# eigenfoo/littlemcmc

Hardware: AMD Instinct MI355X
Metric: leapfrog-steps/sec (all chains) (higher is better)
Workload: dtype f64

## Files before the change

include/lmc_hip.h:

```cpp
#ifndef LMC_HIP_H_
#define LMC_HIP_H_

#include <stdint.h>

#ifdef __cplusplus
extern "C" {
#endif

#define LMC_ABI_VERSION 8

#define LMC_OK 0
#define LMC_ERR_INVALID 1
#define LMC_ERR_HIP 2
#define LMC_ERR_STATE 3

#define LMC_KIND_NUTS 0
#define LMC_KIND_HMC 1

#define LMC_POT_DIAG_ADAPT 0
#define LMC_POT_DIAG 1
#define LMC_POT_FULL 2
#define LMC_POT_FULL_INV 3
#define LMC_POT_FULL_ADAPT 4
#define LMC_POT_FULL_F64 5

#define LMC_TARGET_STD_NORMAL 0
#define LMC_TARGET_DIAG_GAUSSIAN 1
#define LMC_TARGET_AR1 2
#define LMC_TARGET_FUNNEL 3
#define LMC_TARGET_NORMAL1D 4
#define LMC_TARGET_USER 5
#define LMC_TARGET_EXTERNAL 6

#define LMC_SDOT_NATIVE 0
#define LMC_SDOT_OPENBLAS_SKYLAKEX 1
#define LMC_SDOT_OPENBLAS_HASWELL 2

#define LMC_RNG_NUMPY 0
#define LMC_RNG_PHILOX 1

#define LMC_LDS_PLAN_AUTO 0
#define LMC_LDS_PLAN_SHALLOW 1
#define LMC_LDS_PLAN_DEEP 2

#define LMC_STATUS_BAD_INITIAL_ENERGY 1

#define LMC_STAT_STEP_SIZE 0
#define LMC_STAT_STEP_SIZE_BAR 1
#define LMC_STAT_ACCEPT 2
#define LMC_STAT_ENERGY_ERROR 3
#define LMC_STAT_ENERGY 4
#define LMC_STAT_MAX_ENERGY_ERROR 5
#define LMC_STAT_MODEL_LOGP 6
#define LMC_NUM_STAT_F64 7
#define LMC_STAT_DEPTH 0
#define LMC_STAT_TREE_SIZE 1
#define LMC_NUM_STAT_I32 2
#define LMC_STAT_DIVERGING 0
#define LMC_STAT_TUNE 1
#define LMC_STAT_ACCEPTED 2
#define LMC_NUM_STAT_U8 3

#define LMC_CT_REACHED_MAX_TREEDEPTH 0
#define LMC_CT_DIVS_AFTER_TUNE 1
#define LMC_CT_SAMPLES_AFTER_TUNE 2
#define LMC_CT_LEAPFROGS 3
#define LMC_CT_WAVE_TICKS 4
#define LMC_NUM_COUNTERS 5

typedef struct lmc_engine lmc_engine;

typedef struct lmc_tuning {
    int32_t sub_blocks;
    int32_t force_general;
    int32_t general_team;
    int32_t run_ns, run_w;
    int32_t dense_coop_off;
    int32_t dense_cache_rows_p1;
    int32_t dense_lds_slots_p1;
    int32_t chol_hbm;
    int32_t reserved[3];
} lmc_tuning;

typedef struct lmc_config {
    int32_t abi_version;
    int32_t device;
    int32_t chains;
    int32_t dim;
    int32_t kind;
    int32_t target_family;
    int32_t potential;
    int32_t adapt_step_size;
    double target_accept;
    double emax;
    double step_scale;
    double gamma;
    double k;
    double t0;
    int32_t max_treedepth;
    int32_t early_max_treedepth;
    double path_length;
    int32_t max_steps;
    int32_t adaptation_window;
    int32_t lds_levels;
    int32_t start_energy_sdot;
    double adaptation_window_multiplier;
    int32_t rng_mode;
    int32_t mass_f64;
    int32_t lds_plan;
    int32_t reserved0;
    lmc_tuning tuning;
} lmc_config;

void lmc_config_defaults(lmc_config* cfg, int32_t chains, int32_t dim);

const char* lmc_last_error(const lmc_engine* e);
int32_t lmc_abi_version(void);
const char* lmc_build_hash(void);
int32_t lmc_device_count(void);
int32_t lmc_has_target(int32_t family);

int lmc_engine_create(const lmc_config* cfg, lmc_engine** out);
void lmc_engine_destroy(lmc_engine* e);
int lmc_engine_set_stream(lmc_engine* e, void* hip_stream);
int lmc_engine_synchronize(lmc_engine* e);

int lmc_engine_set_target_params(lmc_engine* e, const double* params, int64_t n);

int lmc_engine_set_potential(lmc_engine* e, const double* initial_mean, const double* initial_diag,
                             double initial_weight, int32_t per_chain);

int lmc_engine_set_dense_potential(lmc_engine* e, const double* matrix, const double* initial_mean,
                                   double initial_weight, int32_t adaptation_window,
                                   double adaptation_window_multiplier, int32_t update_window);

int lmc_engine_seed(lmc_engine* e, const uint32_t* seeds);
int lmc_engine_set_rng_state(lmc_engine* e, int32_t chain, const uint32_t* key, int32_t pos,
                             int32_t has_gauss, double gauss);
int lmc_engine_get_rng_state(lmc_engine* e, int32_t chain, uint32_t* key, int32_t* pos,
                             int32_t* has_gauss, double* gauss);

int lmc_engine_set_position(lmc_engine* e, const double* q, int32_t per_chain);
int lmc_engine_get_position(lmc_engine* e, double* q);

int lmc_engine_reset_tuning(lmc_engine* e);
int lmc_engine_set_dual_average(lmc_engine* e, double log_step, double log_bar, double hbar,
                                int32_t count);

int lmc_engine_set_step_jitter(lmc_engine* e, int32_t enable, double lo, double hi);
int lmc_engine_set_step_sizes(lmc_engine* e, const double* step_sizes);
int lmc_engine_diag_update(lmc_engine* e, int32_t tune);
int lmc_engine_reserve(lmc_engine* e, int64_t capacity, int64_t trace_begin);
int lmc_engine_attach_trace(lmc_engine* e, double* dst, int64_t trace_begin);
int lmc_engine_request_stop(lmc_engine* e, int32_t stop);
int64_t lmc_engine_progress(lmc_engine* e);
int lmc_engine_run(lmc_engine* e, int64_t n_tune, int64_t iter_begin, int32_t n_iters);
#define LMC_MAX_RUN_STREAMS 8
int lmc_engine_run_streams(lmc_engine* e, void** streams, int32_t capacity);
int32_t lmc_engine_last_run_plan(lmc_engine* e);

int lmc_engine_get_trace(lmc_engine* e, double* dst, int64_t iter_begin, int64_t n_iters);
int lmc_engine_get_stat_f64(lmc_engine* e, int32_t stat, double* dst, int64_t iter_begin, int64_t n_iters);
int lmc_engine_get_stat_i32(lmc_engine* e, int32_t stat, int32_t* dst, int64_t iter_begin, int64_t n_iters);
int lmc_engine_get_stat_u8(lmc_engine* e, int32_t stat, uint8_t* dst, int64_t iter_begin, int64_t n_iters);
#define LMC_PLANE_F64 0
#define LMC_PLANE_I32 1
#define LMC_PLANE_U8 2
#define LMC_AS_NATIVE 0
#define LMC_AS_F64 1
#define LMC_AS_I64 2
#define LMC_MAX_PLANES 16
typedef struct lmc_window_plane {
    void* dst;
    int32_t kind;
    int32_t idx;
    int32_t as;
    int32_t reserved;
} lmc_window_plane;
typedef struct lmc_window_dst {
    int64_t n_out;
    int64_t first;
    double* trace;
    int32_t n_planes;
    int32_t copy_workgroups;
    lmc_window_plane plane[LMC_MAX_PLANES];
} lmc_window_dst;
int lmc_engine_copy_window_async(lmc_engine* e, const lmc_window_dst* dst, int64_t iter_begin, int64_t n_iters);
int lmc_engine_copy_wait(lmc_engine* e);
void* lmc_host_alloc(uint64_t bytes);
void lmc_host_free(void* p);
int lmc_host_register(void* p, uint64_t bytes);
int lmc_host_unregister(void* p);

#define LMC_STAT_RECORD_BYTES 64
void* lmc_engine_trace_device_ptr(lmc_engine* e);
void* lmc_engine_stat_records_device_ptr(lmc_engine* e);
int64_t lmc_engine_trace_begin(lmc_engine* e);
int64_t lmc_engine_capacity(lmc_engine* e);

int lmc_engine_get_adapt_state(lmc_engine* e, float* var, double* dual_avg, int32_t* da_count,
                               int32_t* n_samples);
typedef struct lmc_chain_state {
    float* var;
    double* fore_mean;
    double* fore_raw_var;
    double* back_mean;
    double* back_raw_var;
    double* fore_w_sum;
    double* back_w_sum;
    int32_t* n_samples;
    double* log_step;
    double* log_bar;
    double* hbar;
    int32_t* da_count;
    int32_t* iter_count;
    int32_t* window;
    double* var64;
} lmc_chain_state;
int lmc_engine_get_chain_state(lmc_engine* e, const lmc_chain_state* dst);
int lmc_engine_set_chain_state(lmc_engine* e, const lmc_chain_state* src);
typedef struct lmc_dense_state {
    float* cov;
    float* chol;
    double* fore_mean;
    double* fore_raw_cov;
    double* fore_n;
    double* back_mean;
    double* back_raw_cov;
    double* back_n;
    int32_t* window;
    int32_t* previous_update;
    int32_t* chol_failures;
    double* cov64;
    double* chol64;
} lmc_dense_state;
int lmc_engine_get_dense_state(lmc_engine* e, const lmc_dense_state* dst);
int lmc_engine_set_dense_state(lmc_engine* e, const lmc_dense_state* src);
int lmc_engine_get_dense_chain(lmc_engine* e, int32_t chain, float* cov, float* chol);
int lmc_engine_get_dense_chain_f64(lmc_engine* e, int32_t chain, double* cov, double* chol);
int lmc_engine_get_dense_factor_f64(lmc_engine* e, double* chol);
int lmc_engine_dense_update(lmc_engine* e, int32_t tune);

// ... 33 lines not shown
```

littlemcmc_amd/_abi.py:

```python
import ctypes as C
import os

import numpy as np

_HERE = os.path.dirname(os.path.abspath(__file__))
LIB_PATH = os.environ.get("LMC_HIP_LIB") or os.path.join(_HERE, "liblmc_hip.so")

ABI_VERSION = 8
OK = 0

KIND_NUTS, KIND_HMC = 0, 1
POT_DIAG_ADAPT, POT_DIAG, POT_FULL, POT_FULL_INV, POT_FULL_ADAPT, POT_FULL_F64 = range(6)
TARGET_STD_NORMAL, TARGET_DIAG_GAUSSIAN, TARGET_AR1, TARGET_FUNNEL, TARGET_NORMAL1D, TARGET_USER, TARGET_EXTERNAL = range(7)
STATUS_BAD_INITIAL_ENERGY = 1
SDOT_NATIVE, SDOT_OPENBLAS_SKYLAKEX, SDOT_OPENBLAS_HASWELL = 0, 1, 2
RNG_NUMPY, RNG_PHILOX = 0, 1
LDS_PLAN_AUTO, LDS_PLAN_SHALLOW, LDS_PLAN_DEEP = 0, 1, 2
PLANE_F64, PLANE_I32, PLANE_U8 = 0, 1, 2
AS_NATIVE, AS_F64, AS_I64 = 0, 1, 2
MAX_PLANES = 16
MAX_RUN_STREAMS = 8
(STAT_STEP_SIZE, STAT_STEP_SIZE_BAR, STAT_ACCEPT, STAT_ENERGY_ERROR, STAT_ENERGY, STAT_MAX_ENERGY_ERROR,
 STAT_MODEL_LOGP) = range(7)
STAT_DEPTH, STAT_TREE_SIZE = 0, 1
STAT_DIVERGING, STAT_TUNE, STAT_ACCEPTED = 0, 1, 2
CT_REACHED_MAX_TREEDEPTH, CT_DIVS_AFTER_TUNE, CT_SAMPLES_AFTER_TUNE, CT_LEAPFROGS, CT_WAVE_TICKS = range(5)
NUM_COUNTERS = 5
STAT_RECORD_BYTES = 64


class Tuning(C.Structure):

    _fields_ = [("sub_blocks", C.c_int32), ("force_general", C.c_int32), ("general_team", C.c_int32), ("run_ns", C.c_int32),
                ("run_w", C.c_int32), ("dense_coop_off", C.c_int32), ("dense_cache_rows_p1", C.c_int32),
                ("dense_lds_slots_p1", C.c_int32), ("chol_hbm", C.c_int32), ("reserved", C.c_int32 * 3)]


class Config(C.Structure):

    _fields_ = [
        ("abi_version", C.c_int32), ("device", C.c_int32), ("chains", C.c_int32), ("dim", C.c_int32),
        ("kind", C.c_int32), ("target_family", C.c_int32), ("potential", C.c_int32),
        ("adapt_step_size", C.c_int32),
        ("target_accept", C.c_double), ("emax", C.c_double), ("step_scale", C.c_double),
        ("gamma", C.c_double), ("k", C.c_double), ("t0", C.c_double),
        ("max_treedepth", C.c_int32), ("early_max_treedepth", C.c_int32),
        ("path_length", C.c_double), ("max_steps", C.c_int32), ("adaptation_window", C.c_int32),
        ("lds_levels", C.c_int32), ("start_energy_sdot", C.c_int32), ("adaptation_window_multiplier", C.c_double),
        ("rng_mode", C.c_int32), ("mass_f64", C.c_int32), ("lds_plan", C.c_int32), ("reserved0", C.c_int32),
        ("tuning", Tuning),
    ]


class WindowPlane(C.Structure):

    _fields_ = [("dst", C.c_void_p), ("kind", C.c_int32), ("idx", C.c_int32), ("as_", C.c_int32), ("reserved", C.c_int32)]


class WindowDst(C.Structure):

    _fields_ = [("n_out", C.c_int64), ("first", C.c_int64), ("trace", C.c_void_p), ("n_planes", C.c_int32),
                ("copy_workgroups", C.c_int32), ("plane", WindowPlane * MAX_PLANES)]


_P = C.c_void_p


class ChainState(C.Structure):

    FIELDS = (("var", np.float32, True), ("fore_mean", np.float64, True), ("fore_raw_var", np.float64, True),
              ("back_mean", np.float64, True), ("back_raw_var", np.float64, True), ("fore_w_sum", np.float64, False),
              ("back_w_sum", np.float64, False), ("n_samples", np.int32, False), ("log_step", np.float64, False),
              ("log_bar", np.float64, False), ("hbar", np.float64, False), ("da_count", np.int32, False),
              ("iter_count", np.int32, False), ("window", np.int32, False), ("var64", np.float64, True))
    _fields_ = [(name, C.c_void_p) for name, _dt, _vec in FIELDS]


class DenseState(C.Structure):

    FIELDS = (("cov", np.float32, "m"), ("chol", np.float32, "m"), ("fore_mean", np.float64, "v"),
              ("fore_raw_cov", np.float64, "m"), ("fore_n", np.float64, "s"), ("back_mean", np.float64, "v"),
              ("back_raw_cov", np.float64, "m"), ("back_n", np.float64, "s"), ("window", np.int32, "s"),
              ("previous_update", np.int32, "s"), ("chol_failures", np.int32, "s"),
              ("cov64", np.float64, "m"), ("chol64", np.float64, "m"))
    _fields_ = [(name, C.c_void_p) for name, _dt, _k in FIELDS]


_SIGNATURES = {
    "lmc_config_defaults": (None, [C.POINTER(Config), C.c_int32, C.c_int32]),
    "lmc_last_error": (C.c_char_p, [_P]),
    "lmc_abi_version": (C.c_int32, []),
    "lmc_build_hash": (C.c_char_p, []),
    "lmc_device_count": (C.c_int32, []),
    "lmc_has_target": (C.c_int32, [C.c_int32]),
    "lmc_engine_create": (C.c_int, [C.POINTER(Config), C.POINTER(_P)]),
    "lmc_engine_destroy": (None, [_P]),
    "lmc_engine_set_stream": (C.c_int, [_P, _P]),
    "lmc_engine_synchronize": (C.c_int, [_P]),
    "lmc_engine_set_target_params": (C.c_int, [_P, _P, C.c_int64]),
    "lmc_engine_set_potential": (C.c_int, [_P, _P, _P, C.c_double, C.c_int32]),
    "lmc_engine_set_dense_potential": (C.c_int, [_P, _P, _P, C.c_double, C.c_int32, C.c_double, C.c_int32]),
    "lmc_engine_get_dense_state": (C.c_int, [_P, C.POINTER(DenseState)]),
    "lmc_engine_set_dense_state": (C.c_int, [_P, C.POINTER(DenseState)]),
    "lmc_engine_dense_update": (C.c_int, [_P, C.c_int32]),
    "lmc_engine_tick_begin": (C.c_int, [_P, C.c_int64, C.c_int64, C.c_int32]),
    "lmc_engine_tick_positions": (_P, [_P]),
    "lmc_engine_tick": (C.c_int, [_P, _P, _P, C.POINTER(C.c_int32)]),
    "lmc_engine_get_dense_chain": (C.c_int, [_P, C.c_int32, _P, _P]),
    "lmc_engine_get_dense_chain_f64": (C.c_int, [_P, C.c_int32, _P, _P]),
    "lmc_engine_get_dense_factor_f64": (C.c_int, [_P, _P]),
    "lmc_engine_seed": (C.c_int, [_P, _P]),
    "lmc_engine_set_rng_state": (C.c_int, [_P, C.c_int32, _P, C.c_int32, C.c_int32, C.c_double]),
    "lmc_engine_get_rng_state": (C.c_int, [_P, C.c_int32, _P, C.POINTER(C.c_int32), C.POINTER(C.c_int32),
                                           C.POINTER(C.c_double)]),
    "lmc_engine_set_position": (C.c_int, [_P, _P, C.c_int32]),
    "lmc_engine_get_position": (C.c_int, [_P, _P]),
    "lmc_engine_reset_tuning": (C.c_int, [_P]),
    "lmc_engine_set_dual_average": (C.c_int, [_P, C.c_double, C.c_double, C.c_double, C.c_int32]),
    "lmc_engine_reserve": (C.c_int, [_P, C.c_int64, C.c_int64]),
    "lmc_engine_attach_trace": (C.c_int, [_P, _P, C.c_int64]),
    "lmc_engine_run": (C.c_int, [_P, C.c_int64, C.c_int64, C.c_int32]),
    "lmc_engine_run_streams": (C.c_int, [_P, _P, C.c_int32]),
    "lmc_engine_last_run_plan": (C.c_int32, [_P]),
    "lmc_engine_copy_window_async": (C.c_int, [_P, C.POINTER(WindowDst), C.c_int64, C.c_int64]),
    "lmc_engine_copy_wait": (C.c_int, [_P]),
    "lmc_host_alloc": (_P, [C.c_uint64]),
    "lmc_host_free": (None, [_P]),
    "lmc_host_register": (C.c_int, [_P, C.c_uint64]),
    "lmc_host_unregister": (C.c_int, [_P]),
    "lmc_engine_set_step_jitter": (C.c_int, [_P, C.c_int32, C.c_double, C.c_double]),
    "lmc_engine_set_step_sizes": (C.c_int, [_P, _P]),
    "lmc_engine_diag_update": (C.c_int, [_P, C.c_int32]),
    "lmc_engine_get_trace": (C.c_int, [_P, _P, C.c_int64, C.c_int64]),
    "lmc_engine_get_stat_f64": (C.c_int, [_P, C.c_int32, _P, C.c_int64, C.c_int64]),
    "lmc_engine_get_stat_i32": (C.c_int, [_P, C.c_int32, _P, C.c_int64, C.c_int64]),
    "lmc_engine_get_stat_u8": (C.c_int, [_P, C.c_int32, _P, C.c_int64, C.c_int64]),
    "lmc_engine_trace_device_ptr": (_P, [_P]),
    "lmc_engine_stat_records_device_ptr": (_P, [_P]),
    "lmc_engine_trace_begin": (C.c_int64, [_P]),
    "lmc_engine_capacity": (C.c_int64, [_P]),
    "lmc_engine_get_adapt_state": (C.c_int, [_P, _P, _P, _P, _P]),
    "lmc_engine_get_chain_state": (C.c_int, [_P, C.POINTER(ChainState)]),
    "lmc_engine_set_chain_state": (C.c_int, [_P, C.POINTER(ChainState)]),
    "lmc_engine_keep_moments": (C.c_int, [_P, C.c_int32]),
    "lmc_engine_get_moments": (C.c_int, [_P, _P, _P, _P]),
    "lmc_engine_get_status": (C.c_int, [_P, _P]),
    "lmc_engine_get_counters": (C.c_int, [_P, _P]),
    "lmc_engine_trajectory": (C.c_int, [_P, _P, _P, C.c_int32, C.c_double, C.c_int32, C.c_int32,
                                        _P, _P, _P, _P, _P, _P]),
    "lmc_engine_logp_dlogp": (C.c_int, [_P, _P, _P, _P]),
    "lmc_engine_rng_draw": (C.c_int, [_P, _P, C.c_int32, _P]),
    "lmc_engine_draw_momentum": (C.c_int, [_P, _P]),
    "lmc_engine_kernel_shape": (C.c_int, [_P, _P, _P, _P]),
    "lmc_engine_uses_general_kernels": (C.c_int32, [_P]),
    "lmc_engine_occupancy": (C.c_int, [_P, _P, _P, _P]),
    "lmc_engine_request_stop": (C.c_int, [_P, C.c_int32]),
    "lmc_engine_progress": (C.c_int64, [_P]),
    "lmc_engine_run_lds_bytes": (C.c_int32, [_P]),
    "lmc_engine_load_user_kernels": (C.c_int, [_P, _P, C.c_char_p, C.c_char_p, C.c_char_p]),
    "lmc_engine_load_user_run_plan1": (C.c_int, [_P, C.c_char_p]),
    "lmc_diag_lags_per_pass": (C.c_int, []),
    "lmc_diag_chain_stats": (C.c_int, [_P, C.c_int64, C.c_int64, C.c_int32, C.c_int64, C.c_int64, C.c_int32, _P, _P]),
}

EXPORTED_SYMBOLS = tuple(_SIGNATURES)
_libs = {}


class HipLibraryError(RuntimeError):
    """The HIP library is missing, stale or failed; there is no CPU path to fall back to."""


def load(path=None):
    path = os.path.abspath(path or LIB_PATH)
    if path in _libs:
        return _libs[path]
    if not os.path.exists(path):
        raise HipLibraryError(
            "%s not found: the HIP extension is not built. Run `python -c \"import __graft_entry__ as g; "
            "g.build()\"` (needs hipcc). littlemcmc_amd has no CPU fallback." % path)
    try:
        lib = C.CDLL(path)
    except OSError as err:
        raise HipLibraryError("cannot load %s: %s" % (path, err))
    for name, (res, args) in _SIGNATURES.items():
        try:
            fn = getattr(lib, name)
        except AttributeError:
            raise HipLibraryError("%s does not export %s (stale build?)" % (path, name))
        fn.restype = res
        fn.argtypes = args
    if lib.lmc_abi_version() != ABI_VERSION:
        raise HipLibraryError("ABI version mismatch: python %d, library %d" % (ABI_VERSION, lib.lmc_abi_version()))
    _libs[path] = lib
    return lib


def ptr(a):
    if a is None:
        return None
    if isinstance(a, (int, np.integer)):
        return C.c_void_p(int(a))
    assert a.flags["C_CONTIGUOUS"], "array must be C-contiguous"
    return C.c_void_p(a.ctypes.data)
```

littlemcmc_amd/csrc/lmc_engine.hip:

```cpp
#include <hip/hip_runtime.h>

#include <cmath>
#include <cstdarg>
#include <cstdio>
#include <algorithm>
#include <cstdlib>
#include <cstring>
#include <new>
#include <string>
#include <vector>

#include "../../include/lmc_hip.h"
#include "lmc_sampler.hpp"
#include "lmc_unit_kernels.hpp"
#include "lmc_dense_launch.hpp"
#include "lmc_tick_launch.hpp"
#include "lmc_wide_launch.hpp"
#ifdef LMC_USER_TARGET_HEADER
#include LMC_USER_TARGET_HEADER
#endif

using namespace lmc;

#define LMC_LAUNCH(...)            \
// ... 176 lines not shown
    const long long k = static_cast<long long>(blockIdx.x) * blockDim.x + threadIdx.x;
    if (k >= static_cast<long long>(chains) * n) return;
    const long long c = k / n, i = k - c * n;
    const StatRecord& r = rec[c * cap + iter_begin + i];
    if (kind == 0) static_cast<double*>(out)[k] = r.f64[idx];
    else if (kind == 1) static_cast<int*>(out)[k] = (idx == kSiTreeSize || hmc) ? r.tree_size : static_cast<int>(r.depth_flags & 0xffffu);
    else static_cast<unsigned char*>(out)[k] = static_cast<unsigned char>((r.depth_flags >> (16 + idx)) & 1u);
}

struct WindowPlanes {
    int n_planes;
    int kind[LMC_MAX_PLANES], idx[LMC_MAX_PLANES], as[LMC_MAX_PLANES];
    void* dst[LMC_MAX_PLANES];
};
__global__ void window_gather_kernel(const StatRecord* rec, long long cap, int chain0, int chains, long long iter_begin, long long n, int hmc,
                                     WindowPlanes W, long long n_out, long long row0) {
    const long long total = static_cast<long long>(chains) * n;
    for (long long k = static_cast<long long>(blockIdx.x) * blockDim.x + threadIdx.x; k < total; k += static_cast<long long>(gridDim.x) * blockDim.x) {
        const long long c = chain0 + k / n, i = k % n;
        const StatRecord r = rec[c * cap + iter_begin + i];
        const long long o = c * n_out + row0 + i;
        for (int p = 0; p < W.n_planes; ++p) {
            void* out = W.dst[p];
            if (W.kind[p] == LMC_PLANE_F64) {
                static_cast<double*>(out)[o] = r.f64[W.idx[p]];
            } else if (W.kind[p] == LMC_PLANE_I32) {
                const int v = (W.idx[p] == kSiTreeSize || hmc) ? r.tree_size : static_cast<int>(r.depth_flags & 0xffffu);
                if (W.as[p] == LMC_AS_F64) static_cast<double*>(out)[o] = static_cast<double>(v);
                else if (W.as[p] == LMC_AS_I64) static_cast<long long*>(out)[o] = static_cast<long long>(v);
                else static_cast<int*>(out)[o] = v;
            } else {
                static_cast<unsigned char*>(out)[o] = static_cast<unsigned char>((r.depth_flags >> (16 + W.idx[p])) & 1u);
            }
        }
    }
}

template <int V>
__global__ void window_trace_copy_kernel(const double* __restrict__ src, long long src_pitch, double* __restrict__ dst, long long dst_pitch,
                                         long long row, int chains) {
    for (int c = blockIdx.x; c < chains; c += gridDim.x) {
        const double* s = src + c * src_pitch;
        double* t = dst + c * dst_pitch;
        if constexpr (V == 2) {
            const double2* s2 = reinterpret_cast<const double2*>(s);
            double2* t2 = reinterpret_cast<double2*>(t);
            for (long long k = threadIdx.x; k < row / 2; k += blockDim.x) t2[k] = s2[k];
        } else {
            for (long long k = threadIdx.x; k < row; k += blockDim.x) t[k] = s[k];
        }
    }
}

__global__ void derive_inv_std_kernel(ChainArrays A, int from64) {
    const long long idx = static_cast<long long>(blockIdx.x) * blockDim.x + threadIdx.x;
    const long long n = static_cast<long long>(A.chains) * A.dpad;
    if (idx >= n) return;
    if (from64) {
        const double v = A.var64[idx];
        A.inv_std64[idx] = 1.0 / sqrt(v);
        A.var[idx] = static_cast<float>(v);
        A.inv_std[idx] = static_cast<float>(A.inv_std64[idx]);
        return;
    }
    const float sd = sqrtf(A.var[idx]);
    A.inv_std[idx] = 1.0f / sd;
    if (A.var64 != nullptr) {
        A.var64[idx] = static_cast<double>(A.var[idx]);
        A.inv_std64[idx] = static_cast<double>(A.inv_std[idx]);
    }
}

}

static thread_local std::string g_last_error;

struct lmc_engine {
    lmc_config cfg;
    int ns = 0, dpad = 0, nlds = 1, lds_bytes = 0;
    int nlds1 = 1, lds_bytes1 = 0, lds_plan = 0;
    int lds_plan_wanted = 0;
    int plan_now = 0;
    int plan_last = -1;
    bool wide = false;
    double* init_diag64 = nullptr;
    int run_ns = 0, run_w = 1;
    hipStream_t own_stream = nullptr, stream_ = nullptr;
#ifndef LMC_MAX_SUB
#define LMC_MAX_SUB 4
#endif
#ifndef LMC_DEFAULT_SUB
#define LMC_DEFAULT_SUB 4
#endif
    static constexpr int kMaxSub = LMC_MAX_SUB;
    int n_sub = 1;
    hipStream_t sub_stream[kMaxSub] = {};
    hipEvent_t sub_done[kMaxSub] = {};
    hipEvent_t main_done = nullptr;
    bool trace_external = false;
    hipStream_t copy_stream = nullptr;
    hipEvent_t copy_dep[kMaxSub + 1] = {};
    double* chol64T = nullptr;
    uint32_t* seeds = nullptr;
    int* stop_host = nullptr;
    int step_jitter = 0;
    int step_jitter_device = 0;
    double* step_override = nullptr;
    double jitter_lo = 1.0, jitter_hi = 1.0;
    bool sub_pending = false;
    bool main_dirty = true;
    ChainArrays A;
    double* tparams = nullptr;
    int64_t n_tparams = 0;
    double* init_mean = nullptr;
    float* init_diag = nullptr;
    double init_weight = 10.0;
    bool potential_set = false;
    double* da_tables = nullptr;
    double initial_step = 0.0;
    DenseArrays D;
    int d8 = 0;
    void* cov1T = nullptr;
    void* fac1 = nullptr;
    double* raw1T = nullptr;
    double* mean1 = nullptr;
    double dense_weight = 1.0, dense_multiplier = 2.0;
    int dense_window = 101, dense_update_window = 1;
    TickArrays K;
    bool ticking = false;
    int* adapt_mask = nullptr;
    hipModule_t user_module = nullptr;
    hipFunction_t user_run = nullptr, user_trajectory = nullptr, user_logp = nullptr;
    hipFunction_t user_run1 = nullptr;
    std::vector<void*> allocs;
    std::string err;
};

static hipStream_t main_stream(lmc_engine* e) {
    if (e->sub_pending) {
        for (int b = 0; b < e->n_sub; ++b) {
            (void)hipEventRecord(e->sub_done[b], e->sub_stream[b]);
            (void)hipStreamWaitEvent(e->stream_, e->sub_done[b], 0);
        }
        e->sub_pending = false;
    }
    e->main_dirty = true;
    return e->stream_;
}

static hipError_t order_sub_blocks_after_main(lmc_engine* e) {
    if (e->n_sub <= 1) return hipSuccess;
    const bool external = e->stream_ != e->own_stream;
    if (!e->main_dirty && !external) return hipSuccess;
    hipError_t err = hipEventRecord(e->main_done, e->stream_);
    for (int b = 0; b < e->n_sub && err == hipSuccess; ++b) err = hipStreamWaitEvent(e->sub_stream[b], e->main_done, 0);
    if (err == hipSuccess) e->main_dirty = false;
    return err;
}
static hipError_t order_external_stream_after_sub_blocks(lmc_engine* e) {
    if (e->n_sub <= 1 || e->stream_ == e->own_stream || !e->sub_pending) return hipSuccess;
    hipError_t err = hipSuccess;
    for (int b = 0; b < e->n_sub && err == hipSuccess; ++b) {
        err = hipEventRecord(e->sub_done[b], e->sub_stream[b]);
        if (err == hipSuccess) err = hipStreamWaitEvent(e->stream_, e->sub_done[b], 0);
    }
    if (err == hipSuccess) e->sub_pending = false;
// ... 227 lines not shown
}

extern "C" {

int32_t lmc_abi_version(void) { return LMC_ABI_VERSION; }

#ifndef LMC_SOURCE_HASH
#define LMC_SOURCE_HASH "unstamped"
#endif
static const char kBuildStamp[] = "LMC_BUILD_HASH=" LMC_SOURCE_HASH;
const char* lmc_build_hash(void) { return kBuildStamp + 15; }

int32_t lmc_device_count(void) {
    int n = 0;
    if (hipGetDeviceCount(&n) != hipSuccess) { (void)hipGetLastError(); return 0; }
    return n;
}

int32_t lmc_has_target(int32_t family) {
#if !(defined(LMC_USER_TARGET_HEADER) && defined(LMC_ONLY_USER))
    if (family >= LMC_TARGET_STD_NORMAL && family <= LMC_TARGET_NORMAL1D) return 1;
#endif
    if (family == LMC_TARGET_USER) return 1;
    if (family == LMC_TARGET_EXTERNAL) return 1;
    return 0;
}

const char* lmc_last_error(const lmc_engine* e) {
    if (e && !e->err.empty()) return e->err.c_str();
    return g_last_error.c_str();
}

void lmc_config_defaults(lmc_config* cfg, int32_t chains, int32_t dim) {
    std::memset(cfg, 0, sizeof(*cfg));
    cfg->abi_version = LMC_ABI_VERSION;
    cfg->device = 0;
    cfg->chains = chains;
    cfg->dim = dim;
    cfg->kind = LMC_KIND_NUTS;
    cfg->target_family = LMC_TARGET_STD_NORMAL;
    cfg->potential = LMC_POT_DIAG_ADAPT;
    cfg->adapt_step_size = 1;
    cfg->target_accept = 0.8;
    cfg->emax = 1000.0;
    cfg->step_scale = 0.25;
    cfg->gamma = 0.05;
    cfg->k = 0.75;
    cfg->t0 = 10.0;
    cfg->max_treedepth = 10;
    cfg->early_max_treedepth = 8;
    cfg->path_length = 2.0;
    cfg->max_steps = 1024;
    cfg->adaptation_window = 101;
    cfg->adaptation_window_multiplier = 1.0;
    cfg->rng_mode = LMC_RNG_NUMPY;
    cfg->mass_f64 = 0;
    cfg->lds_levels = 0;
    cfg->lds_plan = LMC_LDS_PLAN_AUTO;
    cfg->start_energy_sdot = LMC_SDOT_OPENBLAS_SKYLAKEX;
}

static int launch_reset(lmc_engine* e, int reset_step, int reset_mass) {
    const long long n = static_cast<long long>(e->cfg.chains) * e->dpad;
    const int threads = 256;
    const int blocks = static_cast<int>((n + threads - 1) / threads);
    const double log_step0 = std::log(e->initial_step);
    const double mu = std::log(10 * e->initial_step);
    LMC_LAUNCH(reset_kernel, dim3(blocks), dim3(threads), 0, main_stream(e), e->A, e->init_mean, e->init_diag,
                       e->init_diag64, e->cfg.mass_f64, e->init_weight, e->cfg.potential == LMC_POT_DIAG_ADAPT ? 1 : 0, log_step0, mu, reset_step,
                       reset_mass, e->cfg.adaptation_window);
    HIP_TRY(e, hipGetLastError());
    return LMC_OK;
}

int lmc_engine_create(const lmc_config* cfg, lmc_engine** out) {
    if (!cfg || !out) return fail(nullptr, LMC_ERR_INVALID, "null argument");
    *out = nullptr;
    if (cfg->abi_version != LMC_ABI_VERSION)
        return fail(nullptr, LMC_ERR_INVALID, "ABI version mismatch: header %d, library %d", cfg->abi_version,
                    LMC_ABI_VERSION);
    if (cfg->chains < 1 || cfg->dim < 1) return fail(nullptr, LMC_ERR_INVALID, "chains and dim must be >= 1");
    if (cfg->lds_plan < LMC_LDS_PLAN_AUTO || cfg->lds_plan > LMC_LDS_PLAN_DEEP)
        return fail(nullptr, LMC_ERR_INVALID, "unknown lds_plan %d", cfg->lds_plan);
    if (cfg->reserved0 != 0 || cfg->tuning.reserved[0] != 0 || cfg->tuning.reserved[1] != 0 || cfg->tuning.reserved[2] != 0)
        return fail(nullptr, LMC_ERR_INVALID, "reserved fields of lmc_config must be 0");
    if (cfg->potential < LMC_POT_DIAG_ADAPT || cfg->potential > LMC_POT_FULL_F64)
        return fail(nullptr, LMC_ERR_INVALID, "unknown potential %d", cfg->potential);
    if (cfg->mass_f64 && cfg->potential > LMC_POT_DIAG && cfg->potential != LMC_POT_FULL_ADAPT)
        return fail(nullptr, LMC_ERR_INVALID, "mass_f64 is the dtype of the diagonal potentials and of LMC_POT_FULL_ADAPT "
                                              "(float64 fixed matrices: LMC_POT_FULL_F64 / LMC_POT_FULL_INV)");
    const bool rtc_dense = cfg->target_family == LMC_TARGET_USER && !kUserCompiledInDense && cfg->potential >= LMC_POT_FULL &&
                           cfg->potential != LMC_POT_FULL_ADAPT;
    const bool forced = cfg->tuning.force_general != 0 && cfg->rng_mode == LMC_RNG_NUMPY &&
                        (cfg->target_family != LMC_TARGET_EXTERNAL || cfg->potential < LMC_POT_FULL);
    const bool wide = cfg->dim > 1024 || (cfg->potential >= LMC_POT_FULL && cfg->dim > 256) || cfg->mass_f64 != 0 || rtc_dense || forced;
    if (wide) {
        if (cfg->dim > kWideMaxDim)
            return fail(nullptr, LMC_ERR_INVALID, "dim %d is beyond the general kernels' %d", cfg->dim, kWideMaxDim);
        if (cfg->potential >= LMC_POT_FULL && cfg->dim > kWideMaxDenseDim)
            return fail(nullptr, LMC_ERR_INVALID, "dense mass matrices are supported up to dim %d (got %d)", kWideMaxDenseDim, cfg->dim);
        if (cfg->potential == LMC_POT_FULL_ADAPT && cfg->dim > kWideMaxDenseAdaptDim)
            return fail(nullptr, LMC_ERR_INVALID, "per-chain adapted dense matrices (FULL_ADAPT) are supported up to dim %d (got %d)",
                        kWideMaxDenseAdaptDim, cfg->dim);
        if (cfg->target_family == LMC_TARGET_EXTERNAL && (cfg->potential >= LMC_POT_FULL || cfg->mass_f64))
            return fail(nullptr, LMC_ERR_INVALID, "an externally evaluated density runs with diagonal float32 mass matrices at any dim up to %d, "
                                                  "with dense ones up to dim 256; give the density as a device functor for the other shapes", kWideMaxDim);
        if (cfg->rng_mode != LMC_RNG_NUMPY)
            return fail(nullptr, LMC_ERR_INVALID, "LMC_RNG_PHILOX runs in the fused kernels only");
    }
    if (!lmc_has_target(cfg->target_family))
        return fail(nullptr, LMC_ERR_INVALID, "target family %d is not built into this library", cfg->target_family);
    if (cfg->target_family == LMC_TARGET_NORMAL1D && cfg->dim != 1)
        return fail(nullptr, LMC_ERR_INVALID, "LMC_TARGET_NORMAL1D requires dim == 1");
    if (cfg->kind != LMC_KIND_NUTS && cfg->kind != LMC_KIND_HMC)
        return fail(nullptr, LMC_ERR_INVALID, "unknown step kind %d", cfg->kind);
    if (cfg->start_energy_sdot < LMC_SDOT_NATIVE || cfg->start_energy_sdot > LMC_SDOT_OPENBLAS_HASWELL)
        return fail(nullptr, LMC_ERR_INVALID, "unknown start_energy_sdot mode %d", cfg->start_energy_sdot);
    if (cfg->adaptation_window < 1 || !(cfg->adaptation_window_multiplier > 0.0))
        return fail(nullptr, LMC_ERR_INVALID, "adaptation_window must be >= 1 and its multiplier > 0");
    if (cfg->rng_mode != LMC_RNG_NUMPY && cfg->rng_mode != LMC_RNG_PHILOX)
        return fail(nullptr, LMC_ERR_INVALID, "unknown rng_mode %d", cfg->rng_mode);
    if (cfg->rng_mode == LMC_RNG_PHILOX && (cfg->potential >= LMC_POT_FULL ||
                                            cfg->target_family == LMC_TARGET_USER || cfg->target_family == LMC_TARGET_EXTERNAL))
        return fail(nullptr, LMC_ERR_INVALID, "LMC_RNG_PHILOX runs in the fused diagonal-mass kernels with the built-in densities");
    if (cfg->max_treedepth < 1 || cfg->max_treedepth > 20 || cfg->early_max_treedepth < 1 ||
        cfg->early_max_treedepth > 20)
        return fail(nullptr, LMC_ERR_INVALID, "max_treedepth must be in [1, 20]");
    int ndev = 0;
    hipError_t herr = hipGetDeviceCount(&ndev);
    if (herr != hipSuccess || ndev < 1)
        return fail(nullptr, LMC_ERR_HIP, "no HIP device available (%s)", hipGetErrorString(herr));
    if (cfg->device < 0 || cfg->device >= ndev)
        return fail(nullptr, LMC_ERR_INVALID, "device %d out of range (%d devices)", cfg->device, ndev);

    lmc_engine* e = new (std::nothrow) lmc_engine();
    if (!e) return fail(nullptr, LMC_ERR_INVALID, "out of host memory");
    e->cfg = *cfg;
    e->wide = wide;
    e->ns = ns_for_dim(cfg->dim);
    e->dpad = 64 * e->ns;
    if (wide) {
        const bool large_team = cfg->dim > kWideOneWaveMaxDim || cfg->target_family == LMC_TARGET_EXTERNAL || cfg->tuning.general_team == 16;
        const int threads = large_team ? kWideBlock : 64;
        int wns = 1;
        while (threads * wns < cfg->dim) wns *= 2;
        e->ns = e->run_ns = wns;
        e->run_w = threads / 64;
        e->dpad = threads * wns;
    } else
    if (e->ns <= 2) { e->run_ns = e->ns; e->run_w = 1; }
    else if (e->ns == 4) { e->run_ns = 4; e->run_w = 1; }
    else if (e->ns == 8) { e->run_ns = 4; e->run_w = 2; }
    else { e->run_ns = 4; e->run_w = 4; }
    if (!wide && cfg->tuning.run_ns > 0 && cfg->tuning.run_w > 0) {
        if (64 * cfg->tuning.run_ns * cfg->tuning.run_w == e->dpad) { e->run_ns = cfg->tuning.run_ns; e->run_w = cfg->tuning.run_w; }
    }
    e->initial_step = cfg->step_scale / std::pow(static_cast<double>(cfg->dim), 0.25);

    auto bail = [&](int rc) {
        lmc_engine_destroy(e);
        return rc;
    };
    hipError_t se = hipSetDevice(cfg->device);
    if (se != hipSuccess) return bail(fail(nullptr, LMC_ERR_HIP, "hipSetDevice: %s", hipGetErrorString(se)));
    {
        int pr_low = 0, pr_high = 0;
        se = hipDeviceGetStreamPriorityRange(&pr_low, &pr_high);
        if (se == hipSuccess) se = hipStreamCreateWithPriority(&e->own_stream, hipStreamNonBlocking, pr_high);
    }
    if (se != hipSuccess) return bail(fail(nullptr, LMC_ERR_HIP, "hipStreamCreate: %s", hipGetErrorString(se)));
    e->stream_ = e->own_stream;
    e->n_sub = (cfg->chains >= 128 && !wide) ? (LMC_DEFAULT_SUB < lmc_engine::kMaxSub ? LMC_DEFAULT_SUB : lmc_engine::kMaxSub) : 1;
    if (e->n_sub > 2 && cfg->potential >= LMC_POT_FULL) e->n_sub = 2;
    if (cfg->tuning.sub_blocks >= 1 && cfg->tuning.sub_blocks <= lmc_engine::kMaxSub && cfg->tuning.sub_blocks <= cfg->chains)
        e->n_sub = cfg->tuning.sub_blocks;
    if (cfg->tuning.sub_blocks <= -1 && e->n_sub > -cfg->tuning.sub_blocks) e->n_sub = -cfg->tuning.sub_blocks;
    if (cfg->tuning.sub_blocks <= -1 && cfg->potential >= LMC_POT_FULL) e->n_sub = 1;
    if (e->n_sub > 1) {
        for (int b = 0; b < e->n_sub; ++b) {
            se = hipStreamCreateWithFlags(&e->sub_stream[b], hipStreamNonBlocking);
            if (se == hipSuccess) se = hipEventCreateWithFlags(&e->sub_done[b], hipEventDisableTiming);
            if (se != hipSuccess) return bail(fail(nullptr, LMC_ERR_HIP, "sub-block stream: %s", hipGetErrorString(se)));
        }
        se = hipEventCreateWithFlags(&e->main_done, hipEventDisableTiming);
        if (se != hipSuccess) return bail(fail(nullptr, LMC_ERR_HIP, "hipEventCreate: %s", hipGetErrorString(se)));
    }

    const int max_levels = (cfg->max_treedepth > cfg->early_max_treedepth ? cfg->max_treedepth
                                                                          : cfg->early_max_treedepth);
    int nlds = 1;
    if (wide) {
        e->nlds = 1;
        e->lds_bytes = wide_lds_bytes(e->dpad);
    } else {
        const int waves_per_cu = 4 * run_waves_per_simd(e->run_ns, e->run_w);
        const int blocks_per_cu = waves_per_cu / e->run_w > 0 ? waves_per_cu / e->run_w : 1;
        const long budget = (163840L / blocks_per_cu) / 1280 * 1280 - lds_tail_doubles(e->run_w) * 8L;
        if (pair_min_doubles(e->run_ns, e->run_w) * 8L > budget)
            return bail(fail(nullptr, LMC_ERR_INVALID, "the sampling kernel's LDS plan does not fit the budget"));
        nlds = cfg->lds_levels > 0 ? cfg->lds_levels : 1;
        if (cfg->lds_levels <= 0)
            while (nlds < max_levels && pair_total_doubles(e->run_ns, e->run_w, nlds + 1) * 8L <= budget) ++nlds;
        if (nlds > max_levels) nlds = max_levels;
        if (nlds < 1) nlds = 1;
        e->nlds = nlds;
        e->lds_bytes = pair_total_doubles(e->run_ns, e->run_w, nlds) * 8;
        e->nlds1 = nlds;
        e->lds_bytes1 = 0;
        e->lds_plan = 0;
        const long budget1 = (163840L / blocks_per_cu) / 1280 * 1280;
        if (e->run_w == 1 && run_mt_in_lds(1) && cfg->lds_levels <= 0 && pair_min_doubles(e->run_ns, 1, 1) * 8L <= budget1) {
            int n1 = 1;
            while (n1 < max_levels && pair_total_doubles(e->run_ns, 1, n1 + 1, 1) * 8L <= budget1) ++n1;
            e->nlds1 = n1;
            e->lds_bytes1 = pair_total_doubles(e->run_ns, 1, n1, 1) * 8;
            e->lds_plan = cfg->lds_plan == LMC_LDS_PLAN_SHALLOW ? 0 : cfg->lds_plan == LMC_LDS_PLAN_DEEP ? 1 : 2;
            if (e->nlds1 <= e->nlds) e->lds_plan = 0;
            if (cfg->rng_mode == LMC_RNG_PHILOX) e->lds_plan = 0;
            e->lds_plan_wanted = e->lds_plan;
            if (cfg->target_family == LMC_TARGET_USER && !kUserCompiledIn)
                e->lds_plan = 0;
            e->plan_now = e->lds_plan == 1 ? 1 : 0;
        }
    }
    if (e->lds_bytes > 160 * 1024) return bail(fail(nullptr, LMC_ERR_INVALID, "lds_levels too large"));

    const size_t C = cfg->chains, dp = e->dpad;
    ChainArrays& A = e->A;
    std::memset(&A, 0, sizeof(A));
    A.chains = cfg->chains;
    A.d = cfg->dim;
    A.dpad = e->dpad;
    int rc = LMC_OK;
#define TRY_ALLOC(x) if ((rc = (x)) != LMC_OK) return bail(rc)
    TRY_ALLOC(dev_alloc(e, &A.q, C * dp));
    TRY_ALLOC(dev_alloc(e, &A.var, C * dp));
    TRY_ALLOC(dev_alloc(e, &A.inv_std, C * dp));
    TRY_ALLOC(dev_alloc(e, &A.wmean, 2 * C * dp));
    TRY_ALLOC(dev_alloc(e, &A.wraw, 2 * C * dp));
    TRY_ALLOC(dev_alloc(e, &A.wsum, C * 2));
    TRY_ALLOC(dev_alloc(e, &A.wsel, C));
    TRY_ALLOC(dev_alloc(e, &A.n_samples, C));
    TRY_ALLOC(dev_alloc(e, &A.awindow, C));
    TRY_ALLOC(dev_alloc(e, &A.da, C * 4));
    TRY_ALLOC(dev_alloc(e, &A.da_count, C));
    TRY_ALLOC(dev_alloc(e, &A.iter_count, C));
    TRY_ALLOC(dev_alloc(e, &A.mt, C * kMtN));
    TRY_ALLOC(dev_alloc(e, &A.rng_pos, C));
    TRY_ALLOC(dev_alloc(e, &A.rng_has_gauss, C));
    TRY_ALLOC(dev_alloc(e, &A.rng_gauss, C));
    TRY_ALLOC(dev_alloc(e, &A.status, C));
    TRY_ALLOC(dev_alloc(e, &A.counters, C * kNumCounters));
    {
        void* dev_view = nullptr;
        if (hipHostMalloc(reinterpret_cast<void**>(&e->stop_host), 128, hipHostMallocMapped | hipHostMallocCoherent) != hipSuccess ||
            hipHostGetDevicePointer(&dev_view, e->stop_host, 0) != hipSuccess)
            return bail(fail(nullptr, LMC_ERR_HIP, "stop word: %s", hipGetErrorString(hipGetLastError())));
        std::memset(e->stop_host, 0, 128);
        A.stop = static_cast<const int*>(dev_view);
        A.progress = static_cast<int*>(dev_view) + 16;
        A.tree_hint = static_cast<int*>(dev_view) + 24;
    }
    TRY_ALLOC(dev_alloc(e, &A.stop_dev, 1));
    TRY_ALLOC(dev_alloc(e, &e->seeds, C));
    A.seed = e->seeds;
    A.scratch_stride = static_cast<long long>(max_levels - nlds + 1) * 4 * dp + static_cast<long long>(kNumColdSlots) * dp;
    const bool dense = cfg->potential >= LMC_POT_FULL;
    if (dense) A.scratch_stride = static_cast<long long>(dense_scratch_vectors(max_levels)) * dp;
    const bool external = cfg->target_family == LMC_TARGET_EXTERNAL;
    if (external) A.scratch_stride = static_cast<long long>(dense ? tick_dense_scratch_vectors(max_levels) : tick_scratch_vectors(max_levels)) * dp;
    if (wide) {
        if (!external) A.scratch_stride = static_cast<long long>(wide_scratch_slots(max_levels)) * dp;
        TRY_ALLOC(dev_alloc(e, &A.var64, C * dp));
        TRY_ALLOC(dev_alloc(e, &A.inv_std64, C * dp));
        TRY_ALLOC(dev_alloc(e, &e->init_diag64, C * dp));
    }
    TRY_ALLOC(dev_alloc(e, &A.scratch, C * static_cast<size_t>(A.scratch_stride), false));
    TRY_ALLOC(dev_alloc(e, &e->init_mean, C * dp));
    TRY_ALLOC(dev_alloc(e, &e->init_diag, C * dp));
    TRY_ALLOC(dev_alloc(e, &e->tparams, 8));
    {
        const int len = 16384;
        std::vector<double> tab(2 * static_cast<size_t>(len));
        for (int i = 0; i < len; ++i) {
            tab[i] = std::sqrt(static_cast<double>(i));
            tab[len + i] = i > 0 ? std::pow(static_cast<double>(i), -cfg->k) : 0.0;
        }
        TRY_ALLOC(dev_alloc(e, &e->da_tables, tab.size(), false));
        hipError_t ce = hipMemcpy(e->da_tables, tab.data(), tab.size() * sizeof(double), hipMemcpyHostToDevice);
        if (ce != hipSuccess) return bail(fail(nullptr, LMC_ERR_HIP, "da tables: %s", hipGetErrorString(ce)));
        A.da_sqrt = e->da_tables;
        A.da_mk = e->da_tables + len;
        A.da_table_len = len;
    }
#undef TRY_ALLOC
    std::memset(&e->K, 0, sizeof(e->K));
    if (external) {
        TickArrays& K = e->K;
// ... 76 lines not shown
        rc = lmc_engine_set_potential(e, zeros.data(), ones.data(), 10.0, 0);
        if (rc != LMC_OK) return bail(rc);
        rc = launch_reset(e, 1, 0);
        if (rc != LMC_OK) return bail(rc);
        if (dense) {
            std::vector<double> eye(static_cast<size_t>(cfg->dim) * cfg->dim, 0.0);
            for (int i = 0; i < cfg->dim; ++i) eye[static_cast<size_t>(i) * cfg->dim + i] = 1.0;
            rc = lmc_engine_set_dense_potential(e, eye.data(), zeros.data(), 1.0, 101, 2.0, 1);
            if (rc != LMC_OK) return bail(rc);
        }
        std::vector<uint32_t> seeds(C, 0u);
        rc = lmc_engine_seed(e, seeds.data());
        if (rc != LMC_OK) return bail(rc);
    }
    se = hipStreamSynchronize(main_stream(e));
    if (se != hipSuccess) return bail(fail(nullptr, LMC_ERR_HIP, "engine init: %s", hipGetErrorString(se)));
    *out = e;
    return LMC_OK;
}

void lmc_engine_destroy(lmc_engine* e) {
    if (!e) return;
    (void)hipSetDevice(e->cfg.device);
    if (e->stream_) (void)hipStreamSynchronize(main_stream(e));
    for (int b = 0; b < lmc_engine::kMaxSub; ++b) {
        if (e->sub_stream[b]) { (void)hipStreamSynchronize(e->sub_stream[b]); (void)hipStreamDestroy(e->sub_stream[b]); }
        if (e->sub_done[b]) (void)hipEventDestroy(e->sub_done[b]);
    }
    if (e->main_done) (void)hipEventDestroy(e->main_done);
    if (e->copy_stream) { (void)hipStreamSynchronize(e->copy_stream); (void)hipStreamDestroy(e->copy_stream); }
    for (hipEvent_t ev : e->copy_dep)
        if (ev) (void)hipEventDestroy(ev);
    if (e->stop_host) (void)hipHostFree(e->stop_host);
    for (void* p : e->allocs)
        if (p) (void)hipFree(p);
    if (e->user_module) (void)hipModuleUnload(e->user_module);
    if (e->own_stream) (void)hipStreamDestroy(e->own_stream);
    delete e;
}


int lmc_engine_kernel_shape(lmc_engine* e, int32_t* unit_ns, int32_t* run_ns, int32_t* run_w) {
    if (!e) return fail(nullptr, LMC_ERR_INVALID, "null engine");
    if (unit_ns) *unit_ns = e->ns;
    if (run_ns) *run_ns = e->run_ns;
    if (run_w) *run_w = e->run_w;
    return LMC_OK;
}

int32_t lmc_engine_uses_general_kernels(lmc_engine* e) { return (e && e->wide) ? 1 : 0; }

int lmc_engine_occupancy(lmc_engine* e, int32_t* resident_chains, int32_t* waves_per_chain, double* wall_clock_hz) {
    if (!e) return fail(nullptr, LMC_ERR_INVALID, "null engine");
    HIP_TRY(e, hipSetDevice(e->cfg.device));
    if (waves_per_chain) *waves_per_chain = e->run_w;
    if (wall_clock_hz) {
        int khz = 0;
        HIP_TRY(e, hipDeviceGetAttribute(&khz, hipDeviceAttributeWallClockRate, e->cfg.device));
        *wall_clock_hz = 1e3 * khz;
    }
    if (!resident_chains) return LMC_OK;
    *resident_chains = 0;
    if (e->cfg.target_family == LMC_TARGET_EXTERNAL || e->cfg.potential >= LMC_POT_FULL || e->wide) return LMC_OK;
    int cus = 0;
    HIP_TRY(e, hipDeviceGetAttribute(&cus, hipDeviceAttributeMultiprocessorCount, e->cfg.device));
    const int run_lds = sampling_lds_bytes(e);
    const int block = 64 * e->run_w;
    int per_cu = 0;
    if (e->cfg.target_family == LMC_TARGET_USER && !kUserCompiledIn) {
        if (!e->user_run) return fail(e, LMC_ERR_STATE, "the user density's kernels are not loaded");
        HIP_TRY(e, hipModuleOccupancyMaxActiveBlocksPerMultiprocessor(&per_cu, e->user_run, block, static_cast<size_t>(run_lds)));
        *resident_chains = per_cu * cus;
        return LMC_OK;
    }
#define OCC_ONE(NSV, WV, T)                                                                                    \
    if (!found && e->run_ns == NSV && e->run_w == WV) {                                                        \
        found = true;                                                                                          \
        if (e->cfg.rng_mode == LMC_RNG_PHILOX) {                                                               \
            if (run_lds > 64 * 1024)                                                                           \
                HIP_TRY(e, hipFuncSetAttribute(reinterpret_cast<const void*>(&run_kernel<NSV, WV, T, 1>),      \
                                               hipFuncAttributeMaxDynamicSharedMemorySize, run_lds));          \
            HIP_TRY(e, hipOccupancyMaxActiveBlocksPerMultiprocessor(&per_cu, run_kernel<NSV, WV, T, 1>, block, \
                                                                    static_cast<size_t>(run_lds)));            \
        } else {                                                                                               \
            if (run_lds > 64 * 1024)                                                                           \
                HIP_TRY(e, hipFuncSetAttribute(reinterpret_cast<const void*>(&run_kernel<NSV, WV, T>),         \
                                               hipFuncAttributeMaxDynamicSharedMemorySize, run_lds));          \
            HIP_TRY(e, hipOccupancyMaxActiveBlocksPerMultiprocessor(&per_cu, run_kernel<NSV, WV, T>, block,    \
                                                                    static_cast<size_t>(run_lds)));            \
        }                                                                                                      \
    }
#define OCC_CALL(T)                                                                                            \
    {                                                                                                          \
        bool found = false;                                                                                    \
        LMC_FOR_EACH_SHAPE(OCC_ONE, T)                                                                         \
        if (!found) return fail(e, LMC_ERR_INVALID, "unsupported kernel shape ns=%d w=%d", e->run_ns, e->run_w); \
    }
    LMC_FAMILY_SWITCH(e, e->cfg.target_family, OCC_CALL)
#undef OCC_CALL
#undef OCC_ONE
    *resident_chains = per_cu * cus;
    return LMC_OK;
}

int32_t lmc_engine_run_lds_bytes(lmc_engine* e) {
    if (!e || e->cfg.target_family == LMC_TARGET_EXTERNAL || (e->cfg.potential >= LMC_POT_FULL && !e->wide)) return -1;
    if (e->wide) return e->lds_bytes;
    return sampling_lds_bytes(e, e->plan_last >= 0 ? e->plan_last : e->plan_now);
}

int32_t lmc_engine_last_run_plan(lmc_engine* e) {
    if (!e || e->plan_last < 0 || e->wide || e->cfg.potential >= LMC_POT_FULL || e->cfg.target_family == LMC_TARGET_EXTERNAL) return 0;
    return e->plan_last == 1 ? LMC_LDS_PLAN_DEEP : LMC_LDS_PLAN_SHALLOW;
}

int lmc_engine_load_user_kernels(lmc_engine* e, const void* code_object, const char* run_name, const char* trajectory_name,
                                 const char* logp_name) {
    if (!e || !code_object || !run_name || !trajectory_name || !logp_name) return fail(e, LMC_ERR_INVALID, "null argument");
    if (e->cfg.target_family != LMC_TARGET_USER)
        return fail(e, LMC_ERR_STATE, "lmc_engine_load_user_kernels() needs cfg.target_family = LMC_TARGET_USER");
    HIP_TRY(e, hipSetDevice(e->cfg.device));
    HIP_TRY(e, hipStreamSynchronize(main_stream(e)));
    if (e->user_module) { (void)hipModuleUnload(e->user_module); e->user_module = nullptr; }
    e->user_run = e->user_trajectory = e->user_logp = nullptr;
    e->user_run1 = nullptr;
    if (e->cfg.target_family == LMC_TARGET_USER && !kUserCompiledIn) { e->lds_plan = 0; e->plan_now = 0; }
    HIP_TRY(e, hipModuleLoadData(&e->user_module, code_object));
    HIP_TRY(e, hipModuleGetFunction(&e->user_run, e->user_module, run_name));
    HIP_TRY(e, hipModuleGetFunction(&e->user_trajectory, e->user_module, trajectory_name));
    HIP_TRY(e, hipModuleGetFunction(&e->user_logp, e->user_module, logp_name));
    return LMC_OK;
}

int lmc_engine_load_user_run_plan1(lmc_engine* e, const char* run_name_plan1) {
    if (!e || !run_name_plan1) return fail(e, LMC_ERR_INVALID, "null argument");
    if (!e->user_module) return fail(e, LMC_ERR_STATE, "lmc_engine_load_user_kernels() first");
    if (e->wide || e->run_w != 1) return fail(e, LMC_ERR_INVALID, "the deep-tree LDS plan exists for the one-wave sampling kernels");
    HIP_TRY(e, hipSetDevice(e->cfg.device));
    HIP_TRY(e, hipModuleGetFunction(&e->user_run1, e->user_module, run_name_plan1));
    e->lds_plan = e->lds_plan_wanted;
    e->plan_now = e->lds_plan == 1 ? 1 : 0;
    return LMC_OK;
}

static int user_launch(lmc_engine* e, hipFunction_t f, hipStream_t st, unsigned grid, unsigned block, unsigned lds, void** args) {
    if (!f)
        return fail(e, LMC_ERR_STATE, "the user density's kernels are not loaded: call lmc_engine_load_user_kernels() "
                                      "(littlemcmc_amd.targets.UserTarget does)");
    if (e->cfg.potential >= LMC_POT_FULL && !e->wide)
        return fail(e, LMC_ERR_INVALID, "a run-time compiled user density runs with diagonal mass matrices in the fused kernels; "
                                        "dense ones (Full / FullInv) take the general kernels, FullAdapt needs the density compiled in (UserTarget(..., jit=\"hipcc\"))");
    (void)hipGetLastError();
    HIP_TRY(e, hipModuleLaunchKernel(f, grid, 1, 1, block, 1, 1, lds, st, args, nullptr));
    return LMC_OK;
}

int lmc_engine_set_step_sizes(lmc_engine* e, const double* step_sizes) {
    if (!e) return fail(nullptr, LMC_ERR_INVALID, "null engine");
    HIP_TRY(e, hipSetDevice(e->cfg.device));
    if (!step_sizes) {
        if (e->step_jitter == 2) e->step_jitter = e->step_jitter_device;
        return LMC_OK;
    }
    if (!e->step_override) {
        int rc = dev_alloc(e, &e->step_override, static_cast<size_t>(e->cfg.chains));
        if (rc != LMC_OK) return rc;
        e->A.step_override = e->step_override;
    }
    HIP_TRY(e, hipMemcpyAsync(e->step_override, step_sizes, sizeof(double) * e->cfg.chains, hipMemcpyDefault, main_stream(e)));
    HIP_TRY(e, hipStreamSynchronize(main_stream(e)));
    e->step_jitter = 2;
    return LMC_OK;
}

int lmc_engine_diag_update(lmc_engine* e, int32_t tune) {
    if (!e) return fail(nullptr, LMC_ERR_INVALID, "null engine");
    if (e->cfg.potential != LMC_POT_DIAG_ADAPT) return LMC_OK;
    if (!tune) return LMC_OK;
    HIP_TRY(e, hipSetDevice(e->cfg.device));
    SamplerParams P;
    std::memset(&P, 0, sizeof(P));
    P.window = e->cfg.adaptation_window;
    P.window_multiplier = e->cfg.adaptation_window_multiplier;
    P.mass_f64 = e->cfg.mass_f64 ? 1 : 0;
    if (e->wide) {
        const int rc = wide_launch_mass_update(e->ns, e->run_w, main_stream(e), e->A, P);
        if (rc != 0) return dense_fail(e, rc, "diag_update (general kernel)");
        return LMC_OK;
    }
    const dim3 grid(e->cfg.chains), block(64);
    LMC_NS_SWITCH(e, e->ns, LMC_LAUNCH((mass_update_kernel<NS>), grid, block, 0, main_stream(e), e->A, P))
    HIP_TRY(e, hipGetLastError());
    return LMC_OK;
// ... 626 lines not shown
    P.k = e->cfg.k;
    P.t0 = e->cfg.t0;
    P.max_treedepth = e->cfg.max_treedepth;
    P.early_max_treedepth = e->cfg.early_max_treedepth;
    P.path_length = e->cfg.path_length;
    P.max_steps = e->cfg.max_steps;
    P.window = e->cfg.adaptation_window;
    P.window_multiplier = e->cfg.adaptation_window_multiplier;
    P.n_tune = n_tune;
    P.iter_begin = iter_begin;
    P.n_iters = n_iters;
    P.nlds = e->nlds;
    P.lds_doubles = e->lds_bytes / 8;
    P.sdot_mode = e->cfg.start_energy_sdot;
    P.rng_mode = e->cfg.rng_mode;
    P.step_jitter = e->step_jitter;
    P.jitter_lo = e->jitter_lo;
    P.jitter_hi = e->jitter_hi;
    P.relay_mask = 255;
    return P;
}

static int wide_run(lmc_engine* e, SamplerParams P) {
    if (e->cfg.potential >= LMC_POT_FULL) P.momentum_f32 = !e->D.mat_f64;
    if (e->cfg.potential != LMC_POT_DIAG_ADAPT) P.adapt_mass = 0;
    P.chain_begin = 0;
    P.relay_mask = relay_mask_for(e->cfg.chains);
    hipStream_t st = main_stream(e);
    const bool rtc = e->cfg.target_family == LMC_TARGET_USER && !kUserCompiledInDense;
    const long long end = P.iter_begin + P.n_iters;
    long long it = P.iter_begin;
    while (it < end) {
        const bool adapt = e->cfg.potential == LMC_POT_FULL_ADAPT && it < P.n_tune;
        SamplerParams Q = P;
        Q.iter_begin = it;
        Q.n_iters = static_cast<int>(adapt ? 1 : end - it);
        int rc;
        if (rtc) {
            void* args[] = {&e->A, &e->D, &Q, &e->tparams};
            rc = user_launch(e, e->user_run, st, static_cast<unsigned>(e->cfg.chains), 64u * e->run_w, static_cast<unsigned>(e->lds_bytes), args);
            if (rc != LMC_OK) return rc;
        } else {
            rc = wide_launch_run(e->cfg.target_family, e->ns, e->run_w, st, e->A, e->D, Q, e->tparams, e->cfg.chains);
            if (rc != 0) return dense_fail(e, rc, "run (general kernel)");
        }
        if (adapt) {
            rc = dense_launch_adapt(st, e->A, e->D, e->dense_multiplier, e->dense_update_window, nullptr, 0, e->cfg.chains,
                                    static_cast<int>(it + 1));
            if (rc != 0) return dense_fail(e, rc, "dense update");
        }
        it += Q.n_iters;
    }
    return LMC_OK;
}

int lmc_engine_run(lmc_engine* e, int64_t n_tune, int64_t iter_begin, int32_t n_iters) {
    if (!e) return fail(nullptr, LMC_ERR_INVALID, "null engine");
    if (e->A.cap <= 0 || !e->A.stat_rec) return fail(e, LMC_ERR_STATE, "lmc_engine_reserve() must be called before run()");
    if (iter_begin < 0 || n_iters < 0 || iter_begin + n_iters > e->A.cap)
        return fail(e, LMC_ERR_INVALID, "iterations [%lld, %lld) exceed reserved capacity %lld", (long long)iter_begin,
                    (long long)(iter_begin + n_iters), (long long)e->A.cap);
    if (n_iters == 0) return LMC_OK;
    if (e->cfg.target_family == LMC_TARGET_EXTERNAL)
        return fail(e, LMC_ERR_STATE, "the density is evaluated by the caller: drive the chains with lmc_engine_tick_begin() / lmc_engine_tick()");
    HIP_TRY(e, hipSetDevice(e->cfg.device));
    SamplerParams P = make_params(e, n_tune, iter_begin, n_iters);
    if (e->wide) return wide_run(e, P);
    if (e->cfg.potential >= LMC_POT_FULL) return dense_run(e, P);
    int plan = choose_lds_plan(e, iter_begin);
    if (e->run_w != 1 || e->lds_bytes1 <= 0 ||
        (e->cfg.target_family == LMC_TARGET_USER && !kUserCompiledIn && !e->user_run1))
        plan = 0;
    e->plan_last = plan;
    if (plan == 1) {
        P.nlds = e->nlds1;
        P.lds_doubles = e->lds_bytes1 / 8;
    }
    const int run_lds = sampling_lds_bytes(e, plan);
    const dim3 block(64 * e->run_w);
    const int n_sub = e->n_sub;
    HIP_TRY(e, order_sub_blocks_after_main(e));
#define RUN_PLAN1(NSV, WV, T)                                                                                  \
    if constexpr (WV == 1) {                                                                                   \
        LMC_LAUNCH((run_kernel<NSV, 1, T, 0, 1>), grid, block, run_lds, st, e->A, P, e->tparams);              \
    }
#define RUN_ONE(NSV, WV, T)                                                                                    \
    if (!found && e->run_ns == NSV && e->run_w == WV) {                                                        \
        found = true;                                                                                          \
        if (e->cfg.rng_mode == LMC_RNG_PHILOX) {                                                               \
            if (run_lds > 64 * 1024)                                                                           \
                HIP_TRY(e, hipFuncSetAttribute(reinterpret_cast<const void*>(&run_kernel<NSV, WV, T, 1>),      \
                                               hipFuncAttributeMaxDynamicSharedMemorySize, run_lds));          \
            LMC_LAUNCH((run_kernel<NSV, WV, T, 1>), grid, block, run_lds, st, e->A, P, e->tparams);            \
        } else if (plan == 1) {                                                                                \
            RUN_PLAN1(NSV, WV, T)                                                                              \
        } else {                                                                                               \
            if (run_lds > 64 * 1024)                                                                           \
                HIP_TRY(e, hipFuncSetAttribute(reinterpret_cast<const void*>(&run_kernel<NSV, WV, T>),         \
                                               hipFuncAttributeMaxDynamicSharedMemorySize, run_lds));          \
            LMC_LAUNCH((run_kernel<NSV, WV, T>), grid, block, run_lds, st, e->A, P, e->tparams);               \
        }                                                                                                      \
    }
#define RUN_CALL(T)                                                                                            \
    {                                                                                                          \
        bool found = false;                                                                                    \
        LMC_FOR_EACH_SHAPE(RUN_ONE, T)                                                                         \
        if (!found) return fail(e, LMC_ERR_INVALID, "unsupported kernel shape ns=%d w=%d", e->run_ns, e->run_w); \
    }
    for (int b = 0; b < n_sub; ++b) {
        const long long lo = static_cast<long long>(e->cfg.chains) * b / n_sub, hi = static_cast<long long>(e->cfg.chains) * (b + 1) / n_sub;
        P.chain_begin = static_cast<int>(lo);
        P.relay_mask = relay_mask_for(hi - lo);
        const dim3 grid(static_cast<unsigned>(hi - lo));
        hipStream_t st = n_sub > 1 ? e->sub_stream[b] : main_stream(e);
        if (n_sub > 1) e->sub_pending = true;
        if (e->cfg.target_family == LMC_TARGET_USER && !kUserCompiledIn) {
            void* args[] = {&e->A, &P, &e->tparams};
            const int rc = user_launch(e, plan == 1 ? e->user_run1 : e->user_run, st, grid.x, block.x, static_cast<unsigned>(run_lds), args);
            if (rc != LMC_OK) return rc;
            continue;
        }
        LMC_FAMILY_SWITCH(e, e->cfg.target_family, RUN_CALL)
    }
#undef RUN_CALL
#undef RUN_ONE
#undef RUN_PLAN1
    HIP_TRY(e, hipGetLastError());
    HIP_TRY(e, order_external_stream_after_sub_blocks(e));
    return LMC_OK;
}

int lmc_engine_run_streams(lmc_engine* e, void** streams, int32_t capacity) {
    if (!e) return fail(nullptr, LMC_ERR_INVALID, "null engine");
    const int n = e->n_sub > 1 ? e->n_sub : 1;
    if (streams)
        for (int b = 0; b < n && b < capacity; ++b) streams[b] = e->n_sub > 1 ? static_cast<void*>(e->sub_stream[b]) : static_cast<void*>(e->stream_);
    return n;
}

int lmc_engine_tick_begin(lmc_engine* e, int64_t n_tune, int64_t iter_begin, int32_t n_iters) {
    if (!e) return fail(nullptr, LMC_ERR_INVALID, "null engine");
    if (e->cfg.target_family != LMC_TARGET_EXTERNAL)
        return fail(e, LMC_ERR_STATE, "lmc_engine_tick*() needs cfg.target_family = LMC_TARGET_EXTERNAL");
    if (e->A.cap <= 0 || !e->A.stat_rec) return fail(e, LMC_ERR_STATE, "lmc_engine_reserve() must be called before tick_begin()");
    if (iter_begin < 0 || n_iters < 0 || iter_begin + n_iters > e->A.cap)
        return fail(e, LMC_ERR_INVALID, "iterations [%lld, %lld) exceed reserved capacity %lld", (long long)iter_begin,
                    (long long)(iter_begin + n_iters), (long long)e->A.cap);
    HIP_TRY(e, hipSetDevice(e->cfg.device));
    e->K.iter_end = iter_begin + n_iters;
    e->K.n_tune = n_tune;
    const int rc = e->wide ? tick_wide_launch_begin(e->ns, main_stream(e), e->A, e->K, iter_begin)
                           : tick_launch_begin(e->ns, main_stream(e), e->A, e->K, iter_begin);
    if (rc != 0) return fail(e, LMC_ERR_HIP, "tick_begin: %s", rc < 0 ? "unsupported vector width" : hipGetErrorString(static_cast<hipError_t>(rc)));
    e->ticking = true;
    return LMC_OK;
}

void* lmc_engine_tick_positions(lmc_engine* e) { return e ? e->K.q_eval : nullptr; }

int lmc_engine_tick(lmc_engine* e, const double* logp, const double* grad, int32_t* n_active) {
    if (!e || !logp || !grad) return fail(e, LMC_ERR_INVALID, "null argument");
    if (!e->ticking) return fail(e, LMC_ERR_STATE, "lmc_engine_tick_begin() must be called first");
    HIP_TRY(e, hipSetDevice(e->cfg.device));
    SamplerParams P = make_params(e, e->K.n_tune, 0, 0);
    if (e->cfg.potential >= LMC_POT_FULL) {
        P.momentum_f32 = !pot_f64(e->cfg.potential);
        P.adapt_mass = 0;
        int rc = tick_dense_launch(e->ns, pot_f64(e->cfg.potential), main_stream(e), e->A, e->D, e->K, P, logp, grad,
                                   e->adapt_mask);
        if (rc != 0) return dense_fail(e, rc, "tick");
        if (e->cfg.potential == LMC_POT_FULL_ADAPT) {
            rc = dense_launch_adapt(main_stream(e), e->A, e->D, e->dense_multiplier, e->dense_update_window, e->adapt_mask);
            if (rc != 0) return dense_fail(e, rc, "dense update");
        }
    } else {
        const int rc = e->wide ? tick_wide_launch(e->ns, main_stream(e), e->A, e->K, P, logp, grad)
                               : tick_launch(e->ns, main_stream(e), e->A, e->K, P, logp, grad);
        if (rc != 0) return fail(e, LMC_ERR_HIP, "tick: %s", rc < 0 ? "unsupported vector width" : hipGetErrorString(static_cast<hipError_t>(rc)));
// ... 526 lines not shown
```

littlemcmc_amd/csrc/lmc_sampler.hpp:

```cpp
#pragma once
#include "lmc_rng.hpp"
#include "lmc_targets.hpp"
#include "lmc_team.hpp"

namespace lmc {

constexpr int kStatusBadInitialEnergy = 1;

enum StatF64 : int {
    kSfStepSize = 0,
    kSfStepSizeBar = 1,
    kSfAccept = 2,
    kSfEnergyError = 3,
    kSfEnergy = 4,
    kSfMaxEnergyError = 5,
    kSfModelLogp = 6,
    kNumStatF64 = 7
};
enum StatI32 : int { kSiDepth = 0 , kSiTreeSize = 1 , kNumStatI32 = 2 };
enum StatU8 : int { kSbDiverging = 0, kSbTune = 1, kSbAccepted = 2, kNumStatU8 = 3 };
enum Counter : int { kCtMaxTreedepth = 0, kCtDivsSample = 1, kCtSamplesAfterTune = 2, kCtLeapfrogs = 3, kCtWaveTicks = 4, kNumCounters = 5 };

struct StatRecord {
    double f64[kNumStatF64];
// ... 446 lines not shown
    __device__ __forceinline__ void get(int j, double& w_, double& a_, double& c, double& d) const {
        w_ = readlane_f64(w, j); a_ = readlane_f64(a, j); c = readlane_f64(pe, j); d = readlane_f64(plogp, j);
    }
};

struct TransitionOut {
    double accept;
    double energy, energy_error, max_energy_error, model_logp;
    int depth;
    int n_leapfrog;
    int diverging;
    int exhausted;
    int accepted;
};

template <class P>
__device__ inline void hmc_transition_any(P& pol, double e0, double logp0, double step_size, double emax, double path_length,
                                          int max_steps, TransitionOut& out) {
    const double plen = first_f64(pol.uniform() * path_length);
    int n_steps = static_cast<int>(plen / step_size);
    n_steps = n_steps < 1 ? 1 : n_steps;
    n_steps = n_steps > max_steps ? max_steps : n_steps;
    typename P::End c;
    pol.start_state(c);
    double energy = e0, logp = logp0;
    for (int i = 0; i < n_steps; ++i) pol.leapfrog(step_size, c, energy, logp);
    bool diverging = !isfinite(energy);
    double de = first_f64(e0 - energy);
    if (isnan(de)) de = -__builtin_inf();
    if (fabs(de) > emax) diverging = true;
    const double accept = first_f64(fmin(1.0, exp_uniform(de)));
    bool accepted = false;
    if (!diverging) {
        const double u = pol.uniform();
        if (!(u >= accept)) { accepted = true; pol.accept_state(c); }
    }
    out.accept = accept;
    out.energy = energy;
    out.energy_error = de;
    out.max_energy_error = plen;
    out.model_logp = logp;
    out.depth = n_steps;
    out.n_leapfrog = n_steps;
    out.diverging = diverging;
    out.exhausted = 0;
    out.accepted = accepted;
}

template <int NS, class Target, class TeamT>
struct FusedHmcPolicy {
    static constexpr int kNS = NS;
    struct End { double q[NS], p[NS], g[NS]; };
    TeamT& tm; const Target& tgt; const double (&var)[NS]; RngState& rng;
    double (&q)[NS]; const double (&p0)[NS]; const double (&g0)[NS];
    UniformWindow win;
    __device__ __forceinline__ double uniform() { return team_uniform(tm, rng, win); }
    __device__ __forceinline__ void start_state(End& c) const { vcopy(c.q, q); vcopy(c.p, p0); vcopy(c.g, g0); }
    __device__ __forceinline__ void leapfrog(double eps, End& c, double& energy, double& logp) {
        lmc::leapfrog<NS>(tm, tgt, var, eps, c.q, c.p, c.g, energy, logp);
    }
    __device__ __forceinline__ void accept_state(const End& c) { vcopy(q, c.q); }
};
template <int NS, class Target, class TeamT>
__device__ inline void hmc_transition(TeamT& tm, const Target& tgt, const double (&var)[NS], RngState& rng,
                                      double (&q)[NS], const double (&p0)[NS], const double (&g0)[NS],
                                      double e0, double logp0, double step_size, double emax,
                                      double path_length, int max_steps, TransitionOut& out) {
    FusedHmcPolicy<NS, Target, TeamT> pol{tm, tgt, var, rng, q, p0, g0, UniformWindow{0.0, 0, 0}};
    hmc_transition_any(pol, e0, logp0, step_size, emax, path_length, max_steps, out);
}

#ifndef LMC_EXP_LANES_SLOAD
#define LMC_EXP_LANES_SLOAD 2
#endif
constexpr int kRedValues = 6;
constexpr int kExpTableDoubles = 32;
constexpr int kLevelScalDoubles = 96;
#ifndef LMC_PAIR_COLD_LDS
#define LMC_PAIR_COLD_LDS 3
#endif
enum ColdSlot : int { kColdAold = 0, kColdPsum = 1, kColdOp = 2, kColdOq = 3, kColdOg = 4, kNumCold = 5 };
constexpr int kNumColdSlots = kNumCold;

template <int NS, int W = 1, int PL = 0>
struct PairLds {
    static constexpr int DP = 64 * NS * W;
    static constexpr int kRedWave = 64 * kRedValues;
    static constexpr int kRedSize = (2 * DP > W * kRedWave) ? 2 * DP : W * kRedWave;
    static constexpr int kExp = kRedSize;
    static constexpr int kXsum = kExp + kExpTableDoubles;
    static constexpr int kXsumSize = W > 1 ? 2 * 8 * W : 0;
    static constexpr int kScal = kXsum + kXsumSize;
    static constexpr int kCold = kScal + W * kLevelScalDoubles;
    static_assert(PL == 0 || W == 1, "the deep-tree plan exists for one-wave kernels");
    static constexpr int kColdLds = PL == 1 ? (NS >= 4 ? 0 : (LMC_PAIR_COLD_LDS < 1 ? LMC_PAIR_COLD_LDS : 1))
                                            : (W >= 8 ? (LMC_PAIR_COLD_LDS < 2 ? LMC_PAIR_COLD_LDS : 2) : LMC_PAIR_COLD_LDS);
    static constexpr int kL1 = kCold + kColdLds * DP;
    static constexpr int kL2 = kL1 + 3 * DP;
    static constexpr int kMinDoubles = kL2;
    static constexpr int kGlbLevels = (kNumCold - kColdLds) * DP;
    __host__ __device__ static constexpr int total_doubles(int nlds) { return kL2 + (nlds > 1 ? (nlds - 1) * 4 * DP : 0); }
};
#ifdef LMC_EXPERIMENTAL_SHAPES
#define LMC_PAIR_SHAPES(X) X(1, 1) X(2, 1) X(4, 1) X(4, 2) X(4, 4) X(2, 8) X(2, 2) X(1, 4)
#else
#define LMC_PAIR_SHAPES(X) X(1, 1) X(2, 1) X(4, 1) X(4, 2) X(4, 4)
#endif
constexpr int pair_min_doubles(int ns, int w, int plan = 0) {
#define X(NSV, WV) if (ns == NSV && w == WV) return (plan == 1 && WV == 1) ? PairLds<NSV, 1, 1>::kMinDoubles : PairLds<NSV, WV, 0>::kMinDoubles;
    LMC_PAIR_SHAPES(X)
#undef X
    return 1 << 30;
}
constexpr int pair_total_doubles(int ns, int w, int nlds, int plan = 0) {
#define X(NSV, WV) if (ns == NSV && w == WV) return (plan == 1 && WV == 1) ? PairLds<NSV, 1, 1>::total_doubles(nlds) : PairLds<NSV, WV, 0>::total_doubles(nlds);
    LMC_PAIR_SHAPES(X)
#undef X
    return 1 << 30;
}

struct PairCtx {
    double* lds;
    double* glb;
    int nlds;
    int red_lane;
    int wave_red;
    int wave_scal;
    int wave;
    int xpar;
};

template <int NS, int W = 1, int PL = 0>
__device__ __forceinline__ void red_put(const PairCtx& cx, int v, double x) {
    if constexpr (W == 1) ((lds_double*)cx.lds)[v * 64 + lane_id()] = x;
    else ((lds_double*)cx.lds)[v * 64 + lane_id() + cx.wave_red] = x;
}
template <int NS, int W = 1, int PL = 0>
__device__ __forceinline__ double red_gather(PairCtx& cx) {
    typedef double d2 __attribute__((ext_vector_type(2)));
    typedef __attribute__((address_space(3))) d2 lds_d2;
    asm volatile("" ::: "memory");
    unsigned r0 = static_cast<unsigned>(cx.red_lane);
    asm volatile("" : "+v"(r0));
    lds_double* L = (lds_double*)cx.lds;
    const d2 a = *(const lds_d2*)(size_t)(r0), b = *(const lds_d2*)(size_t)(r0 ^ 16u);
    const d2 c = *(const lds_d2*)(size_t)(r0 ^ 32u), d = *(const lds_d2*)(size_t)(r0 ^ 48u);
    asm volatile("" ::: "memory");
    double s = ((a.x + a.y) + (b.x + b.y)) + ((c.x + c.y) + (d.x + d.y));
    s += dpp_f64<0x111>(s);
    s += dpp_f64<0x112>(s);
    s += dpp_f64<0x114>(s);
    if constexpr (W > 1) {
        const int lane = lane_id();
        lds_double* xs = L + (PairLds<NS, W, PL>::kXsum + cx.xpar * (8 * W)) + (lane >> 3) * W;
        if ((lane & 7) == 7) xs[cx.wave] = s;
        __syncthreads();
        double t = xs[0];
#pragma unroll
        for (int w = 1; w < W; ++w) t += xs[w];
        s = t;
        cx.xpar ^= 1;
    }
    return s;
}
__device__ __forceinline__ int red_lane_init() {
    const int lane = lane_id();
    const int row = lane < 8 * kRedValues ? lane : 0;
    return row * 8 + 2 * ((lane >> 2) & 3);
}
__device__ __forceinline__ bool red_any_nonpositive(double s, int k0, int n) {
    const unsigned long long m = ballot64(s <= 0.0);
    unsigned long long sel = 0ull;
    for (int k = k0; k < k0 + n; ++k) sel |= 1ull << (8 * k + 7);
    return (m & sel) != 0ull;
}

__constant__ double kExpLanesConst[8] = {46.166241308446828,
                                         2.16608493865351192654e-02,
                                         5.96317165397058656256e-12,
                                         1.0 / 720.0, 1.0 / 120.0, 1.0 / 24.0, 1.0 / 6.0, 0.0};
struct ExpLanesConst { double inv, hi, lo, c6, c5, c4, c3; };
__device__ __forceinline__ ExpLanesConst exp_lanes_const() {
    ExpLanesConst c;
#if LMC_EXP_LANES_SLOAD == 2
    typedef const __attribute__((address_space(4))) double cst_double;
    cst_double* p = (cst_double*)kExpLanesConst;
    asm volatile("" : "+s"(p));
    c.inv = p[0]; c.hi = p[1]; c.lo = p[2]; c.c6 = p[3]; c.c5 = p[4]; c.c4 = p[5]; c.c3 = p[6];
#elif LMC_EXP_LANES_SLOAD == 1
    c.inv = kExpLanesConst[0]; c.hi = kExpLanesConst[1]; c.lo = kExpLanesConst[2];
    c.c6 = kExpLanesConst[3]; c.c5 = kExpLanesConst[4]; c.c4 = kExpLanesConst[5]; c.c3 = kExpLanesConst[6];
#else
    c.inv = LMC_SC(46.166241308446828); c.hi = LMC_SC(2.16608493865351192654e-02); c.lo = LMC_SC(5.96317165397058656256e-12);
    c.c6 = LMC_SC(1.0 / 720.0); c.c5 = LMC_SC(1.0 / 120.0); c.c4 = LMC_SC(1.0 / 24.0); c.c3 = LMC_SC(1.0 / 6.0);
#endif
    return c;
}
template <int NS, int W = 1, int PL = 0>
__device__ __forceinline__ double exp_lanes(const PairCtx& cx, const ExpLanesConst& c, double x) {
    const double kf = rint(x * c.inv);
    double r = __builtin_fma(-kf, c.hi, x);
    r = __builtin_fma(-kf, c.lo, r);
    const int ki = static_cast<int>(kf);
    const double t = ((const lds_double*)cx.lds)[PairLds<NS, W, PL>::kExp + (ki & 31)];
    double p = fma_sgpr_addend(r, c.c6, c.c5);
    p = fma_sgpr_addend(p, r, c.c4);
    p = fma_sgpr_addend(p, r, c.c3);
    p = __builtin_fma(p, r, 0.5);
    p = __builtin_fma(p, r, 1.0);
    p = __builtin_fma(p, r, 1.0);
    return ldexp(p * t, ki >> 5);
}

template <int NS, int W, int PL, int SLOT>
__device__ __forceinline__ void cold_load(const PairCtx& cx, double (&x)[NS]) {
    using L = PairLds<NS, W, PL>;
    if constexpr (SLOT < L::kColdLds) vload_as<NS>((lds_double*)cx.lds + (L::kCold + SLOT * L::DP), x);
    else vload_as<NS>((glb_double*)cx.glb + (SLOT - L::kColdLds) * L::DP, x);
}
template <int NS, int W, int PL, int SLOT>
__device__ __forceinline__ void cold_store(const PairCtx& cx, const double (&x)[NS]) {
    using L = PairLds<NS, W, PL>;
    if constexpr (SLOT < L::kColdLds) vstore_as<NS>((lds_double*)cx.lds + (L::kCold + SLOT * L::DP), x);
    else vstore_as<NS>((glb_double*)cx.glb + (SLOT - L::kColdLds) * L::DP, x);
}
template <int NS, int W = 1, int PL = 0>
__device__ __forceinline__ void level1_load(const PairCtx& cx, double (&lp)[NS], double (&rp)[NS], double (&ps)[NS]) {
    using L = PairLds<NS, W, PL>;
    lds_double* b = (lds_double*)cx.lds + L::kL1;
    vload_as<NS>(b, lp); vload_as<NS>(b + L::DP, rp);
#pragma unroll
    for (int s = 0; s < NS; ++s) ps[s] = lp[s] + rp[s];
}
template <int NS, int W = 1, int PL = 0>
__device__ __forceinline__ void level1_store(const PairCtx& cx, const double (&lp)[NS], const double (&rp)[NS], const double (&pq)[NS]) {
    using L = PairLds<NS, W, PL>;
    lds_double* b = (lds_double*)cx.lds + L::kL1;
    vstore_as<NS>(b, lp); vstore_as<NS>(b + L::DP, rp); vstore_as<NS>(b + 2 * L::DP, pq);
}
template <int NS, int W = 1, int PL = 0>
__device__ __forceinline__ unsigned glb_level_offset(const PairCtx& cx, int j, int v) {
    using L = PairLds<NS, W, PL>;
    unsigned off = L::kGlbLevels + static_cast<unsigned>(j - cx.nlds - 1) * (4u * L::DP) + static_cast<unsigned>(v) * L::DP;
    asm volatile("" : "+s"(off));
    return off;
}
template <int NS, int W = 1, int PL = 0>
__device__ __forceinline__ void levelN_load(const PairCtx& cx, int j, int v, double (&x)[NS]) {
    using L = PairLds<NS, W, PL>;
    int nl = cx.nlds;
    asm volatile("" : "+s"(nl));
    if (j <= nl) vload_as<NS>((lds_double*)cx.lds + (L::kL2 + (j - 2) * 4 * L::DP + v * L::DP), x);
    else vload_as<NS>((glb_double*)cx.glb + glb_level_offset<NS, W, PL>(cx, j, v), x);
}
template <int NS, int W = 1, int PL = 0>
__device__ __forceinline__ void levelN_store(const PairCtx& cx, int j, int v, const double (&x)[NS]) {
    using L = PairLds<NS, W, PL>;
    int nl = cx.nlds;
    asm volatile("" : "+s"(nl));
    if (j <= nl) vstore_as<NS>((lds_double*)cx.lds + (L::kL2 + (j - 2) * 4 * L::DP + v * L::DP), x);
    else vstore_as<NS>((glb_double*)cx.glb + glb_level_offset<NS, W, PL>(cx, j, v), x);
}
template <int NS, int W = 1, int PL = 0>
__device__ __forceinline__ void level_load_lp(const PairCtx& cx, int j, double (&x)[NS]) {
    if (j == 1) vload_as<NS>((lds_double*)cx.lds + PairLds<NS, W, PL>::kL1, x); else levelN_load<NS, W, PL>(cx, j, 0, x);
}
template <int NS, int W = 1, int PL = 0>
__device__ __forceinline__ void level_load_q(const PairCtx& cx, int j, double (&x)[NS]) {
    if (j == 1) vload_as<NS>((lds_double*)cx.lds + (PairLds<NS, W, PL>::kL1 + 2 * PairLds<NS, W, PL>::DP), x); else levelN_load<NS, W, PL>(cx, j, 3, x);
}
template <int NS, int W = 1, int PL = 0>
__device__ __forceinline__ void level_scal_put(const PairCtx& cx, int j, double w, double a, double pe, double plogp) {
    if (lane_id() == 0) {
        lds_double* s = (lds_double*)cx.lds + (PairLds<NS, W, PL>::kScal + 4 * j) + (W > 1 ? cx.wave_scal : 0);
        s[0] = w; s[1] = a; s[2] = pe; s[3] = plogp;
    }
}
template <int NS, int W = 1, int PL = 0>
__device__ __forceinline__ void level_scal_get_wa(const PairCtx& cx, int j, double& w, double& a) {
    const lds_double* s = (const lds_double*)cx.lds + (PairLds<NS, W, PL>::kScal + 4 * j) + (W > 1 ? cx.wave_scal : 0);
    w = s[0]; a = s[1];
}
template <int NS, int W = 1, int PL = 0>
__device__ __forceinline__ void level_scal_park(const PairCtx& cx, int j, double w, double a, int src, int elane, double en, double lp) {
    lds_double* s = (lds_double*)cx.lds + (PairLds<NS, W, PL>::kScal + 4 * j) + (W > 1 ? cx.wave_scal : 0);
    const int lane = lane_id();
    if (src < 0) {
        if (lane == elane) { s[2] = en; s[3] = lp; }
    } else {
        const lds_double* f = (const lds_double*)cx.lds + (PairLds<NS, W, PL>::kScal + 4 * src) + (W > 1 ? cx.wave_scal : 0);
        const double pe = f[2], pl = f[3];
        if (lane == 0) { s[2] = pe; s[3] = pl; }
    }
    if (lane == 0) { s[0] = w; s[1] = a; }
}
template <int NS, int W = 1, int PL = 0>
__device__ __forceinline__ void level_scal_get(const PairCtx& cx, int j, double& w, double& a, double& pe, double& plogp) {
    const lds_double* s = (const lds_double*)cx.lds + (PairLds<NS, W, PL>::kScal + 4 * j) + (W > 1 ? cx.wave_scal : 0);
    w = s[0]; a = s[1]; pe = s[2]; plogp = s[3];
}

template <int NS, class Target, class TeamT>
__device__ __forceinline__ void leapfrog_partial(TeamT& tm, const Target& tgt, const double (&var)[NS], double eps,
                                                 double (&q)[NS], double (&p)[NS], double (&g)[NS], double (&v)[NS],
                                                 double& kin_part, double& lp_part) {
    const double dt = 0.5 * eps;
#pragma unroll
    for (int s = 0; s < NS; ++s) {
        p[s] = p[s] + dt * g[s];
        const double vh = var[s] * p[s];
        q[s] = q[s] + eps * vh;
    }
    if constexpr (Target::kLanePartial) {
        lp_part = tgt.logp_grad_partial(tm, q, g);
    } else {
        const double lp = first_f64(tgt.logp_grad(tm, q, g));
        lp_part = (tm.tid() == 0) ? lp : 0.0;
    }
    double kin = 0.0;
#pragma unroll
    for (int s = 0; s < NS; ++s) {
        p[s] = p[s] + dt * g[s];
        v[s] = var[s] * p[s];
        kin = __builtin_fma(p[s], v[s], kin);
    }
    kin_part = kin;
}

template <int NS, int W = 1, int PL = 0>
__device__ __forceinline__ double cascade_dots(PairCtx& cx, const double (&var)[NS], const double (&alp)[NS],
                                               const double (&arp)[NS], const double (&aps)[NS], const double (&tl)[NS],
                                               double (&tps)[NS], const double (&v)[NS]) {
    double d0 = 0.0, d1 = 0.0, d2 = 0.0, d3 = 0.0, d4 = 0.0, d5 = 0.0;
#pragma unroll
    for (int s = 0; s < NS; ++s) {
        const double p1 = aps[s] + tl[s];
        const double p2 = arp[s] + tps[s];
        const double ps = aps[s] + tps[s];
        const double valp = var[s] * alp[s], vtlp = var[s] * tl[s], varp = var[s] * arp[s];
        d0 = __builtin_fma(ps, valp, d0); d1 = __builtin_fma(ps, v[s], d1);
        d2 = __builtin_fma(p1, valp, d2); d3 = __builtin_fma(p1, vtlp, d3);
        d4 = __builtin_fma(p2, varp, d4); d5 = __builtin_fma(p2, v[s], d5);
        tps[s] = ps;
    }
    red_put<NS, W, PL>(cx, 0, d0); red_put<NS, W, PL>(cx, 1, d1); red_put<NS, W, PL>(cx, 2, d2);
    red_put<NS, W, PL>(cx, 3, d3); red_put<NS, W, PL>(cx, 4, d4); red_put<NS, W, PL>(cx, 5, d5);
    return red_gather<NS, W, PL>(cx);
}

template <int NS, int PL, class Target, class TeamT>
__device__ inline void nuts_transition2(TeamT& tm, const Target& tgt, const double (&var)[NS], RngState& rng,
                                        PairCtx& cx, double* qrow, const double (&q)[NS],
                                        const double (&p0)[NS], const double (&g0)[NS], double e0, double logp0,
                                        double step_size, double emax, int max_depth, bool momentum_f32,
                                        TransitionOut& out) {
    constexpr int W = TeamT::kWaves;
    double cq[NS], cp[NS], cg[NS];
    vcopy(cq, q); vcopy(cp, p0); vcopy(cg, g0);
    cold_store<NS, W, PL, kColdOq>(cx, q); cold_store<NS, W, PL, kColdOp>(cx, p0); cold_store<NS, W, PL, kColdOg>(cx, g0);
    cold_store<NS, W, PL, kColdPsum>(cx, p0);
    bool c_right = true;
    bool c_start = momentum_f32, o_start = momentum_f32;
    double prop_e = e0, prop_logp = logp0;
    double coff = 0.0;
    lds_double* tot = (lds_double*)cx.lds + PairLds<NS, W, PL>::kScal + (W > 1 ? cx.wave_scal : 0);
    if (lane_id() == 0) { tot[0] = 0.0; tot[1] = 0.0; tot[2] = 1.0; tot[3] = 0.0; }
    int depth = 0, n_leap = 0;
    bool diverging = false, turning = false, exhausted = true;
    const bool odd_lane = (lane_id() & 1) != 0;
    UniformWindow win;
    window_reset(win);

    double mde = 0.0;
    const bool lane15 = lane_id() == 15, lane31 = lane_id() == 31;
    auto mde_combined = [&]() -> double {
        const double a = readlane_f64(mde, 15), b = readlane_f64(mde, 31);
        return (fabs(b) > fabs(a)) ? b : a;
    };
    auto leaf_scalars = [&](double s, int n, double& en, double& ev) -> int {
        const ExpLanesConst ec = exp_lanes_const();
        en = 0.5 * dpp_f64<0x118>(s) - s;
        double de = en - e0;
        int ok = 0;
        const bool leaf_lane = lane15 | (lane31 & (n == 2));
        const unsigned long long leaf_bits = (n == 2) ? ((1ull << 15) | (1ull << 31)) : (1ull << 15);
        const unsigned long long rare = ballot64(!(fabs(de) < emax)) | ballot64((-de) - coff > 600.0);
        bool examined = leaf_lane;
        double de_x = de;
        if ((rare & leaf_bits) == 0ull) {
            n_leap += n;
            ok = n;
        } else {
            int seen = 0;
            for (int i = 0; i < n; ++i) {
                double dei = readlane_f64(de, 15 + 16 * i);
                ++n_leap; ++seen;
                if (isnan(dei)) dei = __builtin_inf();
                if (!(fabs(dei) < emax)) { diverging = true; break; }
                const double x = -dei;
                if (x - coff > 600.0) {
                    const double f = exp_uniform(coff - x);
                    const int lane = lane_id();
                    if (lane >= 1 && lane < kLevelScalDoubles / 4) {
                        lds_double* sc = (lds_double*)cx.lds + (PairLds<NS, W, PL>::kScal + 4 * lane) + (W > 1 ? cx.wave_scal : 0);
                        sc[0] = sc[0] * f; sc[1] = sc[1] * f;
                    }
                    coff = x;
                }
                ++ok;
            }
            de_x = isnan(de) ? __builtin_inf() : de;
            examined = lane15 | (lane31 & (seen == 2));
        }
        const bool upd = (fabs(de_x) > fabs(mde)) & examined;
        mde = upd ? de_x : mde;
        const double x = -de;
        const double xn = dpp_f64<0x101>(x);
        const double arg = odd_lane ? (x - coff) : ((xn - coff) + fmin(xn, 0.0));
        ev = exp_lanes<NS, W, PL>(cx, ec, arg);
        return ok;
    };

    for (int dd = 0; dd < max_depth; ++dd) {
        const bool right = team_uniform(tm, rng, win) < 0.5;
        const double eps = right ? step_size : -step_size;
        if (right != c_right) {
            double t[NS];
            cold_load<NS, W, PL, kColdOq>(cx, t); cold_store<NS, W, PL, kColdOq>(cx, cq); vcopy(cq, t);
            cold_load<NS, W, PL, kColdOp>(cx, t); cold_store<NS, W, PL, kColdOp>(cx, cp); vcopy(cp, t);
            cold_load<NS, W, PL, kColdOg>(cx, t); cold_store<NS, W, PL, kColdOg>(cx, cg); vcopy(cg, t);
            const bool tb = c_start; c_start = o_start; o_start = tb;
            c_right = right;
        }
        cold_store<NS, W, PL, kColdAold>(cx, cp);
        const bool aold_start = c_start;

        double tps[NS], eq[NS], ep[NS];
        double tw = 0.0, ta = 0.0;
        int qsrc = -1;
        int elane = 15;
        double en_last = 0.0, lp_last = 0.0;
        const int D = depth;
        if (D == 0) {
            double v[NS], kinp, lp, en, ev;
            leapfrog_partial<NS>(tm, tgt, var, eps, cq, cp, cg, v, kinp, lp);
            red_put<NS, W, PL>(cx, 0, kinp); red_put<NS, W, PL>(cx, 1, lp);
            const double s0 = red_gather<NS, W, PL>(cx);
            if (leaf_scalars(s0, 1, en, ev) == 1) {
                tw = readlane_f64(ev, 15); ta = readlane_f64(ev, 14);
                en_last = en; lp_last = s0;
                vcopy(tps, cp);
            }
        } else {
            const int n_pairs = 1 << (D - 1);
            for (int k = 0; k < n_pairs; ++k) {
                double v[NS], kinA, lpA, kinB, lpB;
                leapfrog_partial<NS>(tm, tgt, var, eps, cq, cp, cg, v, kinA, lpA);
                red_put<NS, W, PL>(cx, 0, kinA); red_put<NS, W, PL>(cx, 1, lpA);
                vcopy(eq, cq); vcopy(ep, cp);
                leapfrog_partial<NS>(tm, tgt, var, eps, cq, cp, cg, v, kinB, lpB);
                red_put<NS, W, PL>(cx, 2, kinB); red_put<NS, W, PL>(cx, 3, lpB);
#pragma unroll
                for (int s = 0; s < NS; ++s) tps[s] = ep[s] + cp[s];
                red_put<NS, W, PL>(cx, 4, pdot_v<NS>(tps, var, ep));
                red_put<NS, W, PL>(cx, 5, pdot<NS>(tps, v));
                const double s0 = red_gather<NS, W, PL>(cx);
                const int m = __builtin_ctz(~static_cast<unsigned>(k) | (1u << (D - 1)));
                double en, ev;
                if (leaf_scalars(s0, 2, en, ev) != 2) break;
                {
                    const double wA = readlane_f64(ev, 15), aA = readlane_f64(ev, 14);
                    const double wB = readlane_f64(ev, 31), aB = readlane_f64(ev, 30);
                    const bool turn = red_any_nonpositive(s0, 4, 2);
                    const double wsum = wA + wB;
                    const bool take_b = uniform_true(team_uniform(tm, rng, win) * wsum < wB);
                    qsrc = take_b ? -1 : -2;
                    elane = take_b ? 31 : 15;
                    en_last = en; lp_last = s0;
                    tw = wsum; ta = aA + aB;
                    if (turn) { turning = true; break; }
                }
                if (m >= 1) {
                    double alp[NS], arp[NS], aps[NS];
                    double aw, aa;
                    level1_load<NS, W, PL>(cx, alp, arp, aps);
                    level_scal_get_wa<NS, W, PL>(cx, 1, aw, aa);
                    const double sj = cascade_dots<NS, W, PL>(cx, var, alp, arp, aps, ep, tps, v);
                    const bool turn = red_any_nonpositive(sj, 0, 6);
                    const double wsum = aw + tw;
                    const bool take_b = uniform_true(team_uniform(tm, rng, win) * wsum < tw);
                    if (!take_b) qsrc = 1;
                    tw = wsum; ta = aa + ta;
                    if (turn) { turning = true; break; }
                }
                for (int j = 2; j <= m; ++j) {
                    double blp[NS], brp[NS], bps[NS], tl[NS];
                    levelN_load<NS, W, PL>(cx, j, 0, blp); levelN_load<NS, W, PL>(cx, j, 1, brp); levelN_load<NS, W, PL>(cx, j, 2, bps);
                    level_load_lp<NS, W, PL>(cx, j - 1, tl);
                    double bw, ba;
                    level_scal_get_wa<NS, W, PL>(cx, j, bw, ba);
                    const double sj = cascade_dots<NS, W, PL>(cx, var, blp, brp, bps, tl, tps, v);
                    const bool turn = red_any_nonpositive(sj, 0, 6);
                    const double wsum = bw + tw;
                    const bool take_b = uniform_true(team_uniform(tm, rng, win) * wsum < tw);
                    if (!take_b) qsrc = j;
                    tw = wsum; ta = ba + ta;
                    if (turn) { turning = true; break; }
                }
                if (turning) break;
                if (k + 1 < n_pairs) {
                    double tl[NS], tqv[NS];
                    if (m == 0) vcopy(tl, ep); else level_load_lp<NS, W, PL>(cx, m, tl);
                    if (qsrc == -1) vcopy(tqv, cq);
                    else if (qsrc == -2) vcopy(tqv, eq);
                    else level_load_q<NS, W, PL>(cx, qsrc, tqv);
#ifndef LMC_PARK_REORDER_MIN_NS
#define LMC_PARK_REORDER_MIN_NS 4
#endif
                    constexpr bool kParkReorder = NS >= LMC_PARK_REORDER_MIN_NS;
                    if constexpr (kParkReorder) level_scal_park<NS, W, PL>(cx, m + 1, tw, ta, qsrc, elane, en_last, lp_last);
                    if (m == 0) {
                        level1_store<NS, W, PL>(cx, tl, cp, tqv);
                    } else {
                        if constexpr (kParkReorder) {
#pragma unroll
                            for (int s = 0; s < NS; ++s) asm volatile("" : "+v"(tl[s]), "+v"(tqv[s]));
                        }
                        levelN_store<NS, W, PL>(cx, m + 1, 0, tl); levelN_store<NS, W, PL>(cx, m + 1, 1, cp);
                        levelN_store<NS, W, PL>(cx, m + 1, 2, tps); levelN_store<NS, W, PL>(cx, m + 1, 3, tqv);
                    }
                    if constexpr (!kParkReorder) level_scal_park<NS, W, PL>(cx, m + 1, tw, ta, qsrc, elane, en_last, lp_last);
                }
            }
        }
        ++depth;
        if (diverging || turning) { exhausted = false; break; }

        double wn = tot[0], an = tot[1], w_start = tot[2];
        const double c_tot = tot[3];
        if (uniform_true(c_tot != coff)) {
            const double f = exp_uniform(first_f64(c_tot) - coff);
            wn = wn * f; an = an * f; w_start = w_start * f;
            if (lane_id() == 0) { tot[2] = w_start; tot[3] = coff; }
        }
        if (uniform_true(team_uniform(tm, rng, win) * (w_start + wn) < tw)) {
            double tqv[NS];
            if (qsrc == -1) vcopy(tqv, cq);
            else if (qsrc == -2) vcopy(tqv, eq);
            else level_load_q<NS, W, PL>(cx, qsrc, tqv);
            vstore_as<NS>((glb_double*)qrow, tqv);
            if (qsrc < 0) {
                prop_e = readlane_f64(en_last, elane); prop_logp = readlane_f64(lp_last, elane);
            } else {
                double w_, a_;
                level_scal_get<NS, W, PL>(cx, qsrc, w_, a_, prop_e, prop_logp);
                prop_e = first_f64(prop_e); prop_logp = first_f64(prop_logp);
            }
        }
        if (lane_id() == 0) { tot[0] = wn + tw; tot[1] = an + ta; }
        double tlp[NS], psum[NS], op[NS], aold[NS];
        if (D == 0) vcopy(tlp, cp);
        else if (D == 1) vcopy(tlp, ep);
        else level_load_lp<NS, W, PL>(cx, D - 1, tlp);
        cold_load<NS, W, PL, kColdPsum>(cx, psum); cold_load<NS, W, PL, kColdOp>(cx, op); cold_load<NS, W, PL, kColdAold>(cx, aold);
#pragma unroll
        for (int s = 0; s < NS; ++s) {
            const double t = psum[s] + tps[s];
            psum[s] = momentum_f32 ? static_cast<double>(static_cast<float>(t)) : t;
        }
        cold_store<NS, W, PL, kColdPsum>(cx, psum);
        double ov[NS], av[NS];
        end_velocity<NS>(ov, var, op, o_start);
        end_velocity<NS>(av, var, aold, aold_start);
        double d0 = 0.0, d1 = 0.0, d2 = 0.0, d3 = 0.0, d4 = 0.0, d5 = 0.0;
        if (right) {
#pragma unroll
            for (int s = 0; s < NS; ++s) {
                const double vtl = var[s] * tlp[s], vtr = var[s] * cp[s];
                const double p1 = psum[s] + tlp[s], p2 = aold[s] + tps[s];
                d0 = __builtin_fma(psum[s], ov[s], d0); d1 = __builtin_fma(psum[s], vtr, d1);
                d2 = __builtin_fma(p1, ov[s], d2);      d3 = __builtin_fma(p1, vtl, d3);
                d4 = __builtin_fma(p2, av[s], d4);      d5 = __builtin_fma(p2, vtr, d5);
            }
        } else {
#pragma unroll
            for (int s = 0; s < NS; ++s) {
                const double vtl = var[s] * tlp[s], vtr = var[s] * cp[s];
                const double p1 = tps[s] + aold[s], p2 = tlp[s] + psum[s];
                d0 = __builtin_fma(psum[s], vtr, d0);   d1 = __builtin_fma(psum[s], ov[s], d1);
                d2 = __builtin_fma(p1, vtr, d2);        d3 = __builtin_fma(p1, av[s], d3);
                d4 = __builtin_fma(p2, vtl, d4);        d5 = __builtin_fma(p2, ov[s], d5);
            }
        }
        c_start = false;
        red_put<NS, W, PL>(cx, 0, d0); red_put<NS, W, PL>(cx, 1, d1); red_put<NS, W, PL>(cx, 2, d2);
        red_put<NS, W, PL>(cx, 3, d3); red_put<NS, W, PL>(cx, 4, d4); red_put<NS, W, PL>(cx, 5, d5);
        if (red_any_nonpositive(red_gather<NS, W, PL>(cx), 0, 6)) { turning = true; exhausted = false; break; }
    }

    const double wn_end = first_f64(tot[0]), an_end = first_f64(tot[1]);
    const double mean_accept = (wn_end > 0.0) ? first_f64(an_end / wn_end) : 0.0;
    out.accept = mean_accept;
    out.energy = prop_e;
    out.energy_error = first_f64(prop_e - e0);
    out.max_energy_error = mde_combined();
    out.model_logp = prop_logp;
    out.depth = depth;
    out.n_leapfrog = n_leap;
    out.diverging = diverging;
    out.exhausted = exhausted;
    out.accepted = 0;
}

#ifndef LMC_NORMALS_IN_REGS
#define LMC_NORMALS_IN_REGS 1
#endif
#ifndef LMC_WAVES_NS1
#define LMC_WAVES_NS1 4
#endif
#ifndef LMC_WAVES_NS2
#define LMC_WAVES_NS2 3
#endif
#ifndef LMC_WAVES_NS4
#define LMC_WAVES_NS4 2
#endif
#ifndef LMC_WAVES_NS2_W8
#define LMC_WAVES_NS2_W8 4
#endif
constexpr int run_waves_per_simd(int ns, int w = 1) {
    return (ns == 2 && w == 8) ? LMC_WAVES_NS2_W8 : ns <= 1 ? LMC_WAVES_NS1 : ns == 2 ? LMC_WAVES_NS2 : ns == 4 ? LMC_WAVES_NS4 : 1;
}
constexpr int kLdsMtDoubles = 320;
#ifndef LMC_MT_IN_LDS_W1
#define LMC_MT_IN_LDS_W1 1
#endif
constexpr bool run_mt_in_lds(int w) { return w > 1 || LMC_MT_IN_LDS_W1; }
constexpr int lds_tail_doubles(int w) {
    return w == 1 ? (run_mt_in_lds(1) ? kLdsMtDoubles : 0) : kLdsMtDoubles + 2 * w * kTeamSlots + 4 + (w >= 4 ? kLdsMtDoubles : 0);
}
constexpr int kPlanUp = 24, kPlanDown = 14;

template <class CA, class PT>
__device__ __forceinline__ int stop_request_load(const CA& A, const PT& P, int chain_in_launch, int it, long long git, long long leaps = -1) {
    int* dev = A.stop_dev;
    const int mask = P.relay_mask;
    const bool relay = (it == 0) ? ((chain_in_launch & mask) == 0)
                                 : ((git & 15) == 0 && ((chain_in_launch + static_cast<int>(git >> 4)) & mask) == 0);
    if (relay) {
        if (__hip_atomic_load(A.stop, __ATOMIC_RELAXED, __HIP_MEMORY_SCOPE_SYSTEM) != 0)
            __hip_atomic_store(dev, 1, __ATOMIC_RELAXED, __HIP_MEMORY_SCOPE_AGENT);
        __hip_atomic_store(A.progress, static_cast<int>(git), __ATOMIC_RELAXED, __HIP_MEMORY_SCOPE_SYSTEM);
        if (leaps >= 0 && it >= 8 && A.tree_hint != nullptr) {
            int mean = static_cast<int>(static_cast<float>(leaps) / static_cast<float>(it));
            mean = mean < 1 ? 1 : (mean > 4095 ? 4095 : mean);
            const int at = git > 0x7ffff ? 0x7ffff : static_cast<int>(git);
            __hip_atomic_store(A.tree_hint, (at << 12) | mean, __ATOMIC_RELAXED, __HIP_MEMORY_SCOPE_SYSTEM);
        }
    }
    return __hip_atomic_load(dev, __ATOMIC_RELAXED, __HIP_MEMORY_SCOPE_AGENT);
}
template <class TeamT>
__device__ __forceinline__ bool stop_requested(TeamT& tm, int loaded, double* bcast) {
    if constexpr (TeamT::kWaves == 1) {
        return first_i32(loaded) != 0;
    } else {
        tm.sync();
        if (tm.tid() == 0) bcast[3] = static_cast<double>(loaded);
        tm.sync();
        return first_f64(bcast[3]) != 0.0;
    }
}
template <int W>
__device__ __forceinline__ bool stop_at_entry(const int* stop_dev, int* word) {
    const int s = __hip_atomic_load(const_cast<int*>(stop_dev), __ATOMIC_RELAXED, __HIP_MEMORY_SCOPE_AGENT);
    if constexpr (W == 1) {
        return first_i32(s) != 0;
    } else {
        if (threadIdx.x == 0) *word = s;
        __syncthreads();
        const int agreed = *word;
// ... 77 lines not shown
    const double ints = __hiloint2double(static_cast<int>(flags), out.n_leapfrog);
    return (tid == 7) ? ints : v;
}
template <int NS, class CA>
__device__ __forceinline__ void store_outputs(const CA& A, int c, int tid, long long git, const double (&q)[NS], double rec) {
    const int d = A.d;
    const long long orow = static_cast<long long>(c) * A.cap + git;
    if (A.trace != nullptr && git >= A.trace_begin) {
        double* tr = A.trace + (static_cast<long long>(c) * (A.cap - A.trace_begin) + (git - A.trace_begin)) * d;
#pragma unroll
        for (int s = 0; s < NS; ++s) {
            const int e = tid * NS + s;
            if (e < d) tr[e] = q[s];
        }
    }
    if (tid < 8) reinterpret_cast<double*>(A.stat_rec + orow)[tid] = rec;
}
template <int NS, class CA>
__device__ __forceinline__ void write_outputs(const CA& A, int c, int tid, long long git, const double (&q)[NS],
                                              const TransitionOut& out, double step_now, double step_bar_now, bool tune) {
    store_outputs<NS>(A, c, tid, git, q, stat_record_value(tid, out, step_now, step_bar_now, tune));
}

struct MassScalars { double wsum_f, wsum_b; int wsel, n_samples, window; };
template <int NS, class CA>
__device__ __forceinline__ void diag_mass_prefetch(const CA& A, long long row, const MassScalars& ms,
                                                   double (&m)[NS], double (&r)[NS], double (&mb)[NS], double (&rb)[NS]) {
    const long long plane = static_cast<long long>(A.chains) * A.dpad;
    vload<NS>(A.wmean + ms.wsel * plane + row, m); vload<NS>(A.wraw + ms.wsel * plane + row, r);
    vload<NS>(A.wmean + (1 - ms.wsel) * plane + row, mb); vload<NS>(A.wraw + (1 - ms.wsel) * plane + row, rb);
}
template <int NS, class CA, class PT>
__device__ __forceinline__ void diag_mass_update(const CA& A, const PT& P, long long row, int tid,
                                                 const double (&q)[NS], float (&var)[NS], float (&inv_std)[NS],
                                                 double (&vard)[NS], MassScalars& ms,
                                                 double (&m)[NS], double (&r)[NS], double (&mb)[NS], double (&rb)[NS]) {
    const int d = A.d;
    const long long plane = static_cast<long long>(A.chains) * A.dpad;
    double* fm = A.wmean + ms.wsel * plane + row;
    double* fr = A.wraw + ms.wsel * plane + row;
    double* bm = A.wmean + (1 - ms.wsel) * plane + row;
    double* br = A.wraw + (1 - ms.wsel) * plane + row;
    ms.wsum_f += 1.0;
    ms.wsum_b += 1.0;
    const double prop_f = first_f64(1.0 / ms.wsum_f), prop_b = first_f64(1.0 / ms.wsum_b);
#pragma unroll
    for (int s = 0; s < NS; ++s) {
        const double od = q[s] - m[s];
        m[s] = m[s] + prop_f * od;
        const double nd = q[s] - m[s];
        r[s] = r[s] + 1.0 * od * nd;
        const int e = tid * NS + s;
        if (e < d) {
            var[s] = static_cast<float>(r[s] / ms.wsum_f);
            const float sd = sqrtf(var[s]);
            inv_std[s] = 1.0f / sd;
            vard[s] = static_cast<double>(var[s]);
        }
    }
    vstore<NS>(fm, m); vstore<NS>(fr, r);
#pragma unroll
    for (int s = 0; s < NS; ++s) {
        const double od = q[s] - mb[s];
        mb[s] = mb[s] + prop_b * od;
        const double nd = q[s] - mb[s];
        rb[s] = rb[s] + 1.0 * od * nd;
        m[s] = mb[s]; r[s] = rb[s];
    }
    if (ms.n_samples > 0 && ms.n_samples % ms.window == 0) {
        vstore<NS>(bm, m); vstore<NS>(br, r);
#pragma unroll
        for (int s = 0; s < NS; ++s) { m[s] = 0.0; r[s] = 0.0; }
        vstore<NS>(fm, m); vstore<NS>(fr, r);
        ms.wsum_f = ms.wsum_b;
        ms.wsum_b = 0.0;
        ms.wsel = 1 - ms.wsel;
        ms.window = static_cast<int>(static_cast<double>(ms.window) * P.window_multiplier);
    } else {
        vstore<NS>(bm, m); vstore<NS>(br, r);
    }
    ++ms.n_samples;
}

template <int NS, int W, template <int> class TargetT, int RNG = 0, int PL = 0>
__global__ __launch_bounds__(64 * W, run_waves_per_simd(NS, W)) void run_kernel(ChainArrays, SamplerParams, const double* tparams) {
    extern __shared__ __attribute__((aligned(16))) double lds[];
    const long long t_resident = wall_clock64();
    const KernArgs ka = KernArgs::get();
    KChainArrays& A0 = ka.A();
    KSamplerParams& P0 = ka.P();
    const int c = blockIdx.x + P0.chain_begin;
    const int d = A0.d, dpad = A0.dpad;
    const long long row = static_cast<long long>(c) * dpad;
    const int lds_doubles = P0.lds_doubles;
    Team<W> tm;
    tm.xbuf = lds + lds_doubles + kLdsMtDoubles;
    tm.parity = 0;
    double* rng_bcast = tm.xbuf + 2 * W * kTeamSlots;
    const int tid = tm.tid();

    if (stop_at_entry<W>(A0.stop_dev, reinterpret_cast<int*>(lds))) return;
    if (A0.status[c] & kStatusBadInitialEnergy) return;

    TargetT<NS> tgt;
    tgt.init(tm, tparams, d);

    double q[NS];
    float var[NS], inv_std[NS];
    double vard[NS];
    double* const qrow = A0.q + row;
    vload<NS>(qrow, q);
#pragma unroll
    for (int s = 0; s < NS; ++s) {
        var[s] = A0.var[row + tid * NS + s];
        inv_std[s] = A0.inv_std[row + tid * NS + s];
        vard[s] = static_cast<double>(var[s]);
    }
    RngState rng;
    uint32_t* mt_glb = A0.mt + static_cast<long long>(c) * kMtN;
    uint32_t* mt_lds = reinterpret_cast<uint32_t*>(lds + lds_doubles);
    uint32_t* mt_lds2 = reinterpret_cast<uint32_t*>(rng_bcast + 4);
    constexpr bool kMtInLds = run_mt_in_lds(W) && PL == 0;
    if constexpr (kMtInLds) {
        for (int i = tid; i < kMtN; i += 64 * W) mt_lds[i] = mt_glb[i];
        tm.sync();
        rng.mt = mt_lds;
    } else {
        rng.mt = mt_glb;
    }
    rng.pos = first_i32(A0.rng_pos[c]);
    rng.has_gauss = first_i32(A0.rng_has_gauss[c]);
    rng.gauss = first_f64(A0.rng_gauss[c]);
    const uint32_t chain_seed = RNG == 1 ? first_u32(A0.seed[c]) : 0u;
    DualAverage da;
    dual_average_load(A0, c, da);
    int iter_count = first_i32(A0.iter_count[c]);
    MassScalars ms;
    ms.n_samples = first_i32(A0.n_samples[c]);
    ms.wsel = first_i32(A0.wsel[c]);
    ms.wsum_f = first_f64(A0.wsum[c * 2 + ms.wsel]);
    ms.wsum_b = first_f64(A0.wsum[c * 2 + (1 - ms.wsel)]);
    ms.window = first_i32(A0.awindow[c]);
    long long ct_maxdepth = 0, ct_divs = 0, ct_after = 0, ct_leap = 0;
    int status = 0;

    static_assert(NS <= 4, "sampling kernels hold at most four elements per lane");
    PairCtx cx;
    cx.lds = lds;
    cx.glb = A0.scratch + static_cast<long long>(c) * A0.scratch_stride;
    cx.nlds = P0.nlds;
    cx.wave = tm.wave();
    cx.wave_red = W > 1 ? cx.wave * PairLds<NS, W>::kRedWave : 0;
    cx.wave_scal = W > 1 ? cx.wave * kLevelScalDoubles : 0;
    cx.red_lane = static_cast<int>(reinterpret_cast<size_t>((lds_double*)lds + (red_lane_init() + cx.wave_red)));
    cx.xpar = 0;
    if (tid < kExpTableDoubles) lds[PairLds<NS, W>::kExp + tid] = kExp2Table[2 * tid];
    tm.sync();

#ifdef LMC_PHASE_TIMING
    unsigned long long ph[6] = {0, 0, 0, 0, 0, 0};
    unsigned long long ph_t = clock64();
#define LMC_PHASE(i) { const unsigned long long now_ = clock64(); ph[i] += now_ - ph_t; ph_t = now_; }
#else
#define LMC_PHASE(i)
#endif
    const int n_iters = P0.n_iters;
    for (int it = 0; it < n_iters; ++it) {
        KSamplerParams& P = ka.P();
        const long long git = P.iter_begin + it;
        const bool tune = git < P.n_tune;
        const bool momentum_f32 = P.momentum_f32 != 0;
        LMC_PHASE(5)
        const int stop_word = stop_request_load(ka.A(), P, static_cast<int>(blockIdx.x), it, git, P.kind == 0 ? ct_leap : -1);

        double p0[NS];
        if constexpr (RNG == 1) {
            double z[NS];
            philox_normals<NS>(chain_seed, git, tid, d, z);
#pragma unroll
            for (int s = 0; s < NS; ++s)
                p0[s] = momentum_f32 ? static_cast<double>(inv_std[s] * static_cast<float>(z[s])) : z[s] * static_cast<double>(inv_std[s]);
        } else {
            double zr[NS];
            if constexpr (W == 1 && LMC_NORMALS_IN_REGS) {
                rng_normals_owned<NS>(rng, d, lds, lds + dpad, zr);
            } else {
                team_normals(tm, rng, d, lds, lds + dpad, rng_bcast, mt_lds, mt_lds2);
#pragma unroll
                for (int s = 0; s < NS; ++s) {
                    const int e = tid * NS + s;
                    zr[s] = (e < d) ? lds[e] : 0.0;
                }
                tm.sync();
            }
#pragma unroll
            for (int s = 0; s < NS; ++s)
                p0[s] = momentum_f32 ? static_cast<double>(inv_std[s] * static_cast<float>(zr[s]))
                                     : zr[s] * static_cast<double>(inv_std[s]);
        }
        LMC_PHASE(0)

        double g0[NS];
        const double logp0 = first_f64(tgt.logp_grad(tm, q, g0));
        double e0;
        if (momentum_f32) {
            const float kin = start_kinetic_f32<NS>(tm, p0, var, d, P.sdot_mode, reinterpret_cast<float*>(lds), dpad);
            e0 = first_f64(static_cast<double>(kin) - logp0);
        } else {
            e0 = first_f64(0.5 * tm.sum(pdot_v<NS>(p0, vard, p0)) - logp0);
        }
        if (!isfinite(e0)) {
            status |= kStatusBadInitialEnergy;
            break;
        }

        const bool adapt_step = tune && P.adapt_step_size;
        const double step_size = jitter_step_size(tm, rng, ka.A(), P, c, adapt_step ? da.step_now : da.step_bar_now);

        LMC_PHASE(1)
        TransitionOut out;
        if (P.kind == 0) {
            const int md = (tune && iter_count < 200) ? P.early_max_treedepth : P.max_treedepth;
            nuts_transition2<NS, PL>(tm, tgt, vard, rng, cx, qrow, q, p0, g0, e0, logp0, step_size, P.emax, md,
                                 momentum_f32, out);
            vload<NS>(qrow, q);
            if (out.exhausted && !tune) ++ct_maxdepth;
        } else {
            hmc_transition<NS>(tm, tgt, vard, rng, q, p0, g0, e0, logp0, step_size, P.emax, P.path_length,
                               P.max_steps, out);
        }
        ct_leap += out.n_leapfrog;
        LMC_PHASE(2)

        KChainArrays& A = ka.A();
        KSamplerParams& P2 = ka.P();
        if (adapt_step) dual_average_update(A, P2, out.accept, da);
        LMC_PHASE(3)

#ifndef LMC_EARLY_STOP_CHECK
#define LMC_EARLY_STOP_CHECK 1
#endif
        double rec_value = 0.0;
        bool stop_now = false;
        if constexpr (LMC_EARLY_STOP_CHECK != 0) {
            rec_value = stat_record_value(tid, out, da.step_now, da.step_bar_now, tune);
            int sw = stop_word;
            asm volatile("" : "+v"(rec_value), "+v"(sw));
            stop_now = stop_requested(tm, sw, rng_bcast);
        }

        if (tune && P2.adapt_mass) {
            double wm[NS], wr[NS], wmb[NS], wrb[NS];
            diag_mass_prefetch<NS>(A, row, ms, wm, wr, wmb, wrb);
            diag_mass_update<NS>(A, P2, row, tid, q, var, inv_std, vard, ms, wm, wr, wmb, wrb);
        }

        LMC_PHASE(4)
        if (out.diverging && !tune) ++ct_divs;
        ++iter_count;
        if (!tune) ++ct_after;

        if (A.mom_mean != nullptr && !tune) moments_update<NS>(A, tm, c, row, q);
        if constexpr (LMC_EARLY_STOP_CHECK != 0) {
            store_outputs<NS>(A, c, tid, git, q, rec_value);
            if (stop_now) break;
        } else {
            write_outputs<NS>(A, c, tid, git, q, out, da.step_now, da.step_bar_now, tune);
            if (stop_requested(tm, stop_word, rng_bcast)) break;
        }
    }

    KChainArrays& A = ka.A();
    tm.sync();
    if constexpr (kMtInLds) {
        for (int i = tid; i < kMtN; i += 64 * W) mt_glb[i] = rng.mt[i];
    }
    vstore<NS>(qrow, q);
#pragma unroll
    for (int s = 0; s < NS; ++s) {
        A.var[row + tid * NS + s] = var[s];
        A.inv_std[row + tid * NS + s] = inv_std[s];
    }
    if (tid == 0) {
        A.rng_pos[c] = rng.pos;
        A.rng_has_gauss[c] = rng.has_gauss;
        A.rng_gauss[c] = rng.gauss;
        A.da[c * 4 + 0] = da.log_step;
        A.da[c * 4 + 1] = da.log_bar;
        A.da[c * 4 + 2] = da.hbar;
        A.da_count[c] = da.count;
        A.iter_count[c] = iter_count;
        A.n_samples[c] = ms.n_samples;
        A.wsel[c] = ms.wsel;
        A.awindow[c] = ms.window;
        A.wsum[c * 2 + ms.wsel] = ms.wsum_f;
        A.wsum[c * 2 + (1 - ms.wsel)] = ms.wsum_b;
        A.status[c] |= status;
        A.counters[c * kNumCounters + kCtMaxTreedepth] += ct_maxdepth;
        A.counters[c * kNumCounters + kCtDivsSample] += ct_divs;
        A.counters[c * kNumCounters + kCtSamplesAfterTune] += ct_after;
        A.counters[c * kNumCounters + kCtLeapfrogs] += ct_leap;
        A.counters[c * kNumCounters + kCtWaveTicks] += static_cast<long long>(W) * (wall_clock64() - t_resident);
#ifdef LMC_PHASE_TIMING
        LMC_PHASE(5)
        A.counters[c * kNumCounters + 0] += static_cast<long long>(((ph[0] & 0xffffffffull) << 32) | (ph[1] & 0xffffffffull)) - ct_maxdepth;
        A.counters[c * kNumCounters + 1] += static_cast<long long>(((ph[2] & 0xffffffffull) << 32) | (ph[3] & 0xffffffffull)) - ct_divs;
// ... 7 lines not shown
```

littlemcmc_amd/csrc/lmc_wave.hpp:

```cpp
#pragma once
#include <hip/hip_runtime.h>
#include <stdint.h>

namespace lmc {

constexpr int kWave = 64;

__device__ __forceinline__ int lane_id() { return static_cast<int>(threadIdx.x) & 63; }
#ifndef LMC_CHAIN_THREAD
#define LMC_CHAIN_THREAD static_cast<int>(threadIdx.x)
#endif
__device__ __forceinline__ unsigned long long ballot64(bool pred) { return __builtin_amdgcn_ballot_w64(pred); }

__device__ __forceinline__ double readlane_f64(double x, int lane) {
    const int lo = __builtin_amdgcn_readlane(__double2loint(x), lane);
    const int hi = __builtin_amdgcn_readlane(__double2hiint(x), lane);
    return __hiloint2double(hi, lo);
}
__device__ __forceinline__ double first_f64(double x) {
    const int lo = __builtin_amdgcn_readfirstlane(__double2loint(x));
    const int hi = __builtin_amdgcn_readfirstlane(__double2hiint(x));
    return __hiloint2double(hi, lo);
}
__device__ __forceinline__ int first_i32(int x) { return __builtin_amdgcn_readfirstlane(x); }
__device__ __forceinline__ uint32_t first_u32(uint32_t x) {
    return static_cast<uint32_t>(__builtin_amdgcn_readfirstlane(static_cast<int>(x)));
}

template <int CTRL>
__device__ __forceinline__ double dpp_f64(double x) {
    const int lo = __builtin_amdgcn_mov_dpp(__double2loint(x), CTRL, 0xf, 0xf, true);
    const int hi = __builtin_amdgcn_mov_dpp(__double2hiint(x), CTRL, 0xf, 0xf, true);
    return __hiloint2double(hi, lo);
}

template <int CTRL>
__device__ __forceinline__ float dpp_f32(float x) {
    return __builtin_bit_cast(float, __builtin_amdgcn_mov_dpp(__builtin_bit_cast(int, x), CTRL, 0xf, 0xf, true));
}
__device__ __forceinline__ float readlane_f32(float x, int lane) {
    return __builtin_bit_cast(float, __builtin_amdgcn_readlane(__builtin_bit_cast(int, x), lane));
}

__device__ __forceinline__ double wave_sum(double x) {
    x += dpp_f64<0x111>(x);
    x += dpp_f64<0x112>(x);
    x += dpp_f64<0x114>(x);
    x += dpp_f64<0x118>(x);
    x += dpp_f64<0x142>(x);
    x += dpp_f64<0x143>(x);
    return readlane_f64(x, 63);
}

__device__ __forceinline__ double swap32_add(double a, double b) {
    const auto lo = __builtin_amdgcn_permlane32_swap(static_cast<unsigned>(__double2loint(a)),
                                                     static_cast<unsigned>(__double2loint(b)), false, false);
    const auto hi = __builtin_amdgcn_permlane32_swap(static_cast<unsigned>(__double2hiint(a)),
                                                     static_cast<unsigned>(__double2hiint(b)), false, false);
    return __hiloint2double(static_cast<int>(hi[0]), static_cast<int>(lo[0])) +
           __hiloint2double(static_cast<int>(hi[1]), static_cast<int>(lo[1]));
}
__device__ __forceinline__ double swap16_add(double a, double b) {
    const auto lo = __builtin_amdgcn_permlane16_swap(static_cast<unsigned>(__double2loint(a)),
                                                     static_cast<unsigned>(__double2loint(b)), false, false);
    const auto hi = __builtin_amdgcn_permlane16_swap(static_cast<unsigned>(__double2hiint(a)),
                                                     static_cast<unsigned>(__double2hiint(b)), false, false);
    return __hiloint2double(static_cast<int>(hi[0]), static_cast<int>(lo[0])) +
           __hiloint2double(static_cast<int>(hi[1]), static_cast<int>(lo[1]));
}
__device__ __forceinline__ double row_scan(double x) {
    x += dpp_f64<0x111>(x);
    x += dpp_f64<0x112>(x);
    x += dpp_f64<0x114>(x);
    x += dpp_f64<0x118>(x);
    return x;
}

__device__ __forceinline__ void wave_sum2(double& a, double& b) {
    double x = swap32_add(a, b);
    x = row_scan(x);
    x += dpp_f64<0x142>(x);
    a = readlane_f64(x, 31);
    b = readlane_f64(x, 63);
}

__device__ __forceinline__ bool any_sum_nonpositive2(double d0, double d1) {
    double x = swap32_add(d0, d1);
    x = row_scan(x);
    x += dpp_f64<0x142>(x);
    const unsigned long long m = ballot64(x <= 0.0);
    return (m & ((1ull << 31) | (1ull << 63))) != 0ull;
}
__device__ __forceinline__ bool any_sum_nonpositive6(const double (&d)[6]) {
    const double x01 = swap32_add(d[0], d[1]);
    const double x23 = swap32_add(d[2], d[3]);
    const double x45 = swap32_add(d[4], d[5]);
    double y = swap16_add(x01, x23);
    double z = swap16_add(x45, 0.0);
    y = row_scan(y);
    z = row_scan(z);
    const unsigned long long my = ballot64(y <= 0.0);
    const unsigned long long mz = ballot64(z <= 0.0);
    const unsigned long long rows = (1ull << 15) | (1ull << 31) | (1ull << 47) | (1ull << 63);
    return ((my & rows) | (mz & ((1ull << 15) | (1ull << 47)))) != 0ull;
}

template <unsigned long long BITS>
__device__ __forceinline__ double sgpr_const() {
    unsigned lo, hi;
    asm("s_mov_b32 %0, %1" : "=s"(lo) : "i"(static_cast<unsigned>(BITS & 0xffffffffull)));
    asm("s_mov_b32 %0, %1" : "=s"(hi) : "i"(static_cast<unsigned>(BITS >> 32)));
    return __hiloint2double(static_cast<int>(hi), static_cast<int>(lo));
}
#define LMC_SC(x) (::lmc::sgpr_const<__builtin_bit_cast(unsigned long long, static_cast<double>(x))>())

__device__ __forceinline__ double fma_sgpr_addend(double p, double r, double c) {
    double out;
    asm("v_fma_f64 %0, %1, %2, %3" : "=v"(out) : "v"(p), "v"(r), "s"(c));
    return out;
}

__device__ __forceinline__ double exp_uniform(double x) {
    double xv = fmin(fmax(x, -800.0), 800.0);
    asm volatile("" : "+v"(xv));
    const double kf = rint(xv * LMC_SC(1.4426950408889634074));
    double r = __builtin_fma(-kf, LMC_SC(6.93147180369123816490e-01), xv);
    r = __builtin_fma(-kf, LMC_SC(1.90821492927058770002e-10), r);
    double p = fma_sgpr_addend(r, LMC_SC(1.0 / 6227020800.0), LMC_SC(1.0 / 479001600.0));
    p = fma_sgpr_addend(p, r, LMC_SC(1.0 / 39916800.0));
    p = fma_sgpr_addend(p, r, LMC_SC(1.0 / 3628800.0));
    p = fma_sgpr_addend(p, r, LMC_SC(1.0 / 362880.0));
    p = fma_sgpr_addend(p, r, LMC_SC(1.0 / 40320.0));
    p = fma_sgpr_addend(p, r, LMC_SC(1.0 / 5040.0));
    p = fma_sgpr_addend(p, r, LMC_SC(1.0 / 720.0));
    p = fma_sgpr_addend(p, r, LMC_SC(1.0 / 120.0));
    p = fma_sgpr_addend(p, r, LMC_SC(1.0 / 24.0));
    p = fma_sgpr_addend(p, r, LMC_SC(1.0 / 6.0));
    p = __builtin_fma(p, r, 0.5);
    p = __builtin_fma(p, r, 1.0);
    p = __builtin_fma(p, r, 1.0);
    return first_f64(ldexp(p, static_cast<int>(kf)));
}

// ... 47 lines not shown
```

littlemcmc_amd/engine.py:

```python
import ctypes as C

import numpy as np

from . import _abi

DEFAULT_SDOT = "auto"


class _TickView:

    def __init__(self, ptr, shape):
        self.__cuda_array_interface__ = {"shape": tuple(shape), "typestr": "<f8", "data": (int(ptr), False), "version": 2}


class _PinnedBlock:

    def __init__(self, lib, raw, base, span, shape, dtype):
        self._lib, self._raw, self._base, self._span, self._registered = lib, raw, int(base), int(span), False
        self.__array_interface__ = {"data": (self._base, False), "shape": tuple(int(x) for x in shape),
                                    "typestr": np.dtype(dtype).str, "version": 3}

    def register(self):
        if not self._registered:
            if self._lib.lmc_host_register(C.c_void_p(self._base), self._span) != _abi.OK:
# ... 20 lines not shown
    share = -(-nbytes // threads // (1 << 21)) * (1 << 21)
    if threads == 1:
        C.memset(address, 0, nbytes)
        return
    work = [threading.Thread(target=C.memset, args=(address + o, 0, min(share, nbytes - o))) for o in range(0, nbytes, share)]
    for t in work:
        t.start()
    for t in work:
        t.join()


def pinned_empty(shape, dtype, lib=None, threads=None, register=True):
    lib = lib or _abi.load()
    dtype = np.dtype(dtype)
    nbytes = int(np.prod(shape, dtype=np.int64)) * dtype.itemsize
    if nbytes == 0:
        return np.empty(shape, dtype=dtype)
    if threads is None:
        import os

        threads = min(16, len(os.sched_getaffinity(0)) if hasattr(os, "sched_getaffinity") else (os.cpu_count() or 1))
    import mmap

    page = mmap.PAGESIZE
    span = -(-nbytes // page) * page
    raw = np.empty(span + page, dtype=np.uint8)
    base = raw.ctypes.data + (-raw.ctypes.data) % page
    _prefault(base, span, threads)
    block = _PinnedBlock(lib, raw, base, span, shape, dtype)
    if register:
        block.register()
    return np.asarray(block)


def pinned_register(array):
    owner = array
    while owner is not None and not isinstance(owner, _PinnedBlock):
        owner = getattr(owner, "base", None)
    if owner is not None:
        owner.register()


class StreamedResults:

    def __init__(self, chains, n_out, first, dim, planes, keep_trace=True, pinned=True, lib=None, copy_workgroups=0, direct=False,
                 register=True):
        self.direct = bool(direct)
        self.copy_workgroups = int(copy_workgroups)
        self.chains, self.n_out, self.first, self.dim = int(chains), int(n_out), int(first), int(dim)
        self.planes = list(planes)
        assert len(self.planes) <= _abi.MAX_PLANES
        alloc = (lambda sh, dt: pinned_empty(sh, dt, lib, register=register)) if pinned else (lambda sh, dt: np.empty(sh, dtype=dt))
        self.registered = bool(register) or not pinned
        self.pinned = bool(pinned)
        self.trace = alloc((self.chains, self.n_out, self.dim), np.float64) if keep_trace else None
        self.stats = {name: alloc((self.chains, self.n_out), dt) for name, _k, _i, _a, dt in self.planes}

    def register(self):
        if not self.registered:
            for a in ([] if self.trace is None else [self.trace]) + list(self.stats.values()):
                pinned_register(a)
            self.registered = True

    def window_dst(self, eng, chain_lo=0):
        w = _abi.WindowDst()
        w.n_out, w.first = self.n_out, self.first
        w.trace = None if (self.trace is None or self.direct) else self.trace[chain_lo:].ctypes.data
        w.n_planes = len(self.planes)
        w.copy_workgroups = self.copy_workgroups
        for p, (name, kind, idx, as_, _dt) in enumerate(self.planes):
            w.plane[p].dst = self.stats[name][chain_lo:].ctypes.data
            w.plane[p].kind, w.plane[p].idx, w.plane[p].as_ = int(kind), int(idx), int(as_)
        return w


_TUNING_ENV = {
    "LMC_SUB_BLOCKS": ("sub_blocks", int),
    "LMC_FORCE_WIDE": ("force_general", lambda v: int(int(v) != 0)),
    "LMC_WIDE_TEAM": ("general_team", int),
    "LMC_DENSE_COOP": ("dense_coop_off", lambda v: int(int(v) == 0)),
    "LMC_DENSE_CACHE_ROWS": ("dense_cache_rows_p1", lambda v: int(v) + 1),
    "LMC_DENSE_LDS_SLOTS": ("dense_lds_slots_p1", lambda v: int(v) + 1),
    "LMC_CHOL_HBM": ("chol_hbm", lambda v: int(int(v) != 0)),
}


def tuning_from_env(environ=None):
    import os

    environ = os.environ if environ is None else environ
    out = {}
    for name, (field, conv) in _TUNING_ENV.items():
        raw = environ.get(name, "")
        if raw != "":
            try:
                out[field] = conv(raw)
            except ValueError:
                pass
    shape = environ.get("LMC_RUN_SHAPE", "")
    if shape:
        try:
            a, b = (int(x) for x in shape.split(","))
            out["run_ns"], out["run_w"] = a, b
        except ValueError:
            pass
    return out


def hw_queue_cap(environ=None):
    import os

    environ = os.environ if environ is None else environ
    try:
        n = int(environ.get("GPU_MAX_HW_QUEUES", ""))
    except ValueError:
        return None
    return n if 1 <= n < 4 else None


class Engine:
    def __init__(self, target, chains, kind="nuts", potential="diag_adapt", device=0, lib_path=None,
                 target_accept=0.8, Emax=1000.0, adapt_step_size=True, step_scale=0.25, gamma=0.05, k=0.75,
                 t0=10, path_length=2.0, max_treedepth=10, early_max_treedepth=8, max_steps=1024,
                 adaptation_window=101, adaptation_window_multiplier=1.0, lds_levels=0, sdot=None, rng="numpy",
                 mass_dtype="float32", lds_plan="auto", tuning=None):
        self._lib = _abi.load(lib_path or getattr(target, "lib_path", None))
        self._h = C.c_void_p()
        self.target = target
        self.chains = int(chains)
        self.dim = int(target.d)
        self.kind = kind
        cfg = _abi.Config()
        self._lib.lmc_config_defaults(C.byref(cfg), self.chains, self.dim)
        cfg.device = int(device)
        cfg.kind = {"nuts": _abi.KIND_NUTS, "hmc": _abi.KIND_HMC}[kind]
        cfg.target_family = int(target.family)
        cfg.potential = {"diag_adapt": _abi.POT_DIAG_ADAPT, "diag": _abi.POT_DIAG, "full": _abi.POT_FULL,
                         "full_inv": _abi.POT_FULL_INV, "full_adapt": _abi.POT_FULL_ADAPT, "full_f64": _abi.POT_FULL_F64}[potential]
        self.potential = potential
        cfg.adapt_step_size = int(bool(adapt_step_size))
        cfg.target_accept = float(target_accept)
        cfg.emax = float(Emax)
        cfg.step_scale = float(step_scale)
        cfg.gamma = float(gamma)
        cfg.k = float(k)
        cfg.t0 = float(t0)
        cfg.max_treedepth = int(max_treedepth)
        cfg.early_max_treedepth = int(early_max_treedepth)
        cfg.path_length = float(path_length)
        cfg.max_steps = int(max_steps)
        cfg.adaptation_window = int(adaptation_window)
        cfg.adaptation_window_multiplier = float(adaptation_window_multiplier)
        cfg.lds_levels = int(lds_levels)
        if lds_plan in ("auto", None):
            import os

            lds_plan = {"0": 0, "1": 1}.get(os.environ.get("LMC_LDS_PLAN", ""), "auto")
        cfg.lds_plan = {"auto": _abi.LDS_PLAN_AUTO, None: _abi.LDS_PLAN_AUTO, 0: _abi.LDS_PLAN_SHALLOW, "shallow": _abi.LDS_PLAN_SHALLOW,
                        1: _abi.LDS_PLAN_DEEP, "deep": _abi.LDS_PLAN_DEEP}[lds_plan]
        for field, value in (tuning_from_env() if tuning is None else dict(tuning)).items():
            setattr(cfg.tuning, field, int(value))
        if cfg.tuning.sub_blocks == 0 and hw_queue_cap() is not None:
            cfg.tuning.sub_blocks = -hw_queue_cap()
        cfg.rng_mode = {"numpy": _abi.RNG_NUMPY, "philox": _abi.RNG_PHILOX}[rng]
        self.mass_f64 = np.dtype(mass_dtype) == np.float64 and potential in ("diag_adapt", "diag", "full_adapt")
        cfg.mass_f64 = int(self.mass_f64)
# ... 78 lines not shown
                                                       int(state[3]), float(state[4])))

    def get_rng_state(self, chain):
        key = np.zeros(624, dtype=np.uint32)
        pos, hg, g = C.c_int32(), C.c_int32(), C.c_double()
        self._check(self._lib.lmc_engine_get_rng_state(self._h, int(chain), _abi.ptr(key), C.byref(pos),
                                                       C.byref(hg), C.byref(g)))
        return ("MT19937", key, int(pos.value), int(hg.value), float(g.value))

    def set_position(self, q):
        q = np.ascontiguousarray(q, dtype=np.float64)
        self._check(self._lib.lmc_engine_set_position(self._h, _abi.ptr(q), int(q.ndim == 2)))

    def get_position(self):
        q = np.empty((self.chains, self.dim))
        self._check(self._lib.lmc_engine_get_position(self._h, _abi.ptr(q)))
        return q

    def reset_tuning(self):
        self._check(self._lib.lmc_engine_reset_tuning(self._h))

    def set_dual_average(self, log_step, log_bar, hbar=0.0, count=1):
        self._check(self._lib.lmc_engine_set_dual_average(self._h, float(log_step), float(log_bar), float(hbar),
                                                          int(count)))

    def reserve(self, capacity, keep_trace=True, trace_begin=0):
        tb = int(trace_begin) if keep_trace else -1
        self._check(self._lib.lmc_engine_reserve(self._h, int(capacity), tb))
        self.capacity = int(capacity)
        self.keep_trace = bool(keep_trace) and tb < capacity
        self.trace_begin = max(tb, 0)
        self._trace_out = None

    def attach_trace(self, out, trace_begin):
        if out is not None:
            assert out.shape == (self.chains, self.capacity - int(trace_begin), self.dim) and out.dtype == np.float64 and out.flags["C_CONTIGUOUS"]
        self._check(self._lib.lmc_engine_attach_trace(self._h, None if out is None else C.c_void_p(out.ctypes.data), int(trace_begin)))
        self._trace_out = out
        self.keep_trace, self.trace_begin = True, int(trace_begin)

    def run(self, n_tune, iter_begin, n_iters):
        if self.target.family == _abi.TARGET_EXTERNAL:
            return self._run_ticks(int(n_tune), int(iter_begin), int(n_iters))
        self._check(self._lib.lmc_engine_run(self._h, int(n_tune), int(iter_begin), int(n_iters)))

    def set_step_jitter(self, lo, hi, enable=True):
        self._check(self._lib.lmc_engine_set_step_jitter(self._h, int(bool(enable)), float(lo), float(hi)))

    def set_step_sizes(self, step_sizes):
        if step_sizes is None:
            self._check(self._lib.lmc_engine_set_step_sizes(self._h, None))
            return
        a = np.ascontiguousarray(np.broadcast_to(np.asarray(step_sizes, dtype=np.float64), (self.chains,)))
        self._check(self._lib.lmc_engine_set_step_sizes(self._h, _abi.ptr(a)))

    def diag_update(self, tune=True):
        self._check(self._lib.lmc_engine_diag_update(self._h, int(bool(tune))))

    def request_stop(self, stop=True):
        self._check(self._lib.lmc_engine_request_stop(self._h, int(bool(stop))))

    def progress(self):
        return int(self._lib.lmc_engine_progress(self._h))

    def completed_iterations(self):
        return int(self.get_chain_state(fields=("iter_count",))["iter_count"].min())

    def occupancy(self):
        rc, wpc, hz = C.c_int32(), C.c_int32(), C.c_double()
        self._check(self._lib.lmc_engine_occupancy(self._h, C.byref(rc), C.byref(wpc), C.byref(hz)))
        return int(rc.value), int(wpc.value), float(hz.value)

    def run_lds_bytes(self):
        n = int(self._lib.lmc_engine_run_lds_bytes(self._h))
        return n if n >= 0 else None

    def resident_chains(self):
        if self.target.family == _abi.TARGET_EXTERNAL:
            return None
        return self.occupancy()[0] or None

    def last_run_plan(self):
        return {_abi.LDS_PLAN_SHALLOW: "shallow", _abi.LDS_PLAN_DEEP: "deep"}.get(int(self._lib.lmc_engine_last_run_plan(self._h)))

    def run_streams(self):
        arr = (C.c_void_p * _abi.MAX_RUN_STREAMS)()
        n = min(self._lib.lmc_engine_run_streams(self._h, arr, _abi.MAX_RUN_STREAMS), _abi.MAX_RUN_STREAMS)
        if n < 0:
            self._check(n)
        return [int(arr[i] or 0) for i in range(n)]

    def tick_begin(self, n_tune, iter_begin, n_iters):
        self._check(self._lib.lmc_engine_tick_begin(self._h, int(n_tune), int(iter_begin), int(n_iters)))

    def tick_positions_ptr(self):
        return int(self._lib.lmc_engine_tick_positions(self._h) or 0)

    def tick(self, logp_ptr, grad_ptr, wait=True):
        n = C.c_int32(-1)
        self._check(self._lib.lmc_engine_tick(self._h, C.c_void_p(int(logp_ptr)), C.c_void_p(int(grad_ptr)),
                                              C.byref(n) if wait else None))
        return int(n.value) if wait else None

    def _run_ticks(self, n_tune, iter_begin, n_iters, poll=32):
        import torch

        if n_iters == 0:
            return
        dev = torch.device("cuda", int(self.cfg.device))
        if getattr(self, "_tick_stream", None) is None:
            self._tick_stream = torch.cuda.Stream(device=dev)
        self.synchronize()
        self.set_stream(self._tick_stream.cuda_stream)
        try:
            with torch.cuda.device(dev), torch.cuda.stream(self._tick_stream):
                self.tick_begin(n_tune, iter_begin, n_iters)
                q = torch.as_tensor(_TickView(self.tick_positions_ptr(), (self.chains, self.dim)), device=dev)
                graph = None
                if getattr(self.target, "graph", False):
                    graph = getattr(self, "_tick_graph", None)
                    if graph is None:
                        for _ in range(3):
                            self.target.evaluate(q)
                        self._tick_stream.synchronize()
                        g = torch.cuda.CUDAGraph()
                        with torch.cuda.graph(g, stream=self._tick_stream):
                            out = self.target.evaluate(q)
                        graph = self._tick_graph = (g, out)
                ticks = 0
                while True:
                    if graph is not None:
                        graph[0].replay()
                        logp, grad = graph[1]
                    else:
                        logp, grad = self.target.evaluate(q)
                    ticks += 1
                    active = self.tick(logp.data_ptr(), grad.data_ptr(),
                                       wait=(ticks % getattr(self.target, "tick_poll", poll) == 0))
                    self._tick_keep = (logp, grad)
                    if active == 0:
                        break
                self._tick_stream.synchronize()
                self.ticks = getattr(self, "ticks", 0) + ticks
        finally:
            self.set_stream(None)

    def trace(self, iter_begin=None, n_iters=None):
        iter_begin = self.trace_begin if iter_begin is None else iter_begin
        n = self.capacity - iter_begin if n_iters is None else n_iters
        out = np.empty((self.chains, n, self.dim))
        self._check(self._lib.lmc_engine_get_trace(self._h, _abi.ptr(out), int(iter_begin), int(n)))
        return out

    def stat_f64(self, stat, iter_begin=0, n_iters=None):
        n = self.capacity - iter_begin if n_iters is None else n_iters
        out = np.empty((self.chains, n))
        self._check(self._lib.lmc_engine_get_stat_f64(self._h, int(stat), _abi.ptr(out), int(iter_begin), int(n)))
        return out

    def stat_i32(self, stat, iter_begin=0, n_iters=None):
        n = self.capacity - iter_begin if n_iters is None else n_iters
        out = np.empty((self.chains, n), dtype=np.int32)
        self._check(self._lib.lmc_engine_get_stat_i32(self._h, int(stat), _abi.ptr(out), int(iter_begin), int(n)))
        return out

    def stat_u8(self, stat, iter_begin=0, n_iters=None):
# ... 330 lines not shown
```

Before: 3.061 billion.

## Build NUTS trees in leaf quads for one-wave small-dim kernels

Adds a leaf-group template parameter so that one-wave kernels with small per-lane state (ns<=2) handle four leapfrog leaves per tree step instead of two. It uses a smaller LDS staging area, 8-row reductions and a permlane32 helper to merge the checks of the two halves. The goal is fewer LDS round trips and reductions per leaf, and a smaller LDS footprint that may allow deeper LDS-resident trees. It is on by default for eligible shapes, can be overridden back to pairs through a tuning field, and adds extra kernel instantiations plus considerable complexity in tree bookkeeping.

Measured after the change: 3.350 billion, median of 6. 9.4% higher.

```diff
diff --git a/include/lmc_hip.h b/include/lmc_hip.h
--- a/include/lmc_hip.h
+++ b/include/lmc_hip.h
@@ -79,7 +79,8 @@
     int32_t dense_cache_rows_p1;
     int32_t dense_lds_slots_p1;
     int32_t chol_hbm;
-    int32_t reserved[3];
+    int32_t leaf_group;
+    int32_t reserved[2];
 } lmc_tuning;
 
 typedef struct lmc_config {
@@ -158,6 +159,7 @@
 #define LMC_MAX_RUN_STREAMS 8
 int lmc_engine_run_streams(lmc_engine* e, void** streams, int32_t capacity);
 int32_t lmc_engine_last_run_plan(lmc_engine* e);
+int32_t lmc_engine_last_run_leaf_group(lmc_engine* e);
 
 int lmc_engine_get_trace(lmc_engine* e, double* dst, int64_t iter_begin, int64_t n_iters);
 int lmc_engine_get_stat_f64(lmc_engine* e, int32_t stat, double* dst, int64_t iter_begin, int64_t n_iters);
diff --git a/littlemcmc_amd/_abi.py b/littlemcmc_amd/_abi.py
--- a/littlemcmc_amd/_abi.py
+++ b/littlemcmc_amd/_abi.py
@@ -33,7 +33,8 @@
 
     _fields_ = [("sub_blocks", C.c_int32), ("force_general", C.c_int32), ("general_team", C.c_int32), ("run_ns", C.c_int32),
                 ("run_w", C.c_int32), ("dense_coop_off", C.c_int32), ("dense_cache_rows_p1", C.c_int32),
-                ("dense_lds_slots_p1", C.c_int32), ("chol_hbm", C.c_int32), ("reserved", C.c_int32 * 3)]
+                ("dense_lds_slots_p1", C.c_int32), ("chol_hbm", C.c_int32), ("leaf_group", C.c_int32),
+                ("reserved", C.c_int32 * 2)]
 
 
 class Config(C.Structure):
@@ -122,6 +123,7 @@
     "lmc_engine_run": (C.c_int, [_P, C.c_int64, C.c_int64, C.c_int32]),
     "lmc_engine_run_streams": (C.c_int, [_P, _P, C.c_int32]),
     "lmc_engine_last_run_plan": (C.c_int32, [_P]),
+    "lmc_engine_last_run_leaf_group": (C.c_int32, [_P]),
     "lmc_engine_copy_window_async": (C.c_int, [_P, C.POINTER(WindowDst), C.c_int64, C.c_int64]),
     "lmc_engine_copy_wait": (C.c_int, [_P]),
     "lmc_host_alloc": (_P, [C.c_uint64]),
diff --git a/littlemcmc_amd/csrc/lmc_engine.hip b/littlemcmc_amd/csrc/lmc_engine.hip
--- a/littlemcmc_amd/csrc/lmc_engine.hip
+++ b/littlemcmc_amd/csrc/lmc_engine.hip
@@ -282,6 +282,7 @@
     int lds_plan_wanted = 0;
     int plan_now = 0;
     int plan_last = -1;
+    int leaf_group = 2;
     bool wide = false;
     double* init_diag64 = nullptr;
     int run_ns = 0, run_w = 1;
@@ -675,8 +676,10 @@
     if (cfg->chains < 1 || cfg->dim < 1) return fail(nullptr, LMC_ERR_INVALID, "chains and dim must be >= 1");
     if (cfg->lds_plan < LMC_LDS_PLAN_AUTO || cfg->lds_plan > LMC_LDS_PLAN_DEEP)
         return fail(nullptr, LMC_ERR_INVALID, "unknown lds_plan %d", cfg->lds_plan);
-    if (cfg->reserved0 != 0 || cfg->tuning.reserved[0] != 0 || cfg->tuning.reserved[1] != 0 || cfg->tuning.reserved[2] != 0)
+    if (cfg->reserved0 != 0 || cfg->tuning.reserved[0] != 0 || cfg->tuning.reserved[1] != 0)
         return fail(nullptr, LMC_ERR_INVALID, "reserved fields of lmc_config must be 0");
+    if (cfg->tuning.leaf_group != 0 && cfg->tuning.leaf_group != 2 && cfg->tuning.leaf_group != 4)
+        return fail(nullptr, LMC_ERR_INVALID, "unknown leaf_group %d (0, 2 or 4)", cfg->tuning.leaf_group);
     if (cfg->potential < LMC_POT_DIAG_ADAPT || cfg->potential > LMC_POT_FULL_F64)
         return fail(nullptr, LMC_ERR_INVALID, "unknown potential %d", cfg->potential);
     if (cfg->mass_f64 && cfg->potential > LMC_POT_DIAG && cfg->potential != LMC_POT_FULL_ADAPT)
@@ -782,6 +785,10 @@
     const int max_levels = (cfg->max_treedepth > cfg->early_max_treedepth ? cfg->max_treedepth
                                                                           : cfg->early_max_treedepth);
     int nlds = 1;
+    e->leaf_group = (!wide && run_leaf_group(e->run_ns, e->run_w) == 4 && cfg->tuning.leaf_group != 2) ? 4 : 2;
+    if ((cfg->target_family == LMC_TARGET_USER && !kUserCompiledIn) || cfg->rng_mode == LMC_RNG_PHILOX)
+        e->leaf_group = run_leaf_group(e->run_ns, e->run_w);
+    const int lg = e->leaf_group;
     if (wide) {
         e->nlds = 1;
         e->lds_bytes = wide_lds_bytes(e->dpad);
@@ -789,24 +796,24 @@
         const int waves_per_cu = 4 * run_waves_per_simd(e->run_ns, e->run_w);
         const int blocks_per_cu = waves_per_cu / e->run_w > 0 ? waves_per_cu / e->run_w : 1;
         const long budget = (163840L / blocks_per_cu) / 1280 * 1280 - lds_tail_doubles(e->run_w) * 8L;
-        if (pair_min_doubles(e->run_ns, e->run_w) * 8L > budget)
+        if (pair_min_doubles(e->run_ns, e->run_w, 0, lg) * 8L > budget)
             return bail(fail(nullptr, LMC_ERR_INVALID, "the sampling kernel's LDS plan does not fit the budget"));
         nlds = cfg->lds_levels > 0 ? cfg->lds_levels : 1;
         if (cfg->lds_levels <= 0)
-            while (nlds < max_levels && pair_total_doubles(e->run_ns, e->run_w, nlds + 1) * 8L <= budget) ++nlds;
+            while (nlds < max_levels && pair_total_doubles(e->run_ns, e->run_w, nlds + 1, 0, lg) * 8L <= budget) ++nlds;
         if (nlds > max_levels) nlds = max_levels;
         if (nlds < 1) nlds = 1;
         e->nlds = nlds;
-        e->lds_bytes = pair_total_doubles(e->run_ns, e->run_w, nlds) * 8;
+        e->lds_bytes = pair_total_doubles(e->run_ns, e->run_w, nlds, 0, lg) * 8;
         e->nlds1 = nlds;
         e->lds_bytes1 = 0;
         e->lds_plan = 0;
         const long budget1 = (163840L / blocks_per_cu) / 1280 * 1280;
-        if (e->run_w == 1 && run_mt_in_lds(1) && cfg->lds_levels <= 0 && pair_min_doubles(e->run_ns, 1, 1) * 8L <= budget1) {
+        if (e->run_w == 1 && run_mt_in_lds(1) && cfg->lds_levels <= 0 && pair_min_doubles(e->run_ns, 1, 1, lg) * 8L <= budget1) {
             int n1 = 1;
-            while (n1 < max_levels && pair_total_doubles(e->run_ns, 1, n1 + 1, 1) * 8L <= budget1) ++n1;
+            while (n1 < max_levels && pair_total_doubles(e->run_ns, 1, n1 + 1, 1, lg) * 8L <= budget1) ++n1;
             e->nlds1 = n1;
-            e->lds_bytes1 = pair_total_doubles(e->run_ns, 1, n1, 1) * 8;
+            e->lds_bytes1 = pair_total_doubles(e->run_ns, 1, n1, 1, lg) * 8;
             e->lds_plan = cfg->lds_plan == LMC_LDS_PLAN_SHALLOW ? 0 : cfg->lds_plan == LMC_LDS_PLAN_DEEP ? 1 : 2;
             if (e->nlds1 <= e->nlds) e->lds_plan = 0;
             if (cfg->rng_mode == LMC_RNG_PHILOX) e->lds_plan = 0;
@@ -1049,6 +1056,9 @@
                                                hipFuncAttributeMaxDynamicSharedMemorySize, run_lds));          \
             HIP_TRY(e, hipOccupancyMaxActiveBlocksPerMultiprocessor(&per_cu, run_kernel<NSV, WV, T, 1>, block, \
                                                                     static_cast<size_t>(run_lds)));            \
+        } else if (e->leaf_group != run_leaf_group(NSV, WV)) {                                                 \
+            HIP_TRY(e, hipOccupancyMaxActiveBlocksPerMultiprocessor(&per_cu, run_kernel<NSV, WV, T, 0, 0, 2>,  \
+                                                                    block, static_cast<size_t>(run_lds)));     \
         } else {                                                                                               \
             if (run_lds > 64 * 1024)                                                                           \
                 HIP_TRY(e, hipFuncSetAttribute(reinterpret_cast<const void*>(&run_kernel<NSV, WV, T>),         \
@@ -1076,6 +1086,10 @@
     return sampling_lds_bytes(e, e->plan_last >= 0 ? e->plan_last : e->plan_now);
 }
 
+int32_t lmc_engine_last_run_leaf_group(lmc_engine* e) {
+    if (!e || e->plan_last < 0 || e->cfg.kind != LMC_KIND_NUTS || e->wide || e->cfg.potential >= LMC_POT_FULL || e->cfg.target_family == LMC_TARGET_EXTERNAL) return 0;
+    return e->leaf_group;
+}
 int32_t lmc_engine_last_run_plan(lmc_engine* e) {
     if (!e || e->plan_last < 0 || e->wide || e->cfg.potential >= LMC_POT_FULL || e->cfg.target_family == LMC_TARGET_EXTERNAL) return 0;
     return e->plan_last == 1 ? LMC_LDS_PLAN_DEEP : LMC_LDS_PLAN_SHALLOW;
@@ -1868,7 +1882,10 @@
     HIP_TRY(e, order_sub_blocks_after_main(e));
 #define RUN_PLAN1(NSV, WV, T)                                                                                  \
     if constexpr (WV == 1) {                                                                                   \
-        LMC_LAUNCH((run_kernel<NSV, 1, T, 0, 1>), grid, block, run_lds, st, e->A, P, e->tparams);              \
+        if (e->leaf_group != run_leaf_group(NSV, 1))                                                           \
+            LMC_LAUNCH((run_kernel<NSV, 1, T, 0, 1, 2>), grid, block, run_lds, st, e->A, P, e->tparams);       \
+        else                                                                                                   \
+            LMC_LAUNCH((run_kernel<NSV, 1, T, 0, 1>), grid, block, run_lds, st, e->A, P, e->tparams);          \
     }
 #define RUN_ONE(NSV, WV, T)                                                                                    \
     if (!found && e->run_ns == NSV && e->run_w == WV) {                                                        \
@@ -1880,6 +1897,9 @@
             LMC_LAUNCH((run_kernel<NSV, WV, T, 1>), grid, block, run_lds, st, e->A, P, e->tparams);            \
         } else if (plan == 1) {                                                                                \
             RUN_PLAN1(NSV, WV, T)                                                                              \
+        } else if (e->leaf_group != run_leaf_group(NSV, WV)) {                                                 \
+            if constexpr (WV == 1)                   \
+                LMC_LAUNCH((run_kernel<NSV, 1, T, 0, 0, 2>), grid, block, run_lds, st, e->A, P, e->tparams);   \
         } else {                                                                                               \
             if (run_lds > 64 * 1024)                                                                           \
                 HIP_TRY(e, hipFuncSetAttribute(reinterpret_cast<const void*>(&run_kernel<NSV, WV, T>),         \
diff --git a/littlemcmc_amd/csrc/lmc_sampler.hpp b/littlemcmc_amd/csrc/lmc_sampler.hpp
--- a/littlemcmc_amd/csrc/lmc_sampler.hpp
+++ b/littlemcmc_amd/csrc/lmc_sampler.hpp
@@ -552,10 +552,13 @@
 enum ColdSlot : int { kColdAold = 0, kColdPsum = 1, kColdOp = 2, kColdOq = 3, kColdOg = 4, kNumCold = 5 };
 constexpr int kNumColdSlots = kNumCold;
 
-template <int NS, int W = 1, int PL = 0>
+constexpr int run_leaf_group(int ns, int w) { return (w == 1 && ns <= 2) ? 4 : 2; }
+template <int NS, int W = 1, int PL = 0, int G = 2>
 struct PairLds {
+    static_assert(G == 2 || (G == 4 && W == 1), "leaf quads exist for the one-wave kernels");
     static constexpr int DP = 64 * NS * W;
-    static constexpr int kRedWave = 64 * kRedValues;
+    static constexpr int kRedRows = G == 4 ? 8 : kRedValues;
+    static constexpr int kRedWave = 64 * kRedRows;
     static constexpr int kRedSize = (2 * DP > W * kRedWave) ? 2 * DP : W * kRedWave;
     static constexpr int kExp = kRedSize;
     static constexpr int kXsum = kExp + kExpTableDoubles;
@@ -565,8 +568,9 @@
     static_assert(PL == 0 || W == 1, "the deep-tree plan exists for one-wave kernels");
     static constexpr int kColdLds = PL == 1 ? (NS >= 4 ? 0 : (LMC_PAIR_COLD_LDS < 1 ? LMC_PAIR_COLD_LDS : 1))
                                             : (W >= 8 ? (LMC_PAIR_COLD_LDS < 2 ? LMC_PAIR_COLD_LDS : 2) : LMC_PAIR_COLD_LDS);
+    static constexpr int kQStage = (G == 4 && (NS >= 2 || PL == 0)) ? 2 : 0;
     static constexpr int kL1 = kCold + kColdLds * DP;
-    static constexpr int kL2 = kL1 + 3 * DP;
+    static constexpr int kL2 = kL1 + (G == 4 ? kQStage : 3) * DP;
     static constexpr int kMinDoubles = kL2;
     static constexpr int kGlbLevels = (kNumCold - kColdLds) * DP;
     __host__ __device__ static constexpr int total_doubles(int nlds) { return kL2 + (nlds > 1 ? (nlds - 1) * 4 * DP : 0); }
@@ -576,14 +580,20 @@
 #else
 #define LMC_PAIR_SHAPES(X) X(1, 1) X(2, 1) X(4, 1) X(4, 2) X(4, 4)
 #endif
-constexpr int pair_min_doubles(int ns, int w, int plan = 0) {
-#define X(NSV, WV) if (ns == NSV && w == WV) return (plan == 1 && WV == 1) ? PairLds<NSV, 1, 1>::kMinDoubles : PairLds<NSV, WV, 0>::kMinDoubles;
+constexpr int pair_min_doubles(int ns, int w, int plan = 0, int g = 2) {
+#define X(NSV, WV) if (ns == NSV && w == WV) {                                                                               \
+        if (g == 4 && run_leaf_group(NSV, WV) == 4)                                                                          \
+            return plan == 1 ? PairLds<NSV, 1, 1, 4>::kMinDoubles : PairLds<NSV, 1, 0, 4>::kMinDoubles;                      \
+        return (plan == 1 && WV == 1) ? PairLds<NSV, 1, 1>::kMinDoubles : PairLds<NSV, WV, 0>::kMinDoubles; }
     LMC_PAIR_SHAPES(X)
 #undef X
     return 1 << 30;
 }
-constexpr int pair_total_doubles(int ns, int w, int nlds, int plan = 0) {
-#define X(NSV, WV) if (ns == NSV && w == WV) return (plan == 1 && WV == 1) ? PairLds<NSV, 1, 1>::total_doubles(nlds) : PairLds<NSV, WV, 0>::total_doubles(nlds);
+constexpr int pair_total_doubles(int ns, int w, int nlds, int plan = 0, int g = 2) {
+#define X(NSV, WV) if (ns == NSV && w == WV) {                                                                               \
+        if (g == 4 && run_leaf_group(NSV, WV) == 4)                                                                          \
+            return plan == 1 ? PairLds<NSV, 1, 1, 4>::total_doubles(nlds) : PairLds<NSV, 1, 0, 4>::total_doubles(nlds);      \
+        return (plan == 1 && WV == 1) ? PairLds<NSV, 1, 1>::total_doubles(nlds) : PairLds<NSV, WV, 0>::total_doubles(nlds); }
     LMC_PAIR_SHAPES(X)
 #undef X
     return 1 << 30;
@@ -600,12 +610,12 @@
     int xpar;
 };
 
-template <int NS, int W = 1, int PL = 0>
+template <int NS, int W = 1, int PL = 0, int G = 2>
 __device__ __forceinline__ void red_put(const PairCtx& cx, int v, double x) {
     if constexpr (W == 1) ((lds_double*)cx.lds)[v * 64 + lane_id()] = x;
     else ((lds_double*)cx.lds)[v * 64 + lane_id() + cx.wave_red] = x;
 }
-template <int NS, int W = 1, int PL = 0>
+template <int NS, int W = 1, int PL = 0, int G = 2>
 __device__ __forceinline__ double red_gather(PairCtx& cx) {
     typedef double d2 __attribute__((ext_vector_type(2)));
     typedef __attribute__((address_space(3))) d2 lds_d2;
@@ -622,7 +632,7 @@
     s += dpp_f64<0x114>(s);
     if constexpr (W > 1) {
         const int lane = lane_id();
-        lds_double* xs = L + (PairLds<NS, W, PL>::kXsum + cx.xpar * (8 * W)) + (lane >> 3) * W;
+        lds_double* xs = L + (PairLds<NS, W, PL, G>::kXsum + cx.xpar * (8 * W)) + (lane >> 3) * W;
         if ((lane & 7) == 7) xs[cx.wave] = s;
         __syncthreads();
         double t = xs[0];
@@ -633,9 +643,9 @@
     }
     return s;
 }
-__device__ __forceinline__ int red_lane_init() {
+__device__ __forceinline__ int red_lane_init(int rows = kRedValues) {
     const int lane = lane_id();
-    const int row = lane < 8 * kRedValues ? lane : 0;
+    const int row = lane < 8 * rows ? lane : 0;
     return row * 8 + 2 * ((lane >> 2) & 3);
 }
 __device__ __forceinline__ bool red_any_nonpositive(double s, int k0, int n) {
@@ -666,13 +676,13 @@
 #endif
     return c;
 }
-template <int NS, int W = 1, int PL = 0>
+template <int NS, int W = 1, int PL = 0, int G = 2>
 __device__ __forceinline__ double exp_lanes(const PairCtx& cx, const ExpLanesConst& c, double x) {
     const double kf = rint(x * c.inv);
     double r = __builtin_fma(-kf, c.hi, x);
     r = __builtin_fma(-kf, c.lo, r);
     const int ki = static_cast<int>(kf);
-    const double t = ((const lds_double*)cx.lds)[PairLds<NS, W, PL>::kExp + (ki & 31)];
+    const double t = ((const lds_double*)cx.lds)[PairLds<NS, W, PL, G>::kExp + (ki & 31)];
     double p = fma_sgpr_addend(r, c.c6, c.c5);
     p = fma_sgpr_addend(p, r, c.c4);
     p = fma_sgpr_addend(p, r, c.c3);
@@ -682,91 +692,91 @@
     return ldexp(p * t, ki >> 5);
 }
 
-template <int NS, int W, int PL, int SLOT>
+template <int NS, int W, int PL, int G, int SLOT>
 __device__ __forceinline__ void cold_load(const PairCtx& cx, double (&x)[NS]) {
-    using L = PairLds<NS, W, PL>;
+    using L = PairLds<NS, W, PL, G>;
     if constexpr (SLOT < L::kColdLds) vload_as<NS>((lds_double*)cx.lds + (L::kCold + SLOT * L::DP), x);
     else vload_as<NS>((glb_double*)cx.glb + (SLOT - L::kColdLds) * L::DP, x);
 }
-template <int NS, int W, int PL, int SLOT>
+template <int NS, int W, int PL, int G, int SLOT>
 __device__ __forceinline__ void cold_store(const PairCtx& cx, const double (&x)[NS]) {
-    using L = PairLds<NS, W, PL>;
+    using L = PairLds<NS, W, PL, G>;
     if constexpr (SLOT < L::kColdLds) vstore_as<NS>((lds_double*)cx.lds + (L::kCold + SLOT * L::DP), x);
     else vstore_as<NS>((glb_double*)cx.glb + (SLOT - L::kColdLds) * L::DP, x);
 }
-template <int NS, int W = 1, int PL = 0>
+template <int NS, int W = 1, int PL = 0, int G = 2>
 __device__ __forceinline__ void level1_load(const PairCtx& cx, double (&lp)[NS], double (&rp)[NS], double (&ps)[NS]) {
-    using L = PairLds<NS, W, PL>;
+    using L = PairLds<NS, W, PL, G>;
     lds_double* b = (lds_double*)cx.lds + L::kL1;
     vload_as<NS>(b, lp); vload_as<NS>(b + L::DP, rp);
 #pragma unroll
     for (int s = 0; s < NS; ++s) ps[s] = lp[s] + rp[s];
 }
-template <int NS, int W = 1, int PL = 0>
+template <int NS, int W = 1, int PL = 0, int G = 2>
 __device__ __forceinline__ void level1_store(const PairCtx& cx, const double (&lp)[NS], const double (&rp)[NS], const double (&pq)[NS]) {
-    using L = PairLds<NS, W, PL>;
+    using L = PairLds<NS, W, PL, G>;
     lds_double* b = (lds_double*)cx.lds + L::kL1;
     vstore_as<NS>(b, lp); vstore_as<NS>(b + L::DP, rp); vstore_as<NS>(b + 2 * L::DP, pq);
 }
-template <int NS, int W = 1, int PL = 0>
+template <int NS, int W = 1, int PL = 0, int G = 2>
 __device__ __forceinline__ unsigned glb_level_offset(const PairCtx& cx, int j, int v) {
-    using L = PairLds<NS, W, PL>;
+    using L = PairLds<NS, W, PL, G>;
     unsigned off = L::kGlbLevels + static_cast<unsigned>(j - cx.nlds - 1) * (4u * L::DP) + static_cast<unsigned>(v) * L::DP;
     asm volatile("" : "+s"(off));
     return off;
 }
-template <int NS, int W = 1, int PL = 0>
+template <int NS, int W = 1, int PL = 0, int G = 2>
 __device__ __forceinline__ void levelN_load(const PairCtx& cx, int j, int v, double (&x)[NS]) {
-    using L = PairLds<NS, W, PL>;
+    using L = PairLds<NS, W, PL, G>;
     int nl = cx.nlds;
     asm volatile("" : "+s"(nl));
     if (j <= nl) vload_as<NS>((lds_double*)cx.lds + (L::kL2 + (j - 2) * 4 * L::DP + v * L::DP), x);
-    else vload_as<NS>((glb_double*)cx.glb + glb_level_offset<NS, W, PL>(cx, j, v), x);
-}
-template <int NS, int W = 1, int PL = 0>
+    else vload_as<NS>((glb_double*)cx.glb + glb_level_offset<NS, W, PL, G>(cx, j, v), x);
+}
+template <int NS, int W = 1, int PL = 0, int G = 2>
 __device__ __forceinline__ void levelN_store(const PairCtx& cx, int j, int v, const double (&x)[NS]) {
-    using L = PairLds<NS, W, PL>;
+    using L = PairLds<NS, W, PL, G>;
     int nl = cx.nlds;
     asm volatile("" : "+s"(nl));
     if (j <= nl) vstore_as<NS>((lds_double*)cx.lds + (L::kL2 + (j - 2) * 4 * L::DP + v * L::DP), x);
-    else vstore_as<NS>((glb_double*)cx.glb + glb_level_offset<NS, W, PL>(cx, j, v), x);
-}
-template <int NS, int W = 1, int PL = 0>
+    else vstore_as<NS>((glb_double*)cx.glb + glb_level_offset<NS, W, PL, G>(cx, j, v), x);
+}
+template <int NS, int W = 1, int PL = 0, int G = 2>
 __device__ __forceinline__ void level_load_lp(const PairCtx& cx, int j, double (&x)[NS]) {
-    if (j == 1) vload_as<NS>((lds_double*)cx.lds + PairLds<NS, W, PL>::kL1, x); else levelN_load<NS, W, PL>(cx, j, 0, x);
-}
-template <int NS, int W = 1, int PL = 0>
+    if (j == 1) vload_as<NS>((lds_double*)cx.lds + PairLds<NS, W, PL, G>::kL1, x); else levelN_load<NS, W, PL, G>(cx, j, 0, x);
+}
+template <int NS, int W = 1, int PL = 0, int G = 2>
 __device__ __forceinline__ void level_load_q(const PairCtx& cx, int j, double (&x)[NS]) {
-    if (j == 1) vload_as<NS>((lds_double*)cx.lds + (PairLds<NS, W, PL>::kL1 + 2 * PairLds<NS, W, PL>::DP), x); else levelN_load<NS, W, PL>(cx, j, 3, x);
-}
-template <int NS, int W = 1, int PL = 0>
+    if (j == 1) vload_as<NS>((lds_double*)cx.lds + (PairLds<NS, W, PL, G>::kL1 + 2 * PairLds<NS, W, PL, G>::DP), x); else levelN_load<NS, W, PL, G>(cx, j, 3, x);
+}
+template <int NS, int W = 1, int PL = 0, int G = 2>
 __device__ __forceinline__ void level_scal_put(const PairCtx& cx, int j, double w, double a, double pe, double plogp) {
     if (lane_id() == 0) {
-        lds_double* s = (lds_double*)cx.lds + (PairLds<NS, W, PL>::kScal + 4 * j) + (W > 1 ? cx.wave_scal : 0);
+        lds_double* s = (lds_double*)cx.lds + (PairLds<NS, W, PL, G>::kScal + 4 * j) + (W > 1 ? cx.wave_scal : 0);
         s[0] = w; s[1] = a; s[2] = pe; s[3] = plogp;
     }
 }
-template <int NS, int W = 1, int PL = 0>
+template <int NS, int W = 1, int PL = 0, int G = 2>
 __device__ __forceinline__ void level_scal_get_wa(const PairCtx& cx, int j, double& w, double& a) {
-    const lds_double* s = (const lds_double*)cx.lds + (PairLds<NS, W, PL>::kScal + 4 * j) + (W > 1 ? cx.wave_scal : 0);
+    const lds_double* s = (const lds_double*)cx.lds + (PairLds<NS, W, PL, G>::kScal + 4 * j) + (W > 1 ? cx.wave_scal : 0);
     w = s[0]; a = s[1];
 }
-template <int NS, int W = 1, int PL = 0>
+template <int NS, int W = 1, int PL = 0, int G = 2>
 __device__ __forceinline__ void level_scal_park(const PairCtx& cx, int j, double w, double a, int src, int elane, double en, double lp) {
-    lds_double* s = (lds_double*)cx.lds + (PairLds<NS, W, PL>::kScal + 4 * j) + (W > 1 ? cx.wave_scal : 0);
+    lds_double* s = (lds_double*)cx.lds + (PairLds<NS, W, PL, G>::kScal + 4 * j) + (W > 1 ? cx.wave_scal : 0);
     const int lane = lane_id();
     if (src < 0) {
         if (lane == elane) { s[2] = en; s[3] = lp; }
     } else {
-        const lds_double* f = (const lds_double*)cx.lds + (PairLds<NS, W, PL>::kScal + 4 * src) + (W > 1 ? cx.wave_scal : 0);
+        const lds_double* f = (const lds_double*)cx.lds + (PairLds<NS, W, PL, G>::kScal + 4 * src) + (W > 1 ? cx.wave_scal : 0);
         const double pe = f[2], pl = f[3];
         if (lane == 0) { s[2] = pe; s[3] = pl; }
     }
     if (lane == 0) { s[0] = w; s[1] = a; }
 }
-template <int NS, int W = 1, int PL = 0>
+template <int NS, int W = 1, int PL = 0, int G = 2>
 __device__ __forceinline__ void level_scal_get(const PairCtx& cx, int j, double& w, double& a, double& pe, double& plogp) {
-    const lds_double* s = (const lds_double*)cx.lds + (PairLds<NS, W, PL>::kScal + 4 * j) + (W > 1 ? cx.wave_scal : 0);
+    const lds_double* s = (const lds_double*)cx.lds + (PairLds<NS, W, PL, G>::kScal + 4 * j) + (W > 1 ? cx.wave_scal : 0);
     w = s[0]; a = s[1]; pe = s[2]; plogp = s[3];
 }
 
@@ -797,7 +807,7 @@
     kin_part = kin;
 }
 
-template <int NS, int W = 1, int PL = 0>
+template <int NS, int W = 1, int PL = 0, int G = 2>
 __device__ __forceinline__ double cascade_dots(PairCtx& cx, const double (&var)[NS], const double (&alp)[NS],
                                                const double (&arp)[NS], const double (&aps)[NS], const double (&tl)[NS],
                                                double (&tps)[NS], const double (&v)[NS]) {
@@ -813,12 +823,12 @@
         d4 = __builtin_fma(p2, varp, d4); d5 = __builtin_fma(p2, v[s], d5);
         tps[s] = ps;
     }
-    red_put<NS, W, PL>(cx, 0, d0); red_put<NS, W, PL>(cx, 1, d1); red_put<NS, W, PL>(cx, 2, d2);
-    red_put<NS, W, PL>(cx, 3, d3); red_put<NS, W, PL>(cx, 4, d4); red_put<NS, W, PL>(cx, 5, d5);
-    return red_gather<NS, W, PL>(cx);
-}
-
-template <int NS, int PL, class Target, class TeamT>
+    red_put<NS, W, PL, G>(cx, 0, d0); red_put<NS, W, PL, G>(cx, 1, d1); red_put<NS, W, PL, G>(cx, 2, d2);
+    red_put<NS, W, PL, G>(cx, 3, d3); red_put<NS, W, PL, G>(cx, 4, d4); red_put<NS, W, PL, G>(cx, 5, d5);
+    return red_gather<NS, W, PL, G>(cx);
+}
+
+template <int NS, int PL, int G, class Target, class TeamT>
 __device__ inline void nuts_transition2(TeamT& tm, const Target& tgt, const double (&var)[NS], RngState& rng,
                                         PairCtx& cx, double* qrow, const double (&q)[NS],
                                         const double (&p0)[NS], const double (&g0)[NS], double e0, double logp0,
@@ -827,13 +837,13 @@
     constexpr int W = TeamT::kWaves;
     double cq[NS], cp[NS], cg[NS];
     vcopy(cq, q); vcopy(cp, p0); vcopy(cg, g0);
-    cold_store<NS, W, PL, kColdOq>(cx, q); cold_store<NS, W, PL, kColdOp>(cx, p0); cold_store<NS, W, PL, kColdOg>(cx, g0);
-    cold_store<NS, W, PL, kColdPsum>(cx, p0);
+    cold_store<NS, W, PL, G, kColdOq>(cx, q); cold_store<NS, W, PL, G, kColdOp>(cx, p0); cold_store<NS, W, PL, G, kColdOg>(cx, g0);
+    cold_store<NS, W, PL, G, kColdPsum>(cx, p0);
     bool c_right = true;
     bool c_start = momentum_f32, o_start = momentum_f32;
     double prop_e = e0, prop_logp = logp0;
     double coff = 0.0;
-    lds_double* tot = (lds_double*)cx.lds + PairLds<NS, W, PL>::kScal + (W > 1 ? cx.wave_scal : 0);
+    lds_double* tot = (lds_double*)cx.lds + PairLds<NS, W, PL, G>::kScal + (W > 1 ? cx.wave_scal : 0);
     if (lane_id() == 0) { tot[0] = 0.0; tot[1] = 0.0; tot[2] = 1.0; tot[3] = 0.0; }
     int depth = 0, n_leap = 0;
     bool diverging = false, turning = false, exhausted = true;
@@ -872,7 +882,7 @@
                     const double f = exp_uniform(coff - x);
                     const int lane = lane_id();
                     if (lane >= 1 && lane < kLevelScalDoubles / 4) {
-                        lds_double* sc = (lds_double*)cx.lds + (PairLds<NS, W, PL>::kScal + 4 * lane) + (W > 1 ? cx.wave_scal : 0);
+                        lds_double* sc = (lds_double*)cx.lds + (PairLds<NS, W, PL, G>::kScal + 4 * lane) + (W > 1 ? cx.wave_scal : 0);
                         sc[0] = sc[0] * f; sc[1] = sc[1] * f;
                     }
                     coff = x;
@@ -887,7 +897,7 @@
         const double x = -de;
         const double xn = dpp_f64<0x101>(x);
         const double arg = odd_lane ? (x - coff) : ((xn - coff) + fmin(xn, 0.0));
-        ev = exp_lanes<NS, W, PL>(cx, ec, arg);
+        ev = exp_lanes<NS, W, PL, G>(cx, ec, arg);
         return ok;
     };
 
@@ -896,45 +906,56 @@
         const double eps = right ? step_size : -step_size;
         if (right != c_right) {
             double t[NS];
-            cold_load<NS, W, PL, kColdOq>(cx, t); cold_store<NS, W, PL, kColdOq>(cx, cq); vcopy(cq, t);
-            cold_load<NS, W, PL, kColdOp>(cx, t); cold_store<NS, W, PL, kColdOp>(cx, cp); vcopy(cp, t);
-            cold_load<NS, W, PL, kColdOg>(cx, t); cold_store<NS, W, PL, kColdOg>(cx, cg); vcopy(cg, t);
+            cold_load<NS, W, PL, G, kColdOq>(cx, t); cold_store<NS, W, PL, G, kColdOq>(cx, cq); vcopy(cq, t);
+            cold_load<NS, W, PL, G, kColdOp>(cx, t); cold_store<NS, W, PL, G, kColdOp>(cx, cp); vcopy(cp, t);
+            cold_load<NS, W, PL, G, kColdOg>(cx, t); cold_store<NS, W, PL, G, kColdOg>(cx, cg); vcopy(cg, t);
             const bool tb = c_start; c_start = o_start; o_start = tb;
             c_right = right;
         }
-        cold_store<NS, W, PL, kColdAold>(cx, cp);
+        cold_store<NS, W, PL, G, kColdAold>(cx, cp);
         const bool aold_start = c_start;
 
         double tps[NS], eq[NS], ep[NS];
+        double q0r[NS], q1r[NS];
         double tw = 0.0, ta = 0.0;
         int qsrc = -1;
+        auto prop_q = [&](double (&t)[NS]) {
+            if (qsrc == -1) vcopy(t, cq);
+            else if (qsrc == -2) vcopy(t, eq);
+            else if (G == 4 && qsrc < -2) {
+                if constexpr (PairLds<NS, W, PL, G>::kQStage > 0)
+                    vload_as<NS>((lds_double*)cx.lds + (PairLds<NS, W, PL, G>::kL1 + (qsrc == -3 ? PairLds<NS, W, PL, G>::DP : 0)), t);
+                else if (qsrc == -3) vcopy(t, q1r);
+                else vcopy(t, q0r);
+            } else level_load_q<NS, W, PL, G>(cx, qsrc, t);
+        };
         int elane = 15;
         double en_last = 0.0, lp_last = 0.0;
         const int D = depth;
         if (D == 0) {
             double v[NS], kinp, lp, en, ev;
             leapfrog_partial<NS>(tm, tgt, var, eps, cq, cp, cg, v, kinp, lp);
-            red_put<NS, W, PL>(cx, 0, kinp); red_put<NS, W, PL>(cx, 1, lp);
-            const double s0 = red_gather<NS, W, PL>(cx);
+            red_put<NS, W, PL, G>(cx, 0, kinp); red_put<NS, W, PL, G>(cx, 1, lp);
+            const double s0 = red_gather<NS, W, PL, G>(cx);
             if (leaf_scalars(s0, 1, en, ev) == 1) {
                 tw = readlane_f64(ev, 15); ta = readlane_f64(ev, 14);
                 en_last = en; lp_last = s0;
                 vcopy(tps, cp);
             }
-        } else {
+        } else if (G == 2 || D == 1) {
             const int n_pairs = 1 << (D - 1);
             for (int k = 0; k < n_pairs; ++k) {
                 double v[NS], kinA, lpA, kinB, lpB;
                 leapfrog_partial<NS>(tm, tgt, var, eps, cq, cp, cg, v, kinA, lpA);
-                red_put<NS, W, PL>(cx, 0, kinA); red_put<NS, W, PL>(cx, 1, lpA);
+                red_put<NS, W, PL, G>(cx, 0, kinA); red_put<NS, W, PL, G>(cx, 1, lpA);
                 vcopy(eq, cq); vcopy(ep, cp);
                 leapfrog_partial<NS>(tm, tgt, var, eps, cq, cp, cg, v, kinB, lpB);
-                red_put<NS, W, PL>(cx, 2, kinB); red_put<NS, W, PL>(cx, 3, lpB);
+                red_put<NS, W, PL, G>(cx, 2, kinB); red_put<NS, W, PL, G>(cx, 3, lpB);
 #pragma unroll
                 for (int s = 0; s < NS; ++s) tps[s] = ep[s] + cp[s];
-                red_put<NS, W, PL>(cx, 4, pdot_v<NS>(tps, var, ep));
-                red_put<NS, W, PL>(cx, 5, pdot<NS>(tps, v));
-                const double s0 = red_gather<NS, W, PL>(cx);
+                red_put<NS, W, PL, G>(cx, 4, pdot_v<NS>(tps, var, ep));
+                red_put<NS, W, PL, G>(cx, 5, pdot<NS>(tps, v));
+                const double s0 = red_gather<NS, W, PL, G>(cx);
                 const int m = __builtin_ctz(~static_cast<unsigned>(k) | (1u << (D - 1)));
                 double en, ev;
                 if (leaf_scalars(s0, 2, en, ev) != 2) break;
@@ -950,12 +971,13 @@
                     tw = wsum; ta = aA + aB;
                     if (turn) { turning = true; break; }
                 }
+                if constexpr (G == 2) {
                 if (m >= 1) {
                     double alp[NS], arp[NS], aps[NS];
                     double aw, aa;
-                    level1_load<NS, W, PL>(cx, alp, arp, aps);
-                    level_scal_get_wa<NS, W, PL>(cx, 1, aw, aa);
-                    const double sj = cascade_dots<NS, W, PL>(cx, var, alp, arp, aps, ep, tps, v);
+                    level1_load<NS, W, PL, G>(cx, alp, arp, aps);
+                    level_scal_get_wa<NS, W, PL, G>(cx, 1, aw, aa);
+                    const double sj = cascade_dots<NS, W, PL, G>(cx, var, alp, arp, aps, ep, tps, v);
                     const bool turn = red_any_nonpositive(sj, 0, 6);
                     const double wsum = aw + tw;
                     const bool take_b = uniform_true(team_uniform(tm, rng, win) * wsum < tw);
@@ -965,11 +987,11 @@
                 }
                 for (int j = 2; j <= m; ++j) {
                     double blp[NS], brp[NS], bps[NS], tl[NS];
-                    levelN_load<NS, W, PL>(cx, j, 0, blp); levelN_load<NS, W, PL>(cx, j, 1, brp); levelN_load<NS, W, PL>(cx, j, 2, bps);
-                    level_load_lp<NS, W, PL>(cx, j - 1, tl);
+                    levelN_load<NS, W, PL, G>(cx, j, 0, blp); levelN_load<NS, W, PL, G>(cx, j, 1, brp); levelN_load<NS, W, PL, G>(cx, j, 2, bps);
+                    level_load_lp<NS, W, PL, G>(cx, j - 1, tl);
                     double bw, ba;
-                    level_scal_get_wa<NS, W, PL>(cx, j, bw, ba);
-                    const double sj = cascade_dots<NS, W, PL>(cx, var, blp, brp, bps, tl, tps, v);
+                    level_scal_get_wa<NS, W, PL, G>(cx, j, bw, ba);
+                    const double sj = cascade_dots<NS, W, PL, G>(cx, var, blp, brp, bps, tl, tps, v);
                     const bool turn = red_any_nonpositive(sj, 0, 6);
                     const double wsum = bw + tw;
                     const bool take_b = uniform_true(team_uniform(tm, rng, win) * wsum < tw);
@@ -980,26 +1002,185 @@
                 if (turning) break;
                 if (k + 1 < n_pairs) {
                     double tl[NS], tqv[NS];
-                    if (m == 0) vcopy(tl, ep); else level_load_lp<NS, W, PL>(cx, m, tl);
+                    if (m == 0) vcopy(tl, ep); else level_load_lp<NS, W, PL, G>(cx, m, tl);
                     if (qsrc == -1) vcopy(tqv, cq);
                     else if (qsrc == -2) vcopy(tqv, eq);
-                    else level_load_q<NS, W, PL>(cx, qsrc, tqv);
+                    else level_load_q<NS, W, PL, G>(cx, qsrc, tqv);
 #ifndef LMC_PARK_REORDER_MIN_NS
 #define LMC_PARK_REORDER_MIN_NS 4
 #endif
                     constexpr bool kParkReorder = NS >= LMC_PARK_REORDER_MIN_NS;
-                    if constexpr (kParkReorder) level_scal_park<NS, W, PL>(cx, m + 1, tw, ta, qsrc, elane, en_last, lp_last);
+                    if constexpr (kParkReorder) level_scal_park<NS, W, PL, G>(cx, m + 1, tw, ta, qsrc, elane, en_last, lp_last);
                     if (m == 0) {
-                        level1_store<NS, W, PL>(cx, tl, cp, tqv);
+                        level1_store<NS, W, PL, G>(cx, tl, cp, tqv);
                     } else {
                         if constexpr (kParkReorder) {
 #pragma unroll
                             for (int s = 0; s < NS; ++s) asm volatile("" : "+v"(tl[s]), "+v"(tqv[s]));
                         }
-                        levelN_store<NS, W, PL>(cx, m + 1, 0, tl); levelN_store<NS, W, PL>(cx, m + 1, 1, cp);
-                        levelN_store<NS, W, PL>(cx, m + 1, 2, tps); levelN_store<NS, W, PL>(cx, m + 1, 3, tqv);
+                        levelN_store<NS, W, PL, G>(cx, m + 1, 0, tl); levelN_store<NS, W, PL, G>(cx, m + 1, 1, cp);
+                        levelN_store<NS, W, PL, G>(cx, m + 1, 2, tps); levelN_store<NS, W, PL, G>(cx, m + 1, 3, tqv);
                     }
-                    if constexpr (!kParkReorder) level_scal_park<NS, W, PL>(cx, m + 1, tw, ta, qsrc, elane, en_last, lp_last);
+                    if constexpr (!kParkReorder) level_scal_park<NS, W, PL, G>(cx, m + 1, tw, ta, qsrc, elane, en_last, lp_last);
+                }
+                }
+            }
+        } else if constexpr (G == 4) {
+            using L = PairLds<NS, W, PL, G>;
+            lds_double* const qst = (lds_double*)cx.lds + L::kL1;
+            const int n_quads = 1 << (D - 2);
+            for (int k = 0; k < n_quads; ++k) {
+                static_assert(NS <= 2, "leaf quads: the left end of a depth-2 subtree waits in two rows of the reduction buffer");
+                double v[NS], kin, lpl, a0[NS], a1[NS];
+                leapfrog_partial<NS>(tm, tgt, var, eps, cq, cp, cg, v, kin, lpl);
+                red_put<NS, W, PL, G>(cx, 0, kin); red_put<NS, W, PL, G>(cx, 1, lpl);
+                if constexpr (L::kQStage > 0) vstore_as<NS>(qst, cq); else vcopy(q0r, cq);
+                vcopy(a0, cp);
+                leapfrog_partial<NS>(tm, tgt, var, eps, cq, cp, cg, v, kin, lpl);
+                red_put<NS, W, PL, G>(cx, 2, kin); red_put<NS, W, PL, G>(cx, 3, lpl);
+                if constexpr (L::kQStage > 0) vstore_as<NS>(qst + L::DP, cq); else vcopy(q1r, cq);
+                vcopy(a1, cp);
+                leapfrog_partial<NS>(tm, tgt, var, eps, cq, cp, cg, v, kin, lpl);
+                red_put<NS, W, PL, G>(cx, 4, kin); red_put<NS, W, PL, G>(cx, 5, lpl);
+                vcopy(eq, cq); vcopy(ep, cp);
+                leapfrog_partial<NS>(tm, tgt, var, eps, cq, cp, cg, v, kin, lpl);
+                red_put<NS, W, PL, G>(cx, 6, kin); red_put<NS, W, PL, G>(cx, 7, lpl);
+                const double s0 = red_gather<NS, W, PL, G>(cx);
+                double ta01[NS], va1[NS];
+#pragma unroll
+                for (int s = 0; s < NS; ++s) { ta01[s] = a0[s] + a1[s]; va1[s] = var[s] * a1[s]; tps[s] = ep[s] + cp[s]; }
+                red_put<NS, W, PL, G>(cx, 0, pdot_v<NS>(ta01, var, a0));
+                red_put<NS, W, PL, G>(cx, 1, pdot<NS>(ta01, va1));
+                red_put<NS, W, PL, G>(cx, 2, pdot_v<NS>(tps, var, ep));
+                red_put<NS, W, PL, G>(cx, 3, pdot<NS>(tps, v));
+                double s1, s2;
+                {
+                    double d0 = 0.0, d1 = 0.0, d2 = 0.0, d3 = 0.0, d4 = 0.0, d5 = 0.0;
+#pragma unroll
+                    for (int s = 0; s < NS; ++s) {
+                        const double p1 = ta01[s] + ep[s];
+                        const double p2 = a1[s] + tps[s];
+                        const double ps = ta01[s] + tps[s];
+                        const double valp = var[s] * a0[s], vtlp = var[s] * ep[s], varp = var[s] * a1[s];
+                        d0 = __builtin_fma(ps, valp, d0); d1 = __builtin_fma(ps, v[s], d1);
+                        d2 = __builtin_fma(p1, valp, d2); d3 = __builtin_fma(p1, vtlp, d3);
+                        d4 = __builtin_fma(p2, varp, d4); d5 = __builtin_fma(p2, v[s], d5);
+                        tps[s] = ps;
+                    }
+                    red_put<NS, W, PL, G>(cx, 4, d0); red_put<NS, W, PL, G>(cx, 5, d1);
+                    red_put<NS, W, PL, G>(cx, 6, d2); red_put<NS, W, PL, G>(cx, 7, d3);
+                    s1 = red_gather<NS, W, PL, G>(cx);
+                    red_put<NS, W, PL, G>(cx, 0, d4); red_put<NS, W, PL, G>(cx, 1, d5);
+                    s2 = red_gather<NS, W, PL, G>(cx);
+                }
+                const unsigned long long np1 = ballot64(s1 <= 0.0), np2 = ballot64(s2 <= 0.0);
+                const ExpLanesConst ec = exp_lanes_const();
+                const double en = 0.5 * dpp_f64<0x118>(s0) - s0;
+                double de_x = en - e0;
+                const unsigned long long rare = ballot64(!(fabs(de_x) < emax)) | ballot64((-de_x) - coff > 600.0);
+                de_x = isnan(de_x) ? __builtin_inf() : de_x;
+                auto weights = [&]() {
+                    const double x = -de_x;
+                    const double xn = dpp_f64<0x101>(x);
+                    const double arg = odd_lane ? (x - coff) : ((xn - coff) + fmin(xn, 0.0));
+                    return exp_lanes<NS, W, PL, G>(cx, ec, arg);
+                };
+                double twA = 0.0, taA = 0.0;
+                auto leaves_seq = [&](int i0, bool hold) -> int {
+                    int seen = 0;
+                    for (int i = i0; i < i0 + 2; ++i) {
+                        const double dei = readlane_f64(de_x, 15 + 16 * i);
+                        ++n_leap; ++seen;
+                        if (!(fabs(dei) < emax)) { diverging = true; break; }
+                        const double xi = -dei;
+                        if (xi - coff > 600.0) {
+                            const double f = exp_uniform(coff - xi);
+                            const int lane = lane_id();
+                            if (lane >= 1 && lane < kLevelScalDoubles / 4) {
+                                lds_double* sc = (lds_double*)cx.lds + (L::kScal + 4 * lane);
+                                sc[0] = sc[0] * f; sc[1] = sc[1] * f;
+                            }
+                            if (hold) { twA = twA * f; taA = taA * f; }
+                            coff = xi;
+                        }
+                    }
+                    return seen;
+                };
+                const bool fast = (rare & ((1ull << 15) | (1ull << 31) | (1ull << 47) | (1ull << 63))) == 0ull;
+                auto mde_update = [&](double dx, bool examined) {
+                    const bool upd = (fabs(dx) > fabs(mde)) & examined;
+                    mde = upd ? dx : mde;
+                };
+                int seen = 2;
+                if (fast) n_leap += 2; else seen = leaves_seq(0, false);
+                double ev = weights();
+                double w2 = readlane_f64(ev, 47), a2w = readlane_f64(ev, 46), w3 = readlane_f64(ev, 63), a3w = readlane_f64(ev, 62);
+                mde_update(de_x, lane15 | (lane31 & (seen == 2)));
+                if (diverging) break;
+                int elane_a;
+                {
+                    const double w0 = readlane_f64(ev, 15), a0w = readlane_f64(ev, 14);
+                    const double w1 = readlane_f64(ev, 31), a1w = readlane_f64(ev, 30);
+                    const bool turn = (np1 & ((1ull << 7) | (1ull << 15))) != 0ull;
+                    const double wsum = w0 + w1;
+                    const bool take_b = uniform_true(team_uniform(tm, rng, win) * wsum < w1);
+                    elane_a = take_b ? 31 : 15;
+                    twA = wsum; taA = a0w + a1w;
+                    if (turn) { turning = true; break; }
+                }
+                if (fast) n_leap += 2;
+                else {
+                    seen = leaves_seq(2, true);
+                    ev = weights();
+                    w2 = readlane_f64(ev, 47); a2w = readlane_f64(ev, 46); w3 = readlane_f64(ev, 63); a3w = readlane_f64(ev, 62);
+                }
+                mde_update(upper_half_down(de_x), lane15 | (lane31 & (seen == 2)));
+                if (diverging) break;
+                {
+                    const bool turn = (np1 & ((1ull << 23) | (1ull << 31))) != 0ull;
+                    const double wsum = w2 + w3;
+                    const bool take_b = uniform_true(team_uniform(tm, rng, win) * wsum < w3);
+                    elane = take_b ? 63 : 47;
+                    tw = wsum; ta = a2w + a3w;
+                    if (turn) { turning = true; break; }
+                }
+                {
+                    const bool turn = ((np1 & ((1ull << 39) | (1ull << 47) | (1ull << 55) | (1ull << 63))) |
+                                       (np2 & ((1ull << 7) | (1ull << 15)))) != 0ull;
+                    const double wsum = twA + tw;
+                    const bool take_b = uniform_true(team_uniform(tm, rng, win) * wsum < tw);
+                    if (!take_b) elane = elane_a;
+                    tw = wsum; ta = taA + ta;
+                    qsrc = elane == 63 ? -1 : elane == 47 ? -2 : elane == 31 ? -3 : -4;
+                    en_last = en; lp_last = s0;
+                    if (turn) { turning = true; break; }
+                }
+                const int m = 1 + __builtin_ctz(~static_cast<unsigned>(k) | (1u << (D - 2)));
+                for (int j = 2; j <= m; ++j) {
+                    double blp[NS], brp[NS], bps[NS], tl[NS];
+                    levelN_load<NS, W, PL, G>(cx, j, 0, blp); levelN_load<NS, W, PL, G>(cx, j, 1, brp); levelN_load<NS, W, PL, G>(cx, j, 2, bps);
+                    if (j == 2) vcopy(tl, a0); else levelN_load<NS, W, PL, G>(cx, j - 1, 0, tl);
+                    double bw, ba;
+                    level_scal_get_wa<NS, W, PL, G>(cx, j, bw, ba);
+                    const double sj = cascade_dots<NS, W, PL, G>(cx, var, blp, brp, bps, tl, tps, v);
+                    const bool turn = red_any_nonpositive(sj, 0, 6);
+                    const double wsum = bw + tw;
+                    const bool take_b = uniform_true(team_uniform(tm, rng, win) * wsum < tw);
+                    if (!take_b) qsrc = j;
+                    tw = wsum; ta = ba + ta;
+                    if (turn) { turning = true; break; }
+                }
+                if (turning) break;
+                if (k + 1 < n_quads) {
+                    double tl[NS], tqv[NS];
+                    if (m == 1) vcopy(tl, a0); else levelN_load<NS, W, PL, G>(cx, m, 0, tl);
+                    prop_q(tqv);
+                    levelN_store<NS, W, PL, G>(cx, m + 1, 0, tl); levelN_store<NS, W, PL, G>(cx, m + 1, 1, cp);
+                    levelN_store<NS, W, PL, G>(cx, m + 1, 2, tps); levelN_store<NS, W, PL, G>(cx, m + 1, 3, tqv);
+                    level_scal_park<NS, W, PL, G>(cx, m + 1, tw, ta, qsrc, elane, en_last, lp_last);
+                } else if (D == 2) {
+#pragma unroll
+                    for (int s = 0; s < NS; ++s) ((lds_double*)cx.lds)[(6 + s) * 64 + lane_id()] = a0[s];
                 }
             }
         }
@@ -1015,15 +1196,13 @@
         }
         if (uniform_true(team_uniform(tm, rng, win) * (w_start + wn) < tw)) {
             double tqv[NS];
-            if (qsrc == -1) vcopy(tqv, cq);
-            else if (qsrc == -2) vcopy(tqv, eq);
-            else level_load_q<NS, W, PL>(cx, qsrc, tqv);
+            prop_q(tqv);
             vstore_as<NS>((glb_double*)qrow, tqv);
             if (qsrc < 0) {
                 prop_e = readlane_f64(en_last, elane); prop_logp = readlane_f64(lp_last, elane);
             } else {
                 double w_, a_;
-                level_scal_get<NS, W, PL>(cx, qsrc, w_, a_, prop_e, prop_logp);
+                level_scal_get<NS, W, PL, G>(cx, qsrc, w_, a_, prop_e, prop_logp);
                 prop_e = first_f64(prop_e); prop_logp = first_f64(prop_logp);
             }
         }
@@ -1031,14 +1210,18 @@
         double tlp[NS], psum[NS], op[NS], aold[NS];
         if (D == 0) vcopy(tlp, cp);
         else if (D == 1) vcopy(tlp, ep);
-        else level_load_lp<NS, W, PL>(cx, D - 1, tlp);
-        cold_load<NS, W, PL, kColdPsum>(cx, psum); cold_load<NS, W, PL, kColdOp>(cx, op); cold_load<NS, W, PL, kColdAold>(cx, aold);
+        else if (G == 4 && D == 2) {
+#pragma unroll
+            for (int s = 0; s < NS; ++s) tlp[s] = ((const lds_double*)cx.lds)[(6 + s) * 64 + lane_id()];
+        }
+        else level_load_lp<NS, W, PL, G>(cx, D - 1, tlp);
+        cold_load<NS, W, PL, G, kColdPsum>(cx, psum); cold_load<NS, W, PL, G, kColdOp>(cx, op); cold_load<NS, W, PL, G, kColdAold>(cx, aold);
 #pragma unroll
         for (int s = 0; s < NS; ++s) {
             const double t = psum[s] + tps[s];
             psum[s] = momentum_f32 ? static_cast<double>(static_cast<float>(t)) : t;
         }
-        cold_store<NS, W, PL, kColdPsum>(cx, psum);
+        cold_store<NS, W, PL, G, kColdPsum>(cx, psum);
         double ov[NS], av[NS];
         end_velocity<NS>(ov, var, op, o_start);
         end_velocity<NS>(av, var, aold, aold_start);
@@ -1063,9 +1246,9 @@
             }
         }
         c_start = false;
-        red_put<NS, W, PL>(cx, 0, d0); red_put<NS, W, PL>(cx, 1, d1); red_put<NS, W, PL>(cx, 2, d2);
-        red_put<NS, W, PL>(cx, 3, d3); red_put<NS, W, PL>(cx, 4, d4); red_put<NS, W, PL>(cx, 5, d5);
-        if (red_any_nonpositive(red_gather<NS, W, PL>(cx), 0, 6)) { turning = true; exhausted = false; break; }
+        red_put<NS, W, PL, G>(cx, 0, d0); red_put<NS, W, PL, G>(cx, 1, d1); red_put<NS, W, PL, G>(cx, 2, d2);
+        red_put<NS, W, PL, G>(cx, 3, d3); red_put<NS, W, PL, G>(cx, 4, d4); red_put<NS, W, PL, G>(cx, 5, d5);
+        if (red_any_nonpositive(red_gather<NS, W, PL, G>(cx), 0, 6)) { turning = true; exhausted = false; break; }
     }
 
     const double wn_end = first_f64(tot[0]), an_end = first_f64(tot[1]);
@@ -1309,7 +1492,7 @@
     ++ms.n_samples;
 }
 
-template <int NS, int W, template <int> class TargetT, int RNG = 0, int PL = 0>
+template <int NS, int W, template <int> class TargetT, int RNG = 0, int PL = 0, int G = run_leaf_group(NS, W)>
 __global__ __launch_bounds__(64 * W, run_waves_per_simd(NS, W)) void run_kernel(ChainArrays, SamplerParams, const double* tparams) {
     extern __shared__ __attribute__((aligned(16))) double lds[];
     const long long t_resident = wall_clock64();
@@ -1377,11 +1560,11 @@
     cx.glb = A0.scratch + static_cast<long long>(c) * A0.scratch_stride;
     cx.nlds = P0.nlds;
     cx.wave = tm.wave();
-    cx.wave_red = W > 1 ? cx.wave * PairLds<NS, W>::kRedWave : 0;
+    cx.wave_red = W > 1 ? cx.wave * PairLds<NS, W, PL, G>::kRedWave : 0;
     cx.wave_scal = W > 1 ? cx.wave * kLevelScalDoubles : 0;
-    cx.red_lane = static_cast<int>(reinterpret_cast<size_t>((lds_double*)lds + (red_lane_init() + cx.wave_red)));
+    cx.red_lane = static_cast<int>(reinterpret_cast<size_t>((lds_double*)lds + (red_lane_init(PairLds<NS, W, PL, G>::kRedRows) + cx.wave_red)));
     cx.xpar = 0;
-    if (tid < kExpTableDoubles) lds[PairLds<NS, W>::kExp + tid] = kExp2Table[2 * tid];
+    if (tid < kExpTableDoubles) lds[PairLds<NS, W, PL, G>::kExp + tid] = kExp2Table[2 * tid];
     tm.sync();
 
 #ifdef LMC_PHASE_TIMING
@@ -1448,7 +1631,7 @@
         TransitionOut out;
         if (P.kind == 0) {
             const int md = (tune && iter_count < 200) ? P.early_max_treedepth : P.max_treedepth;
-            nuts_transition2<NS, PL>(tm, tgt, vard, rng, cx, qrow, q, p0, g0, e0, logp0, step_size, P.emax, md,
+            nuts_transition2<NS, PL, G>(tm, tgt, vard, rng, cx, qrow, q, p0, g0, e0, logp0, step_size, P.emax, md,
                                  momentum_f32, out);
             vload<NS>(qrow, q);
             if (out.exhausted && !tune) ++ct_maxdepth;
diff --git a/littlemcmc_amd/csrc/lmc_wave.hpp b/littlemcmc_amd/csrc/lmc_wave.hpp
--- a/littlemcmc_amd/csrc/lmc_wave.hpp
+++ b/littlemcmc_amd/csrc/lmc_wave.hpp
@@ -59,6 +59,13 @@
                                                      static_cast<unsigned>(__double2hiint(b)), false, false);
     return __hiloint2double(static_cast<int>(hi[0]), static_cast<int>(lo[0])) +
            __hiloint2double(static_cast<int>(hi[1]), static_cast<int>(lo[1]));
+}
+__device__ __forceinline__ double upper_half_down(double x) {
+    const auto lo = __builtin_amdgcn_permlane32_swap(static_cast<unsigned>(__double2loint(x)),
+                                                     static_cast<unsigned>(__double2loint(x)), false, false);
+    const auto hi = __builtin_amdgcn_permlane32_swap(static_cast<unsigned>(__double2hiint(x)),
+                                                     static_cast<unsigned>(__double2hiint(x)), false, false);
+    return __hiloint2double(static_cast<int>(hi[1]), static_cast<int>(lo[1]));
 }
 __device__ __forceinline__ double swap16_add(double a, double b) {
     const auto lo = __builtin_amdgcn_permlane16_swap(static_cast<unsigned>(__double2loint(a)),
diff --git a/littlemcmc_amd/engine.py b/littlemcmc_amd/engine.py
--- a/littlemcmc_amd/engine.py
+++ b/littlemcmc_amd/engine.py
@@ -126,6 +126,7 @@
     "LMC_DENSE_CACHE_ROWS": ("dense_cache_rows_p1", lambda v: int(v) + 1),
     "LMC_DENSE_LDS_SLOTS": ("dense_lds_slots_p1", lambda v: int(v) + 1),
     "LMC_CHOL_HBM": ("chol_hbm", lambda v: int(int(v) != 0)),
+    "LMC_LEAF_GROUP": ("leaf_group", int),
 }
 
 
@@ -370,6 +371,9 @@
 
     def last_run_plan(self):
         return {_abi.LDS_PLAN_SHALLOW: "shallow", _abi.LDS_PLAN_DEEP: "deep"}.get(int(self._lib.lmc_engine_last_run_plan(self._h)))
+
+    def last_run_leaf_group(self):
+        return int(self._lib.lmc_engine_last_run_leaf_group(self._h)) or None
 
     def run_streams(self):
         arr = (C.c_void_p * _abi.MAX_RUN_STREAMS)()
```
